# taichi-dev/taichi-nerfs

Measured on AMD Instinct MI355X. Metric: training rays/sec, higher is better.
Workload: dtype f32-table+f16-mlp

## Files before the change

include/ngp_hip.h:

```cpp
#ifndef NGP_HIP_H
#define NGP_HIP_H

#include <stdint.h>

#ifdef __cplusplus
extern "C" {
#endif

#define NGP_MAX_LEVELS 16
#define NGP_ABI_VERSION 3

typedef struct ngp_hash_levels {
    int32_t  n_levels;
    int32_t  n_features;
    int32_t  begin_fast_hash_level;
    int32_t  total_entries;
    float    scale[NGP_MAX_LEVELS];
    uint32_t resolution[NGP_MAX_LEVELS];
    uint32_t map_size[NGP_MAX_LEVELS];
    uint32_t offset[NGP_MAX_LEVELS];
    uint32_t bwd_plan;
} ngp_hash_levels;

#define NGP_BWD_PLAN_DETERMINISTIC 1u
#define NGP_BWD_PLAN_CONCENTRATED  2u

int ngp_abi_version(void);


int ngp_hash_levels_init(ngp_hash_levels* lv, double max_params, int levels, double base_res,
                         double max_res, int features);

int ngp_ray_aabb(const float* rays_o, const float* rays_d, float scale, int n_rays,
                 float* hits_t , void* stream);

int ngp_bitfield_coarsen(const uint8_t* density_bitfield, int cascades, int grid_size, uint32_t* coarse,
                         void* stream);
int ngp_march_train_count_ex(const float* rays_o, const float* rays_d, const float* hits_t,
                             const uint8_t* density_bitfield, const uint32_t* coarse, const float* noise,
                             int cascades, int grid_size, float scale, float exp_step_factor, int max_samples,
                             int n_rays, float* stage, int32_t* counts, void* stream);
int ngp_march_train_fused(const float* rays_o, const float* rays_d, const float* hits_t,
                          const uint8_t* density_bitfield, const uint32_t* coarse, const float* noise, int cascades,
                          int grid_size, float scale, float exp_step_factor, int max_samples, int n_rays,
                          float* stage, int32_t* ctr, int32_t* rays_a, int32_t* total, float* xyzs, float* dirs,
                          float* deltas, float* ts, void* stream);
int ngp_march_train_fused_cap(const float* rays_o, const float* rays_d, const float* hits_t, const uint8_t* density_bitfield,
                              const uint32_t* coarse, const float* noise, int cascades, int grid_size, float scale,
                              float exp_step_factor, int max_samples, int n_rays, long long capacity, float* stage, int32_t* ctr,
                              int32_t* rays_a, int32_t* total, float* xyzs, float* dirs, float* deltas, float* ts, void* stream);
int ngp_march_train_fused_rng(const float* rays_o, const float* rays_d, const float* hits_t, const uint8_t* density_bitfield,
                              const uint32_t* coarse, unsigned long long seed, int cascades, int grid_size, float scale,
                              float exp_step_factor, int max_samples, int n_rays, float* stage, int32_t* ctr, int32_t* rays_a,
                              int32_t* total, float* xyzs, float* dirs, float* deltas, float* ts, void* stream);
int ngp_march_train_fused_shaped(const float* rays_o, const float* rays_d, const float* hits_t, const uint8_t* density_bitfield,
                                 const uint32_t* coarse, const float* noise, unsigned long long seed, int cascades, int grid_size,
                                 float scale, float exp_step_factor, int max_samples, int n_rays, int block_waves, int lds_pad_bytes,
                                 float* stage, int32_t* ctr, int32_t* rays_a, int32_t* total, float* xyzs, float* dirs, float* deltas,
                                 float* ts, void* stream);
int ngp_rng_uniform(unsigned long long seed, int n, float* out, void* stream);
int ngp_march_train_scan(const int32_t* counts, int n_rays, int32_t* rays_a ,
                         int32_t* total , void* stream);
int ngp_march_train_write(const float* rays_o, const float* rays_d, const int32_t* rays_a,
                          const float* stage, int max_samples, int n_rays,
                          float* xyzs, float* dirs, float* deltas, float* ts, void* stream);

int ngp_march_test(const float* rays_o, const float* rays_d, float* hits_t ,
                   const int64_t* alive_indices, const uint8_t* density_bitfield,
                   int cascades, int grid_size, float scale, float exp_step_factor,
                   int max_samples, int n_alive,
                   int64_t* ray_indices, uint8_t* valid_mask, float* deltas, float* ts,
                   int32_t* samples_counter, void* stream);

int ngp_hash_fwd_f32(const float* xyzs , const float* table,
                     const ngp_hash_levels* lv, int n, float* out , void* stream);
int ngp_hash_bwd_f32(const float* xyzs, const float* dout ,
                     const ngp_hash_levels* lv, int n, float* dtable, void* stream);

int ngp_hash_bwd_input_f32 (const float* xyzs, const float* table, const float* denc , const ngp_hash_levels* lv, int n,
                            float* dxyzs , void* stream);
int ngp_hash_bwd_input_bf16(const float* xyzs, const uint16_t* table, const float* denc , const ngp_hash_levels* lv, int n,
                            float* dxyzs , void* stream);
int ngp_hash_bwd_input_f16 (const float* xyzs, const uint16_t* table, const uint16_t* denc , const ngp_hash_levels* lv,
                            int n, float* dxyzs , void* stream);

int ngp_hash_bwd2_gather_f32 (const float* xyzs, const float* table, const float* denc , const float* ddx ,
                              const ngp_hash_levels* lv, int n, float* d_denc , float* d_xyzs ,
                              void* stream);
int ngp_hash_bwd2_gather_bf16(const float* xyzs, const uint16_t* table, const float* denc , const float* ddx ,
                              const ngp_hash_levels* lv, int n, float* d_denc , float* d_xyzs ,
                              void* stream);
int ngp_hash_bwd2_table_f32  (const float* xyzs, const float* denc , const float* ddx , const ngp_hash_levels* lv,
                              int n, float* dtable , void* stream);

int ngp_hash_fwd_f32_ex(const float* xyzs, const float* table, const ngp_hash_levels* lv, int n_max,
                        const int32_t* n_dev, int normalize, float lo, float hi, int enc_pairs, float* out,
                        void* stream);
int ngp_hash_fwd_bf16_ex(const float* xyzs, const uint16_t* table, const ngp_hash_levels* lv, int n_max,
                         const int32_t* n_dev, int normalize, float lo, float hi, int enc_pairs, float* out,
                         void* stream);
int ngp_hash_fwd_list(const float* xyzs, const void* table, int table_kind, const ngp_hash_levels* lv, int n_max,
                      const int32_t* n_list, const int32_t* list, int normalize, float lo, float hi, int enc_pairs, float* out,
                      void* stream);

typedef struct ngp_triplane_levels {
    int32_t  n_levels;
    int32_t  n_features;
    int32_t  max_res;
    int32_t  reserved;
    float    scale[NGP_MAX_LEVELS];
    uint32_t resolution[NGP_MAX_LEVELS];
} ngp_triplane_levels;

int ngp_triplane_levels_init(ngp_triplane_levels* lv, double base_res, double max_res, int levels, int features);
int ngp_triplane_fwd_f32(const float* xyzs , const float* table, const ngp_triplane_levels* lv, int n, int normalize,
                         float lo, float hi, float* out , void* stream);
int ngp_triplane_bwd_f32(const float* xyzs, const float* dout , const float* table, const ngp_triplane_levels* lv,
                         int n, int normalize, float lo, float hi, float* dtable, void* stream);

int ngp_voxel_fwd(const float* xyzs , const float* dirs , const float* sh, const float* density, int n,
                  int grid_size, int sh_degree, float grid_min, float grid_radius, float* sigmas , float* rgbs ,
                  void* stream);
int ngp_voxel_density(const float* xyzs, const float* density, int n, int grid_size, float grid_min, float grid_radius,
                      float* sigmas, void* stream);
int ngp_voxel_bwd(const float* xyzs, const float* dirs, const float* sigmas, const float* rgbs, const float* dsigmas ,
                  const float* drgbs , int n, int grid_size, int sh_degree, float grid_min, float grid_radius, float* dsh,
                  float* ddensity, void* stream);
int ngp_voxel_trilinear_fwd(const float* xyzs , const float* dirs , const float* sh, const float* density,
                            int n, int grid_size, int sh_degree, float grid_min, float grid_radius, float* sigmas ,
                            float* rgbs , void* stream);
int ngp_voxel_trilinear_density(const float* xyzs, const float* density, int n, int grid_size, float grid_min, float grid_radius,
                                float* sigmas, void* stream);
int ngp_voxel_trilinear_bwd(const float* xyzs, const float* dirs, const float* sigmas, const float* rgbs, const float* dsigmas ,
                            const float* drgbs , int n, int grid_size, int sh_degree, float grid_min, float grid_radius,
                            float* dsh, float* ddensity, void* stream);
int ngp_voxel_occ_scratch_doubles(void);
int ngp_voxel_occ_pack(const float* density_grid, long long n_bytes, double density_threshold, double* scratch, uint8_t* bitfield,
                       void* stream);

int ngp_hash_fwd_f16(const float* xyzs, const uint16_t* table, const ngp_hash_levels* lv, int n,
                     uint16_t* out , void* stream);
int ngp_hash_bwd_f16(const float* xyzs, const uint16_t* dout, const ngp_hash_levels* lv, int n,
                     uint16_t* dtable , void* stream);

int ngp_hash_fwd_f16_ex(const float* xyzs, const uint16_t* table, const ngp_hash_levels* lv, int n_max,
                        const int32_t* n_dev, int normalize, float lo, float hi, int enc_pairs, float* out,
                        void* stream);
int ngp_check_finite_f16(const uint16_t* g, long long n, int32_t* found_inf, void* stream);

int ngp_sh16_fwd(const float* dirs , int n, float* out , void* stream);
int ngp_sh16_bwd(const float* dirs, const float* dout , int n, float* ddirs ,
                 void* stream);

int ngp_composite_train_fwd(const float* sigmas, const void* rgbs, int rgbs_is_half,
                            const float* deltas, const float* ts, const int32_t* rays_a,
                            float T_threshold, int n_rays,
                            int32_t* total_samples , float* opacity, float* depth,
                            float* rgb , float* ws , void* stream);
int ngp_composite_train_bwd(const float* dL_dopacity, const float* dL_ddepth, const float* dL_drgb,
                            const float* dL_dws, const float* sigmas, const void* rgbs,
                            int rgbs_is_half, const float* deltas, const float* ts,
                            const int32_t* rays_a, const float* opacity, const float* depth,
                            const float* rgb, const float* ws, float T_threshold, int n_rays,
                            float* dL_dsigmas, void* dL_drgbs, void* stream);
int ngp_composite_train_fwd_bg(const float* sigmas, const void* rgbs, int rgbs_is_half, const float* deltas, const float* ts,
                               const int32_t* rays_a, float T_threshold, int n_rays, int32_t* total_samples, float* opacity,
                               float* depth, float* rgb, float* ws, float* rgb_out, float bg, void* stream);
int ngp_composite_train_bwd_bg(const float* dL_dopacity, const float* dL_ddepth, const float* dL_drgb, const float* dL_dws,
                               const float* sigmas, const void* rgbs, int rgbs_is_half, const float* deltas, const float* ts,
                               const int32_t* rays_a, const float* opacity, const float* depth, const float* rgb, const float* ws,
                               float T_threshold, int n_rays, float* dL_dsigmas, void* dL_drgbs, float bg, void* stream);

int ngp_chunk_schedule(const int32_t* rays_a, const float* sigmas, const float* deltas, int n_rays, int begin, int len,
                       int prev_begin, float thr_stop, float* T_state, int32_t* list, int32_t* count, int32_t* count_zero,
                       void* stream);
int ngp_live_list(const int32_t* rays_a, const int32_t* vr_per_ray , int n_rays, int32_t* live_idx,
                  int32_t* live_total, int32_t* live_zero, void* stream);
int ngp_composite_train_fused_live(const float* sigmas, const void* rgbs, int rgbs_is_half, const float* deltas,
                                   const float* ts, const int32_t* rays_a, const float* target, float bg,
                                   const float* loss_scale, float T_threshold, int n_rays, int32_t* vr_per_ray,
                                   float* opacity, float* depth, float* rgb, float* ws, float* d_sigmas, void* d_rgbs,
                                   float* sq_err, int32_t* live_idx, int32_t* live_total, int32_t* live_zero,
                                   void* stream);

int ngp_live_compact(const int32_t* rays_a, const int32_t* vr_per_ray , int n_rays, int32_t* live_off,
                     int32_t* live_idx, int32_t* live_total, void* stream);
int ngp_mlp_bwd_live(const float* enc, const float* dirs, const uint16_t* wpack, const float* dsigmas, const uint16_t* drgbs,
                     int n_max, const int32_t* n_dev, const int32_t* live_idx, int enc_pairs, float* d_enc, float* dW,
                     int32_t* found_inf, void* stream);
int ngp_mlp_dw_parts_max(void);
int ngp_mlp_bwd_live_parts(const float* enc, const float* dirs, const uint16_t* wpack, const float* dsigmas,
                           const uint16_t* drgbs, int n_max, const int32_t* n_dev, const int32_t* live_idx, int enc_pairs,
                           float* d_enc, float* dW_parts, int32_t* found_inf, void* stream);
int ngp_mlp_dw_reduce(const float* dW_parts, int n_parts, float* dW, void* stream);
int ngp_hash_bwd_f32_live(const float* xyzs, const float* dout, const ngp_hash_levels* lv, int n_max, const int32_t* n_dev,
                          const int32_t* live_idx, int normalize, float lo, float hi, int enc_pairs, float* dtable,
                          int32_t* found_inf, void* stream);
int ngp_hash_bwd_f16_live(const float* xyzs, const float* dout, const ngp_hash_levels* lv, int n_max, const int32_t* n_dev,
                          const int32_t* live_idx, int normalize, float lo, float hi, int enc_pairs, uint16_t* dtable,
                          int32_t* found_inf, void* stream);
long long ngp_hash_bwd_sliced_workspace(const ngp_hash_levels* lv, int n_max);
int ngp_hash_bwd_sliced_prep(const float* xyzs, const ngp_hash_levels* lv, int n_max, const int32_t* n_dev,
                             const int32_t* live_idx, int normalize, float lo, float hi, void* workspace,
                             long long workspace_bytes, void* stream);
int ngp_hash_bwd_sliced_main(const float* dout, const ngp_hash_levels* lv, int n_max, const int32_t* n_dev, int enc_pairs,
                             float* dtable, int32_t* found_inf, const void* workspace, long long workspace_bytes,
                             void* stream);
int ngp_hash_bwd_sliced_main_slabs(const float* dout, const ngp_hash_levels* lv, int n_max, const int32_t* n_dev, int enc_pairs,
                                   void* dtable, int table_is_f16, int32_t* found_inf, const void* workspace,
                                   long long workspace_bytes, const float* mlp_dw_parts, int n_parts, float* mlp_dw, void* stream);
long long ngp_hash_bwd_sliced_adam_prefix(const ngp_hash_levels* lv);
int ngp_hash_bwd_sliced_main_adam_step(const float* dout, const ngp_hash_levels* lv, int n_max, const int32_t* n_dev, int enc_pairs,
                                       float* dtable, const void* workspace, long long workspace_bytes, const float* mlp_dw_parts,
                                       int n_parts, float* mlp_dw, float* table, float* table_m, float* table_v, uint16_t* table_bf16,
                                       float* state_f, int32_t* state_i, float lr0, float eta_min, int t_max, float beta1, float beta2,
                                       float eps, float growth, float backoff, int growth_interval, void* stream);
int ngp_hash_bwd_sliced_main_f16(const float* dout, const ngp_hash_levels* lv, int n_max, const int32_t* n_dev, int enc_pairs,
                                 uint16_t* dtable_f16, int32_t* found_inf, const void* workspace, long long workspace_bytes,
                                 void* stream);
int ngp_hash_bwd_f32_sliced(const float* xyzs, const float* dout, const ngp_hash_levels* lv, int n_max, const int32_t* n_dev,
                            const int32_t* live_idx, int normalize, float lo, float hi, int enc_pairs, float* dtable,
                            int32_t* found_inf, void* workspace, long long workspace_bytes, void* stream);

int ngp_composite_test(const float* sigmas, const void* rgbs, int rgbs_is_half, const float* deltas,
                       const float* ts, const int64_t* pack_info ,
                       int64_t* alive_indices , float T_threshold, int n_alive,
                       float* opacity, float* depth, float* rgb, void* stream);

int ngp_mlp_wpack_halfs(void);
int ngp_mlp_pack(const float* W1, const float* W2, const float* W3, const float* W4, const float* W5,
                 int enc_pairs, uint16_t* wpack, void* stream);
int ngp_mlp_fwd(const float* enc, const float* dirs, const uint16_t* wpack, int n, float* sigmas,
                uint16_t* rgbs, void* stream);
int ngp_mlp_bwd(const float* enc, const float* dirs, const uint16_t* wpack, const float* dsigmas,
                const uint16_t* drgbs, int n, float* d_enc, float* dW, void* stream);

int ngp_mlp_fwd_ex(const float* enc, const float* dirs, const uint16_t* wpack, int n_max, const int32_t* n_dev,
                   int enc_pairs, float* sigmas, uint16_t* rgbs, void* stream);
int ngp_mlp_fwd_list(const float* enc, const float* dirs, const uint16_t* wpack, int n_max, const int32_t* n_list,
                     const int32_t* list, int enc_pairs, float* sigmas, uint16_t* rgbs, void* stream);

int ngp_event_create(void** event);
int ngp_event_record(void* event, void* stream);
int ngp_stream_wait_event(void* stream, void* event);
int ngp_event_destroy(void* event);
int ngp_event_synchronize(void* event);
int ngp_stream_create_low_priority(void** stream, int* least, int* greatest);
int ngp_stream_destroy(void* stream);
int ngp_host_alloc(void** host, long long bytes);
int ngp_host_free(void* host);
int ngp_copy_to_host_async(void* host, const void* dev, long long bytes, void* stream);

typedef struct ngp_render_args {
    const float* rays_o; const float* rays_d; const float* hits_t ; const float* noise ;
    int32_t n_rays, max_samples;
    const uint8_t* bitfield; uint32_t* coarse; int32_t rebuild_coarse, cascades, grid_size;
    float scale, exp_step_factor, T_threshold;
    const void* table; int32_t table_kind , enc_pairs;
    const ngp_hash_levels* levels; float lo, hi;
    const float* w[5]; uint16_t* wpack;
    long long cap;
    float* stage; int32_t* march_ctr; float* xyzs; float* dirs; float* deltas; float* ts; float* enc; float* sigmas; uint16_t* rgbs; float* ws;
    int32_t* rays_a; int32_t* total; int32_t* vr_per_ray; float* opacity; float* depth; float* rgb;
    const float* g_opacity; const float* g_depth; const float* g_rgb; const float* g_ws;
    float* d_sigmas; uint16_t* d_rgbs; float* d_enc; int32_t* live_off; int32_t* live_idx; int32_t* live_total;
    void* workspace; long long workspace_bytes;
    int32_t force_atomic, reserved;
    float* dW_parts; int32_t* live_zero;
    float* dW ; void* dtable ; long long dtable_bytes;
    float bg; int32_t clear_grads; float* rgb_out;
} ngp_render_args;
int ngp_render_train_fwd(const ngp_render_args* args, void* stream);
int ngp_render_train_bwd(const ngp_render_args* args, void* stream);

int ngp_mse_loss_grad(const float* rgb, const float* opacity, const float* target, float bg, int n_rays,
                      float* state_f, float* g_rgb, float* g_opacity, void* stream);
int ngp_mse_loss_grad_rays(const float* rgb, const float* opacity, const float* target, float bg, int n_rays,
                           const float* state_f, float* g_rgb, float* g_opacity, float* sq_err, void* stream);
int ngp_train_prologue(float* state_f, int32_t* state_i, float lr0, float eta_min, int t_max, float beta1,
                       float beta2, float growth, float backoff, int growth_interval, void* stream);
int ngp_train_prologue_reduce(float* state_f, int32_t* state_i, float lr0, float eta_min, int t_max, float beta1,
                              float beta2, float growth, float backoff, int growth_interval, const float* dW_parts,
                              int n_parts, float* dW, void* stream);
int ngp_adam_amp_prologue(float* state_f, int32_t* state_i, const float* grad_scale, const float* found_inf, float lr,
                          float beta1, float beta2, void* stream);
#define NGP_ADAM_MULTI_MAX 16
int ngp_adam_multi(int n_tensors, float* const* p, float* const* g, float* const* m, float* const* v, const long long* n,
                   const float* state_f, const int32_t* state_i, float beta1, float beta2, float eps, void* stream);
int ngp_check_finite_multi(int n_tensors, const float* const* g, const long long* n, float* found_inf, void* stream);
int ngp_adam_amp_check_prologue(int n_tensors, const float* const* g, const long long* n, float* found_inf, float* clear_next,
                                uint32_t* done, float* state_f, int32_t* state_i, const float* grad_scale, float lr, float beta1,
                                float beta2, void* stream);
int ngp_cast_f32_bf16(const float* src, uint16_t* dst, long long n, void* stream);
int ngp_adam_all_ex(float* table, void* table_g, int grad_is_f16, float* table_m, float* table_v, long long n,
                    uint16_t* table_16, int copy_kind, float* mlp, float* mlp_g, float* mlp_m, float* mlp_v,
                    const float* state_f, const int32_t* state_i, float beta1, float beta2, float eps, int enc_pairs,
                    uint16_t* wpack, void* stream);
int ngp_adam_mlp_pack(float* p, float* g, float* m, float* v, const float* state_f, const int32_t* state_i,
                      float beta1, float beta2, float eps, int enc_pairs, uint16_t* wpack, void* stream);

int ngp_morton3d(const int32_t* coords , int m, int32_t* indices, void* stream);
int ngp_morton3d_invert(const int32_t* indices, int m, int32_t* coords , void* stream);
int ngp_packbits(const float* density_grid , float threshold, int n_bytes,
                 uint8_t* bitfield, void* stream);

int ngp_distortion_fwd(const float* ws, const float* deltas, const float* ts, const int32_t* rays_a, int n_rays,
                       float* loss, float* ws_inc, float* wts_inc, void* stream);
int ngp_distortion_bwd(const float* dL_dloss, const float* ws, const float* deltas, const float* ts,
                       const float* ws_inc, const float* wts_inc, const int32_t* rays_a, int n_rays,
                       float* dL_dws, void* stream);

int ngp_get_rays(const float* directions , const float* poses, int per_ray_pose, int n, float* rays_o,
                 float* rays_d, void* stream);
int ngp_stage_batch(const float* a, float* da, const float* b, float* db, const float* c, float* dc, int n, void* stream);
int ngp_sample_rays(const float* poses , const float* directions , const float* rays, int ray_c,
                    long long hw, const int64_t* img_idx, long long img0, const int64_t* pix_idx, int n, float* rays_o,
                    float* rays_d, float* rgb, void* stream);

int ngp_march_train_bwd(const float* d_xyzs , const float* d_dirs , const float* ts ,
                        const int32_t* rays_a , int n_rays, float* d_rays_o , float* d_rays_d , void* stream);
int ngp_sample_rays_bwd(const float* directions , const int64_t* img_idx , long long img0,
                        const int64_t* pix_idx , const float* d_rays_o , const float* d_rays_d ,
                        int n, int n_img, float* d_poses , void* stream);
int ngp_get_rays_bwd(const float* directions , const float* d_rays_o, const float* d_rays_d, int n, float* d_poses , void* stream);

int ngp_occ_compact(const float* density_grid, float threshold, int n_cells, int32_t* list, int32_t* count,
                    int32_t* scratch , void* stream);
int ngp_sorted_uniforms(const float* u, int m, int sets, float* work, float* out, void* stream);
int ngp_occ_sample(const float* u_cell, const float* u_pick, const float* u_jit, const int32_t* list, const int32_t* count,
                   int m, int grid_size, float s, float half_grid, int32_t* indices, float* xyzs, void* stream);
int ngp_occ_all_cells(const float* u_jit, int n_cells, int grid_size, float s, float half_grid, float* xyzs, void* stream);
int ngp_occ_scatter(const int32_t* indices, const float* sigmas, int n, float* tmp, void* stream);
int ngp_occ_scatter_max(const int32_t* indices, const float* sigmas, int n, float* tmp, void* stream);
int ngp_occ_stats_floats(void);
int ngp_occ_merge(float* density_grid, const float* tmp, float decay, int n, float* stats, void* stream);
int ngp_occ_pack(const float* density_grid, float* stats, float density_threshold, int n_bytes, uint8_t* bitfield,
                 void* stream);

int ngp_deploy_shade(const float* xyzs, const float* dirs, const float* table, const ngp_hash_levels* lv, const float* sigma_w,
                     const float* rgb_w, int n, float* sigmas , float* rgbs , float* enc_out, void* stream);

int ngp_deploy_render(const float* rays_o, const float* rays_d, const uint8_t* density_bitfield, const uint32_t* coarse ,
                      const float* table, const ngp_hash_levels* lv, const float* sigma_w, const float* rgb_w, int n_rays,
                      int max_samples, float T_threshold, float* rgb, float* opacity, float* depth, int32_t* n_samples, float* t_last,
                      void* stream);

long long ngp_mesh_workspace_bytes(int nx, int ny, int nz);
int ngp_mesh_count(const float* values, int nx, int ny, int nz, float iso, int sign, void* workspace, int32_t* counts ,
                   void* stream);
int ngp_mesh_emit(const float* values, int nx, int ny, int nz, float iso, int sign, const float* lo ,
                  const float* h , const void* workspace, float* vertices, float* normals , int32_t* faces,
                  void* stream);

#define NGP_MESH_SDF_MAX_LEAF 8
long long ngp_mesh_bvh_bytes(long long n_faces, int leaf_size);
int ngp_mesh_bvh_build(const float* vertices, const int32_t* faces, const int32_t* order, int n_faces, int leaf_size, float* boxes,
                       void* stream);
int ngp_mesh_sdf_query(const float* points, int n, const float* vertices, const int32_t* faces, const int32_t* order, const float* boxes,
                       int n_faces, int leaf_size, const float* edge_normals , const float* vertex_normals ,
                       float* sdf, float* closest , int32_t* face , int32_t* feature ,
                       void* stream);

#define NGP_RAYCAST_ANY_HIT 1
#define NGP_RAYCAST_CULL_BACK 2
#define NGP_RAYCAST_CULL_FRONT 4
int ngp_mesh_raycast(const float* rays_o, const float* rays_d, int n,
                     const float* vertices, const int32_t* faces, const int32_t* order, const float* boxes,
                     int n_faces, int leaf_size, float t_min, float t_max, int flags,
                     float* t , int32_t* face , float* bary ,
                     int32_t* side , void* stream);

long long ngp_mesh_winding_bytes(long long n_faces, int leaf_size);
int ngp_mesh_winding_build(const float* vertices, const int32_t* faces, const int32_t* order, const float* boxes, int n_faces,
                           int leaf_size, float* moments, void* stream);
int ngp_mesh_winding_query(const float* points, int n, const float* vertices, const int32_t* faces, const int32_t* order,
                           const float* moments, int n_faces, int leaf_size, float beta, int order_terms ,
                           float* winding , void* stream);

long long ngp_mesh_components_bytes(int n_faces, int n_vertices);
int ngp_mesh_components_rounds(const int32_t* faces, int n_faces, int n_vertices, int32_t* parent, int32_t* changed, int n_rounds,
                               void* stream);
int ngp_mesh_components_label(const int32_t* faces, int n_faces, int n_vertices, const int32_t* parent, void* workspace,
                              int32_t* vertex_component, int32_t* face_component, int32_t* counts , void* stream);
int ngp_mesh_components_edge_keys(const int32_t* faces, int n_faces, int n_vertices, int64_t* keys , void* stream);
int ngp_mesh_components_table(int n_faces, int n_vertices, const int32_t* vertex_component, const int32_t* face_component,
                              const int64_t* sorted_keys, int n_components, int32_t* table , void* stream);
long long ngp_mesh_components_partial_bytes(int n_faces, int n_components);
int ngp_mesh_components_measure(const float* vertices, const int32_t* faces, const int64_t* order, int n_faces, int n_vertices,
                                const int32_t* face_start, const int32_t* block_start, int n_components, void* partials, double* area,
                                double* volume, float* lo, float* hi, void* stream);
int ngp_mesh_select_count(int n_faces, int n_vertices, const int32_t* vertex_component, const int32_t* face_component,
                          const uint8_t* keep, int n_components, void* workspace, int32_t* vertex_map, int32_t* face_map,
                          int32_t* counts , void* stream);
int ngp_mesh_select_emit(const float* vertices, const float* normals , const int32_t* faces, int n_faces, int n_vertices,
                         const int32_t* vertex_map, const int32_t* face_map, int n_out_vertices, int n_out_faces, float* out_vertices,
                         float* out_normals , int32_t* out_faces, void* stream);

int ngp_surface_composite_fwd(const float* sdf, const float* cosv, const float* rgbs, const float* aux ,
                              const float* deltas, const float* ts, const int32_t* rays_a, const float* inv_s ,
                              float cos_anneal, float T_threshold, int n_rays, float bg, int32_t* total_samples, float* opacity,
                              float* depth, float* rgb, float* rgb_out , float* aux_out , float* ws,
                              float* alphas, void* stream);
int ngp_surface_composite_bwd(const float* dL_dopacity, const float* dL_ddepth, const float* dL_drgb, const float* dL_daux,
                              const float* dL_dws, const float* sdf, const float* cosv, const float* rgbs, const float* aux,
                              const float* deltas, const float* ts, const int32_t* rays_a, const float* inv_s, float cos_anneal, int n_rays,
                              float bg, const int32_t* total_samples, const float* alphas, float* d_sdf, float* d_cos, float* d_rgbs,
                              float* d_aux , float* d_inv_s , float* workspace , void* stream);

int ngp_resample_count(const float* ws, const float* deltas, const float* ts, const int32_t* rays_a, const float* noise, int n_rays,
                       int n_orig, long long n_samples, int K, float floor_w, float* cdf, float* stage_t, int32_t* stage_j,
                       int32_t* counts, int32_t* total , void* stream);
int ngp_resample_scan(const int32_t* counts, const int32_t* rays_a, int n_rays, int32_t* rays_a_out, int32_t* total, void* stream);
int ngp_resample_write(const float* rays_o, const float* rays_d, const float* deltas, const float* ts, const int32_t* rays_a,
                       const int32_t* rays_a_out, const float* stage_t, const int32_t* stage_j, int n_rays, int n_orig,
                       long long n_samples, int K, float* xyzs, float* dirs, float* deltas_out, float* ts_out, int32_t* parent,
                       void* stream);

int ngp_sdf_eval(const float* xyzs, const float* table, const ngp_hash_levels* lv, const float* wpack, int width, int depth, float scale,
                 int n, float* f, float* enc_out , void* stream);
int ngp_sdf_trace(const float* rays_o, const float* rays_d, const uint8_t* density_bitfield, const uint32_t* coarse ,
                  const float* table, const ngp_hash_levels* lv, const float* wpack, int width, int depth, int cascades, float scale,
                  int grid_size, int n_rays, float eps, float step_scale, float min_step, int n_refine, int max_evals, int32_t* status,
                  float* t, float* xyz, int32_t* n_eval, float* f_last, unsigned long long* stats , void* stream);

#ifdef __cplusplus
}
#endif
#endif
```

include/ngp_hip_experimental.h:

```cpp
#ifndef NGP_HIP_EXPERIMENTAL_H
#define NGP_HIP_EXPERIMENTAL_H
#include "ngp_hip.h"

#ifdef __cplusplus
extern "C" {
#endif

int ngp_adam_all(float* table, float* table_g, float* table_m, float* table_v, long long n, uint16_t* table_bf16,
                 float* mlp, float* mlp_g, float* mlp_m, float* mlp_v, const float* state_f, const int32_t* state_i,
                 float beta1, float beta2, float eps, int enc_pairs, uint16_t* wpack, void* stream);

int ngp_adam_step(float* p, float* g, float* m, float* v, long long n, const float* state_f,
                  const int32_t* state_i, float beta1, float beta2, float eps, void* stream);

int ngp_adam_step_bf16(float* p, float* g, float* m, float* v, long long n, const float* state_f,
                       const int32_t* state_i, float beta1, float beta2, float eps, uint16_t* p_bf16, void* stream);

int ngp_composite_train_fused(const float* sigmas, const void* rgbs, int rgbs_is_half, const float* deltas,
                              const float* ts, const int32_t* rays_a, const float* target, float bg,
                              const float* loss_scale, float T_threshold, int n_rays, int32_t* vr_per_ray,
                              float* opacity, float* depth, float* rgb, float* ws, float* d_sigmas, void* d_rgbs,
                              float* sq_err, void* stream);

int ngp_hash_bwd_f16_ex(const float* xyzs, const float* dout, const ngp_hash_levels* lv, int n_max,
                        const int32_t* n_dev, int normalize, float lo, float hi, int enc_pairs, uint16_t* dtable,
                        int32_t* found_inf, void* stream);

int ngp_hash_bwd_f32_ex(const float* xyzs, const float* dout, const ngp_hash_levels* lv, int n_max,
                        const int32_t* n_dev, int normalize, float lo, float hi, int enc_pairs, float* dtable,
                        int32_t* found_inf, void* stream);

int ngp_hash_bwd_sliced_debug(void* device_buffer);

int ngp_hash_bwd_sliced_plan(const ngp_hash_levels* lv, uint16_t* tasks, int max_tasks, uint16_t* xoff , uint16_t* xlen ,
                             uint8_t* nrep , uint32_t* merge_mask, uint32_t* single_mask);

int ngp_march_train_count(const float* rays_o, const float* rays_d, const float* hits_t,
                          const uint8_t* density_bitfield, const float* noise,
                          int cascades, int grid_size, float scale, float exp_step_factor,
                          int max_samples, int n_rays,
                          float* stage , int32_t* counts ,
                          void* stream);

int ngp_mlp_bwd_ex(const float* enc, const float* dirs, const uint16_t* wpack, const float* dsigmas,
                   const uint16_t* drgbs, int n_max, const int32_t* n_dev, int enc_pairs, float* d_enc, float* dW,
                   int32_t* found_inf, void* stream);

int ngp_hash_bwd_sliced_main_adam(const float* dout, const ngp_hash_levels* lv, int n_max, const int32_t* n_dev, int enc_pairs,
                                  float* dtable, const void* workspace, long long workspace_bytes, const float* mlp_dw_parts,
                                  int n_parts, float* mlp_dw, float* table, float* table_m, float* table_v, uint16_t* table_bf16,
                                  const float* state_f, const int32_t* state_i, float beta1, float beta2, float eps,
                                  void* stream);

int ngp_hash_bwd_sliced_main_levels(const float* dout, const ngp_hash_levels* lv, int n_max, const int32_t* n_dev, int enc_pairs,
                                    float* dtable, int32_t* found_inf, const void* workspace, long long workspace_bytes,
                                    unsigned int level_mask, int max_blocks, void* stream);

int ngp_p2p_max_peers(void);
int ngp_p2p_push(const void* src, long long n_per_peer, int elem_bytes, int world, void* const* peer_dst, int32_t* const* peer_flags,
                 long long dst_offset, int broadcast, int rank, int step, uint32_t* done, void* stream);
int ngp_p2p_wait(const int32_t* flags, int world, int step, long long max_spins, const float* inbox, long long n, float scale, int reduce,
                 float* out, int32_t* err, void* stream);

#ifdef __cplusplus
}
#endif
#endif
```

taichi-nerfs_amd/csrc/hash_bwd_lds.hip:

```cpp
#include "ngp_device.h"
#include "hash_common.h"

namespace ngp {

constexpr int BW_SLICE_LOG2 = 13;
constexpr int BW_SLICE_ENTRIES = 1 << BW_SLICE_LOG2;
constexpr int BW_MAX_SLICES = 64;
constexpr int BW_THREADS = 1024;
constexpr int BW_WAVES = BW_THREADS / 64;
constexpr int BW_Q = 256;
constexpr int BW_MAX_TASKS = 1536;
constexpr int BW_PREP_BLOCKS = 2048;
constexpr size_t BW_CTR_BYTES = 64;
constexpr int BW_PERSISTENT_BLOCKS = 256;

struct BwdPlan {
    int32_t n_blocks;
    uint32_t merge_mask;
    uint32_t diag;
    uint32_t det;
    int32_t merge_chunks;
    uint8_t nrep[NGP_MAX_LEVELS];
    uint16_t task[BW_MAX_TASKS];
    uint16_t xoff[8], xlen[8];
// ... 352 lines not shown
            const int i0 = w0 * 64 + lane, i1 = i0 + 64;
            const Batch nxt = load_batch(level, i0, i0 < n, i1, (w0 + 1 < hi_w) && i1 < n, xyzc, dout, plane, enc_pairs, nl, P.diag, HALF);
            accumulate_batch<KIND>(P, sl, pend, slice, found_inf);
            pend = nxt;
        }
        accumulate_batch<KIND>(P, sl, pend, slice, found_inf);
        return;
    }
    int qhead = 0, qlen = 0;
    int SCW = 64;
    if (K == KIND_MERGE || K == KIND_MERGE0) {
        SCW = 4; while (SCW < 64 && SCW < 2 * (int)P.map.ns) SCW <<= 1;
        if (P.merge_chunks > 0) while (SCW > 4 && (hi_w - lo_w) < P.merge_chunks * SCW) SCW >>= 1;
    }
    const int n_sc = (hi_w - lo_w + SCW - 1) / SCW;
    auto load_words = [&](int c) -> unsigned long long {
        const int w = lo_w + c * SCW + lane;
        return (c < n_sc && lane < SCW && w < hi_w) ? brow[w] : 0ull;
    };
    auto grab = [&]() -> int {
        int c = 0;
        if (lane == 0) c = (int)atomicAdd(next_sc, 1u);
        return __builtin_amdgcn_readfirstlane(c);
    };
    auto drain = [&]() {
        __builtin_amdgcn_fence(__ATOMIC_ACQ_REL, "wavefront");
        __builtin_amdgcn_wave_barrier();
        const int i0 = (int)q[(qhead + lane) & (BW_Q - 1)], i1 = (int)q[(qhead + 64 + lane) & (BW_Q - 1)];
        const Batch nxt = load_batch(level, i0, true, i1, true, xyzc, dout, plane, enc_pairs, nl, P.diag, HALF);
        accumulate_batch<KIND>(P, sl, pend, slice, found_inf);
        pend = nxt;
        __builtin_amdgcn_wave_barrier();
        qhead = (qhead + 128) & (BW_Q - 1); qlen -= 128;
    };
    int sc = grab();
    unsigned long long cur = load_words(sc);
    while (sc < n_sc) {
        const int sc_next = grab();
        const unsigned long long nxtw = load_words(sc_next);
        const int wbase = lo_w + sc * SCW;
        if (K == KIND_MERGE || K == KIND_MERGE0) {
            unsigned long long nonzero = __ballot(cur != 0ull);
            while (nonzero) {
                const int k = __builtin_ctzll(nonzero);
                nonzero &= nonzero - 1;
                const unsigned long long b = ((unsigned long long)(uint32_t)__builtin_amdgcn_readlane((int)(cur >> 32), k) << 32) |
                                             (uint32_t)__builtin_amdgcn_readlane((int)cur, k);
                const bool hit = (b >> lane) & 1ull;
                const int pos = qlen + __builtin_amdgcn_mbcnt_hi((uint32_t)(b >> 32), __builtin_amdgcn_mbcnt_lo((uint32_t)b, 0));
                if (hit) q[(qhead + pos) & (BW_Q - 1)] = (uint32_t)((wbase + k) * 64 + lane);
                qlen += __popcll(b);
                if (qlen >= 128) drain();
            }
        } else {
            const unsigned long long w = cur;
            if (__ballot(w != 0ull) != 0ull) {
                int total = 0, pass = 0;
                do {
                    const int sbase = qhead + 128;
                    int off = 0;
#pragma unroll
                    for (int pc = 0; pc < 8; ++pc) {
                        const uint32_t b8 = (uint32_t)(w >> (8 * pc)) & 0xffu;
                        const unsigned long long nz = __ballot(b8 != 0u);
                        const int dst = off - 64 * pass + __builtin_amdgcn_mbcnt_hi((uint32_t)(nz >> 32), __builtin_amdgcn_mbcnt_lo((uint32_t)nz, 0));
                        if (b8 != 0u && (uint32_t)dst < 64u) q[(sbase + dst) & (BW_Q - 1)] = b8 | ((uint32_t)lane << 8) | ((uint32_t)pc << 14);
                        off += __popcll(nz);
                    }
                    total = off;
                    __builtin_amdgcn_fence(__ATOMIC_ACQ_REL, "wavefront");
                    __builtin_amdgcn_wave_barrier();
                    const uint32_t d = (lane < total - 64 * pass) ? q[(sbase + lane) & (BW_Q - 1)] : 0u;
                    __builtin_amdgcn_fence(__ATOMIC_ACQ_REL, "wavefront");
                    __builtin_amdgcn_wave_barrier();
                    uint32_t bits = d & 0xffu;
                    const uint32_t s0 = (uint32_t)(wbase + (int)((d >> 8) & 63u)) * 64u + 8u * (d >> 14);
                    unsigned long long live = __ballot(bits != 0u);
                    while (live) {
                        const int pos = qlen + __builtin_amdgcn_mbcnt_hi((uint32_t)(live >> 32), __builtin_amdgcn_mbcnt_lo((uint32_t)live, 0));
                        if (bits != 0u) {
                            q[(qhead + pos) & (BW_Q - 1)] = s0 + (uint32_t)__builtin_ctz(bits);
                            bits &= bits - 1u;
                        }
                        qlen += __popcll(live);
                        if (qlen >= 128) drain();
                        live = __ballot(bits != 0u);
                    }
                    ++pass;
                } while (64 * pass < total);
            }
        }
        if ((K == KIND_MERGE || K == KIND_MERGE0) && P.det && qlen > 0) {
            __builtin_amdgcn_fence(__ATOMIC_ACQ_REL, "wavefront");
            __builtin_amdgcn_wave_barrier();
            const bool v0 = lane < qlen, v1 = lane + 64 < qlen;
            const int i0 = v0 ? (int)q[(qhead + lane) & (BW_Q - 1)] : 0, i1 = v1 ? (int)q[(qhead + 64 + lane) & (BW_Q - 1)] : 0;
            const Batch nxt = load_batch(level, i0, v0, i1, v1, xyzc, dout, plane, enc_pairs, nl, P.diag, HALF);
            accumulate_batch<KIND>(P, sl, pend, slice, found_inf);
            pend = nxt;
            __builtin_amdgcn_wave_barrier();
            qhead = (qhead + 128) & (BW_Q - 1); qlen = 0;
        }
        cur = nxtw; sc = sc_next;
    }
    if (qlen > 0) {
        __builtin_amdgcn_fence(__ATOMIC_ACQ_REL, "wavefront");
        __builtin_amdgcn_wave_barrier();
        const bool v0 = lane < qlen, v1 = lane + 64 < qlen;
        const int i0 = v0 ? (int)q[(qhead + lane) & (BW_Q - 1)] : 0, i1 = v1 ? (int)q[(qhead + 64 + lane) & (BW_Q - 1)] : 0;
        const Batch nxt = load_batch(level, i0, v0, i1, v1, xyzc, dout, plane, enc_pairs, nl, P.diag, HALF);
        accumulate_batch<KIND>(P, sl, pend, slice, found_inf);
        pend = nxt;
    }
    accumulate_batch<KIND>(P, sl, pend, slice, found_inf);
}

__device__ __forceinline__ uint32_t claim_task(const BwdPlan& plan, uint32_t* __restrict__ ctr, uint32_t xcc, bool& own_empty) {
    const int lane = threadIdx.x & 63;
    if (!own_empty) {
        uint32_t old = 0u;
        if (lane == 0) old = atomicAdd(&ctr[xcc], 1u);
        old = (uint32_t)__builtin_amdgcn_readfirstlane((int)old);
        const uint32_t f = old & 0xffffu, b = old >> 16;
        if (f + b < plan.xlen[xcc]) return plan.xoff[xcc] + f;
        own_empty = true;
    }
    uint32_t dead = 1u << xcc;
    for (int tries = 0; tries < 7; ++tries) {
        int left = 0;
        if (lane < 8 && !((dead >> lane) & 1u)) {
            const uint32_t c = __atomic_load_n(&ctr[lane], __ATOMIC_RELAXED);
            left = (int)plan.xlen[lane] - (int)((c & 0xffffu) + (c >> 16));
        }
        int key = left > 0 ? (left << 3) | (7 - lane) : 0;
#pragma unroll
        for (int d = 1; d < 8; d <<= 1) key = max(key, __shfl_xor(key, d, NGP_WAVE));
        key = __builtin_amdgcn_readfirstlane(key);
        if (key <= 0) break;
        const int best = 7 - (key & 7);
        uint32_t old = 0u;
        if (lane == 0) old = atomicAdd(&ctr[best], 0x10000u);
        old = (uint32_t)__builtin_amdgcn_readfirstlane((int)old);
        const uint32_t f = old & 0xffffu, b = old >> 16;
        if (f + b < plan.xlen[best]) return plan.xoff[best] + plan.xlen[best] - 1u - b;
        dead |= 1u << best;
    }
    return 0xffffffffu;
}

struct MlpSlabs {
    const float* parts;
    int n_parts;
    float* dW;
};

struct FlushAdam {
    float* p;
    float* m;
    float* v;
    uint16_t* shadow;
    const float* sf;
    const int32_t* si;
    float beta1, beta2, eps;
};

struct StepSchedule {
    float* sf;
    int32_t* si;
    float lr0, eta_min;
    int t_max;
    float growth, backoff;
    int growth_interval;
};

template <bool HALF, int ADAM>
__global__ void __launch_bounds__(BW_THREADS) hash_bwd_lds_kernel(const float* __restrict__ xyzc,
                                                                  const unsigned long long* __restrict__ bitmap, size_t wstride,
                                                                  const float* __restrict__ dout, ngp_hash_levels lv, int n,
                                                                  const int32_t* __restrict__ n_dev, int enc_pairs, BwdPlan plan,
                                                                  void* __restrict__ dtable ,
                                                                  int32_t* __restrict__ found_inf, uint32_t* __restrict__ ctr,
                                                                  unsigned long long* __restrict__ dbg, MlpSlabs mlp, FlushAdam ad_in,
                                                                  StepSchedule sch) {
    __shared__ double slice[2 * BW_SLICE_ENTRIES];
    __shared__ float s_sf[8];
    __shared__ int32_t s_si[8];
    FlushAdam ad = ad_in;
    const bool own_schedule = ADAM != 0 && sch.sf != nullptr;
    if (own_schedule) {
        if (threadIdx.x == 0) {
#pragma unroll
            for (int k = 0; k < 8; ++k) { s_sf[k] = sch.sf[k]; s_si[k] = sch.si[k]; }
            train_prologue_thread(s_sf, s_si, sch.lr0, sch.eta_min, sch.t_max, ad.beta1, ad.beta2, sch.growth, sch.backoff,
                                  sch.growth_interval);
        }
        ad.sf = s_sf; ad.si = s_si;
    }
    __shared__ uint32_t queues[BW_WAVES * BW_Q];
    __shared__ uint32_t next_sc;
    __shared__ uint32_t s_claim;
    if (mlp.parts) {
        for (int b = blockIdx.x; b < NGP_MLP_REDUCE_BLOCKS; b += gridDim.x) {
            mlp_dw_reduce_block(mlp.parts, mlp.n_parts, mlp.dW, b);
            __syncthreads();
        }
    }
    const size_t plane = (size_t)n;
    if (n_dev) n = min(n, *n_dev);
    if (n <= 0 && !ADAM) return;
    if (n < 0) n = 0;
    const int tid = threadIdx.x;
    uint32_t xcc;
    asm volatile("s_getreg_b32 %0, hwreg(HW_REG_XCC_ID)" : "=s"(xcc));
    xcc &= 7u;
    double2* s2 = reinterpret_cast<double2*>(slice);
    for (int j = tid; j < BW_SLICE_ENTRIES; j += BW_THREADS) s2[j] = make_double2(0.0, 0.0);
    bool own_empty = false;
    if (tid < 64) {
        const uint32_t c0 = claim_task(plan, ctr, xcc, own_empty);
        if (tid == 0) { s_claim = c0; next_sc = 0u; }
    }
    __syncthreads();
    uint32_t claim = s_claim;
  while (claim != 0xffffffffu) {
    const uint32_t task = plan.task[claim];
    unsigned long long t_begin = 0;
    if (dbg) t_begin = wall_clock64();
    const int level = task & 0xf, rep = (task >> 10) & 0x3f, nrep = plan.nrep[level];
    const uint32_t sl = (task >> 4) & 0x3f;
    LevelParams P;
    P.scale = lv.scale[level]; P.res = lv.resolution[level]; P.size = lv.map_size[level]; P.offset = lv.offset[level];
    P.dense = level < lv.begin_fast_hash_level;
    P.mode = level_mode(lv, level);
    P.map = slice_map(P.size, P.res, P.dense);
    P.diag = plan.diag;
    P.det = plan.det;
    P.merge_chunks = plan.merge_chunks;
    const bool single = P.size <= (uint32_t)BW_SLICE_ENTRIES;
    const bool merge = (plan.merge_mask >> level) & 1u;
    const bool hashed = !P.dense && P.mode == 1u && P.res < (1u << BW_SLICE_LOG2) && !single;

    unsigned long long t_init = 0;
    if (dbg) t_init = wall_clock64();
    uint32_t* q = queues + (tid >> 6) * BW_Q;
    const unsigned long long* brow = bitmap + ((size_t)level * BW_MAX_SLICES + sl) * wstride;
    if (merge && P.dense && P.mode == 0u) bwd_task<KIND_MERGE0 | (HALF ? KIND_HALF : 0)>(P, level, sl, single, n, rep, nrep, xyzc, brow, dout, plane, enc_pairs, lv.n_levels, slice, q, &next_sc, found_inf);
    else if (merge) bwd_task<KIND_MERGE | (HALF ? KIND_HALF : 0)>(P, level, sl, single, n, rep, nrep, xyzc, brow, dout, plane, enc_pairs, lv.n_levels, slice, q, &next_sc, found_inf);
    else if (hashed) bwd_task<KIND_HASHED | (HALF ? KIND_HALF : 0)>(P, level, sl, single, n, rep, nrep, xyzc, brow, dout, plane, enc_pairs, lv.n_levels, slice, q, &next_sc, found_inf);
    else bwd_task<KIND_GENERIC | (HALF ? KIND_HALF : 0)>(P, level, sl, single, n, rep, nrep, xyzc, brow, dout, plane, enc_pairs, lv.n_levels, slice, q, &next_sc, found_inf);
    unsigned long long t_wave = 0;
    if (dbg) t_wave = wall_clock64();
    __syncthreads();
    unsigned long long t_acc = 0;
    if (dbg) t_acc = wall_clock64();
    if (tid < 64) {
        const uint32_t c1 = claim_task(plan, ctr, xcc, own_empty);
        if (tid == 0) { s_claim = c1; next_sc = 0u; }
    }
    if (HALF) {
        typedef _Float16 half2v __attribute__((ext_vector_type(2)));
        half2v* dh = reinterpret_cast<half2v*>(dtable) + P.offset;
        for (int j = tid; j < BW_SLICE_ENTRIES; j += BW_THREADS) {
            const double2 a = s2[j];
            if (a.x == 0.0 && a.y == 0.0) continue;
            s2[j] = make_double2(0.0, 0.0);
            const uint32_t h = entry_of(P.map, sl, (uint32_t)j);
            half2v val;
            val.x = (_Float16)(float)a.x; val.y = (_Float16)(float)a.y;
            if (nrep == 1) dh[h] = dh[h] + val;
            else if (!(val.x == (_Float16)0 && val.y == (_Float16)0))
                __builtin_amdgcn_global_atomic_fadd_v2f16((__attribute__((address_space(1))) half2v*)(dh + h), val);
        }
    } else if (ADAM && nrep == 1) {
        const bool skip = ad.si[SI_SKIP] != 0;
        const AdamConsts ac = adam_consts(ad.sf, ad.beta1, ad.beta2, ad.eps);
        float2* p2 = reinterpret_cast<float2*>(ad.p) + P.offset;
        float2* m2 = reinterpret_cast<float2*>(ad.m) + P.offset;
        float2* v2 = reinterpret_cast<float2*>(ad.v) + P.offset;
        uint32_t* sh = reinterpret_cast<uint32_t*>(ad.shadow) + P.offset;
        constexpr int UNR = BW_SLICE_ENTRIES / BW_THREADS;
        static_assert(UNR * BW_THREADS == BW_SLICE_ENTRIES, "one trip covers the slice");
        {
            float2 pi[UNR], mi[UNR], vi[UNR];
            uint32_t h[UNR];
#pragma unroll
            for (int k = 0; k < UNR; ++k) {
                const int j = tid + k * BW_THREADS;
                h[k] = entry_of(P.map, sl, (uint32_t)j);
                const uint32_t hc = (!skip && h[k] < P.size) ? h[k] : 0u;
                mi[k] = m2[hc]; vi[k] = v2[hc]; pi[k] = p2[hc];
            }
#pragma unroll
            for (int k = 0; k < UNR; ++k) {
                const int j = tid + k * BW_THREADS;
                const double2 a = s2[j];
                if (a.x != 0.0 || a.y != 0.0) s2[j] = make_double2(0.0, 0.0);
                const float gx = 0.0f + (float)a.x, gy = 0.0f + (float)a.y;
                float2 mk = mi[k], vk = vi[k], pk = pi[k];
                const bool in = !skip && h[k] < P.size;
                if (!in || (gx == 0.f && gy == 0.f && mk.x == 0.f && mk.y == 0.f && vk.x == 0.f && vk.y == 0.f)) continue;
                if (!(isfinite(gx) && isfinite(gy))) { atomicOr(&ctr[9], 1u); continue; }
                adam_update(pk.x, mk.x, vk.x, gx, ac);
                adam_update(pk.y, mk.y, vk.y, gy, ac);
                p2[h[k]] = pk; m2[h[k]] = mk; v2[h[k]] = vk;
                if (ADAM == 2) sh[h[k]] = f32_to_bf16_bits(pk.x) | (f32_to_bf16_bits(pk.y) << 16);
            }
        }
    } else {
    float2* dl = reinterpret_cast<float2*>(reinterpret_cast<float*>(dtable) + 2 * (size_t)P.offset);
    for (int j = tid; j < BW_SLICE_ENTRIES; j += BW_THREADS) {
        const double2 a = s2[j];
        if (a.x == 0.0 && a.y == 0.0) continue;
        s2[j] = make_double2(0.0, 0.0);
        const uint32_t h = entry_of(P.map, sl, (uint32_t)j);
        const float vx = (float)a.x, vy = (float)a.y;
        if (nrep == 1) {
            float2 d = dl[h];
            d.x += vx; d.y += vy;
            dl[h] = d;
        } else {
            float* dp = reinterpret_cast<float*>(dl + h);
            if (vx != 0.0f) unsafeAtomicAdd(dp, vx);
            if (vy != 0.0f) unsafeAtomicAdd(dp + 1, vy);
        }
    }
    }
    if (dbg) {
        if (tid == 0 && claim < (uint32_t)BW_MAX_TASKS) {
            unsigned long long* o = dbg + 8 * (size_t)claim;
            o[0] = task; o[1] = t_begin; o[2] = t_init; o[3] = t_wave; o[4] = t_acc; o[5] = wall_clock64(); o[6] = xcc & 0xf; o[7] = (unsigned long long)n;
        }
    }
    __syncthreads();
    claim = s_claim;
  }
    if (tid == 0) {
        if (atomicAdd(&ctr[8], 1u) == gridDim.x - 1u) {
            for (int x = 0; x < 8; ++x) ctr[x] = 0u;
            ctr[8] = 0u;
            const uint32_t overflow = ADAM ? __atomic_load_n(&ctr[9], __ATOMIC_RELAXED) : 0u;
            if (ADAM) ctr[9] = 0u;
            if (own_schedule) {
#pragma unroll
                for (int k = 0; k < 8; ++k) { sch.sf[k] = s_sf[k]; sch.si[k] = s_si[k]; }
                if (overflow) sch.si[SI_FOUND_INF] = 1;
            }
        }
    }
}

struct Knobs {
    int rep_target = 48, merge_res = 128, dense_min_rep = 8;
    uint32_t level_mask = 0xffffffffu, diag = 0u;
    int blocks = 0;
    bool deterministic = false;
    int hashed_rep_res = 0, hashed_rep = 1;
    bool merge_hashed = false;
    int merge_chunks = 32;
    bool operator==(const Knobs& o) const {
        return merge_chunks == o.merge_chunks && rep_target == o.rep_target && merge_res == o.merge_res && dense_min_rep == o.dense_min_rep && level_mask == o.level_mask &&
               diag == o.diag && blocks == o.blocks && deterministic == o.deterministic && hashed_rep_res == o.hashed_rep_res &&
               hashed_rep == o.hashed_rep && merge_hashed == o.merge_hashed;
    }
};
static Knobs read_knobs() {
    Knobs k;
    if (const char* e = ngp_experiment("bwd_rep_target")) k.rep_target = atoi(e) > 0 ? atoi(e) : k.rep_target;
    if (const char* e = ngp_experiment("bwd_merge_res")) k.merge_res = atoi(e);
    if (const char* e = ngp_experiment("bwd_dense_min_rep")) k.dense_min_rep = atoi(e) > 0 ? atoi(e) : k.dense_min_rep;
    if (const char* e = ngp_experiment("bwd_merge_chunks")) k.merge_chunks = atoi(e) >= 0 ? atoi(e) : k.merge_chunks;
#ifdef NGP_BWD_DIAG
    if (const char* e = ngp_experiment("bwd_levels")) k.level_mask = (uint32_t)strtoul(e, nullptr, 0);
    if (const char* e = ngp_experiment("bwd_diag")) k.diag = (uint32_t)atoi(e);
    if (const char* e = ngp_experiment("bwd_blocks")) k.blocks = atoi(e);
#endif
    return k;
}
static void apply_modes(Knobs& k, uint32_t plan_bits) {
    k.deterministic = (plan_bits & NGP_BWD_PLAN_DETERMINISTIC) != 0u;
    if (plan_bits & NGP_BWD_PLAN_CONCENTRATED) {
        static const int res = [] { const char* e = ngp_experiment("bwd_hashed_rep_res"); return e ? atoi(e) : 256; }();
        static const int rep = [] { const char* e = ngp_experiment("bwd_hashed_rep"); return e && atoi(e) > 0 ? atoi(e) : 3; }();
        static const bool mh = [] { const char* e = ngp_experiment("bwd_merge_hashed"); return e ? atoi(e) != 0 : false; }();
        k.hashed_rep_res = res; k.hashed_rep = rep; k.merge_hashed = mh;
    } else { k.hashed_rep_res = 0; k.hashed_rep = 1; k.merge_hashed = false; }
}
static Knobs knobs(uint32_t plan_bits) {
    static const bool dynamic = ngp_experiment("bwd_knobs_dynamic") != nullptr;
    static const Knobs fixed = read_knobs();
    Knobs k;
#ifndef NGP_BWD_DIAG
    if (!dynamic) { k = fixed; apply_modes(k, plan_bits); return k; }
#endif
    k = read_knobs();
    apply_modes(k, plan_bits);
    return k;
}

static bool build_plan_with(const ngp_hash_levels& lv, BwdPlan& plan, uint32_t& single_mask, int dense_min_rep, const Knobs& K) {
    if (lv.n_features != 2 || lv.n_levels < 1 || lv.n_levels > NGP_MAX_LEVELS) return false;
    struct Lvl { int level, n_slices, nrep, tasks; };
    Lvl lvls[NGP_MAX_LEVELS];
    single_mask = 0u;
    plan.merge_mask = 0u;
    const int rep_target = K.rep_target;
    const int merge_res = K.merge_res;
    const uint32_t level_mask = K.level_mask;
    for (int l = 0; l < lv.n_levels; ++l) {
        const uint32_t size = lv.map_size[l];
        const int ns = (int)((size + BW_SLICE_ENTRIES - 1) / BW_SLICE_ENTRIES);
        if (ns < 1 || ns > BW_MAX_SLICES || size % 2 != 0) return false;
        int nrep = ns >= BW_MAX_SLICES ? 1 : (rep_target + ns / 2) / ns;
        if (l < lv.begin_fast_hash_level && ns > 1 && nrep < dense_min_rep) nrep = dense_min_rep;
        if (l >= lv.begin_fast_hash_level && (int)lv.resolution[l] <= K.hashed_rep_res && nrep < K.hashed_rep) nrep = K.hashed_rep;
        if (nrep < 1) nrep = 1;
        if (nrep > 63) nrep = 63;
        if (K.deterministic) nrep = 1;
        lvls[l] = {l, ns, nrep, ((level_mask >> l) & 1u) ? ns * nrep : 0};
        plan.nrep[l] = (uint8_t)nrep;
        if (ns == 1) single_mask |= 1u << l;
        if ((int)lv.resolution[l] <= merge_res && (l < lv.begin_fast_hash_level || K.merge_hashed)) plan.merge_mask |= 1u << l;
    }
    for (int l = lv.n_levels; l < NGP_MAX_LEVELS; ++l) plan.nrep[l] = 1;
    plan.diag = K.diag;
    plan.det = K.deterministic ? 1u : 0u;
    plan.merge_chunks = K.merge_chunks;
    static thread_local uint16_t lists[8][BW_MAX_TASKS];
    int len[8] = {0, 0, 0, 0, 0, 0, 0, 0};
    float load[8] = {0.f, 0.f, 0.f, 0.f, 0.f, 0.f, 0.f, 0.f};
    auto encode = [](int level, int slice, int rep) { return (uint16_t)(level | (slice << 4) | (rep << 10)); };
    auto least = [&]() { int b = 0; for (int x = 1; x < 8; ++x) if (load[x] < load[b]) b = x; return b; };
    auto cost = [&](const Lvl& L) {
        const float S = 400.0f;
        if (L.level >= lv.begin_fast_hash_level) return 3.0f + 1.9f * S * 4.0f / (float)L.n_slices / (float)L.nrep;
        const float frac = L.n_slices == 1 ? 1.0f : (L.n_slices < 8 ? 1.5f : 2.7f) / (float)L.n_slices;
        return 3.0f + 2.7f * S * frac / (float)L.nrep;
    };
    int order[NGP_MAX_LEVELS];
    for (int l = 0; l < lv.n_levels; ++l) order[l] = l;
    for (int a = 0; a < lv.n_levels; ++a)
        for (int b = a + 1; b < lv.n_levels; ++b) {
            const float cb = lvls[order[b]].tasks * cost(lvls[order[b]]), ca = lvls[order[a]].tasks * cost(lvls[order[a]]);
            if (cb > ca || (cb == ca && order[b] > order[a])) { const int t = order[a]; order[a] = order[b]; order[b] = t; }
        }
    int total = 0;
    for (int a = 0; a < lv.n_levels; ++a) total += lvls[order[a]].tasks;
    if (total > BW_MAX_TASKS - 64) return false;
    for (int pass = 0; pass < 2; ++pass)
        for (int a = 0; a < lv.n_levels; ++a) {
            const Lvl& L = lvls[order[a]];
            if (L.tasks == 0) continue;
            const int chunk = L.level < lv.begin_fast_hash_level ? 16 : 32;
            const int full = (L.tasks / chunk) * chunk;
            int t = 0, x = 0;
            for (int s = 0; s < L.n_slices; ++s)
                for (int r = 0; r < L.nrep; ++r, ++t) {
                    const bool in_full = t < full;
                    if ((pass == 0) != in_full) continue;
                    if (pass == 0 ? (t % chunk == 0) : (t == full)) x = least();
                    lists[x][len[x]++] = encode(L.level, s, r);
                    load[x] += cost(L);
                }
        }
    float lcost[NGP_MAX_LEVELS];
    for (int l = 0; l < lv.n_levels; ++l) lcost[l] = cost(lvls[l]);
    int nb = 0;
    for (int x = 0; x < 8; ++x) {
        for (int a = 1; a < len[x]; ++a) {
            const uint16_t t = lists[x][a];
            int b = a - 1;
            while (b >= 0 && lcost[lists[x][b] & 0xf] < lcost[t & 0xf]) { lists[x][b + 1] = lists[x][b]; --b; }
            lists[x][b + 1] = t;
        }
        plan.xoff[x] = (uint16_t)nb; plan.xlen[x] = (uint16_t)len[x];
        for (int p = 0; p < len[x]; ++p) plan.task[nb++] = lists[x][p];
    }
    plan.n_blocks = nb < BW_PERSISTENT_BLOCKS ? nb : BW_PERSISTENT_BLOCKS;
    if (K.blocks > 0 && K.blocks < plan.n_blocks) plan.n_blocks = K.blocks;
    return true;
}

static bool build_plan_uncached(const ngp_hash_levels& lv, BwdPlan& plan, uint32_t& single_mask, const Knobs& K) {
    for (int dense_min_rep = K.dense_min_rep; dense_min_rep >= 1; dense_min_rep >>= 1)
        if (build_plan_with(lv, plan, single_mask, dense_min_rep, K)) return true;
    return false;
}

struct PlanCache {
    bool valid = false, ok = false;
    ngp_hash_levels key;
    Knobs knobs;
    BwdPlan plan;
    uint32_t single_mask = 0u;
};
static const BwdPlan* get_plan(const ngp_hash_levels& lv, uint32_t& single_mask, uint32_t level_mask = 0xffffffffu, int max_blocks = 0) {
    static thread_local PlanCache cache[8];
    static thread_local int victim = 0;
    Knobs K = knobs(lv.bwd_plan);
    K.level_mask &= level_mask;
    if (max_blocks > 0 && (K.blocks <= 0 || max_blocks < K.blocks)) K.blocks = max_blocks;
    for (PlanCache& c : cache)
        if (c.valid && memcmp(&c.key, &lv, sizeof(lv)) == 0 && c.knobs == K) { single_mask = c.single_mask; return c.ok ? &c.plan : nullptr; }
    PlanCache& c = cache[victim];
    victim = (victim + 1) % 8;
    c.valid = true; c.key = lv; c.knobs = K;
    c.ok = build_plan_uncached(lv, c.plan, c.single_mask, K);
    single_mask = c.single_mask;
    return c.ok ? &c.plan : nullptr;
}

struct WsLayout {
    size_t ms, words;
    size_t off_bitmap, off_ctr, total;
};
static WsLayout ws_layout(const ngp_hash_levels& lv, int n_max) {
    WsLayout w;
    w.ms = ((size_t)n_max + 511) & ~(size_t)511;
    w.words = w.ms / 64;
    w.off_bitmap = w.ms * 3 * sizeof(float);
    w.off_ctr = w.off_bitmap + (size_t)lv.n_levels * BW_MAX_SLICES * w.words * sizeof(unsigned long long);
    w.total = w.off_ctr + BW_CTR_BYTES;
    return w;
}

}

using namespace ngp;

static unsigned long long* g_bwd_debug = nullptr;

extern "C" {

int ngp_hash_bwd_sliced_debug(void* device_buffer) { g_bwd_debug = (unsigned long long*)device_buffer; return 0; }

int ngp_hash_bwd_sliced_plan(const ngp_hash_levels* lv, uint16_t* tasks, int max_tasks, uint16_t* xoff, uint16_t* xlen, uint8_t* nrep,
                             uint32_t* merge_mask, uint32_t* single_mask) {
    if (!lv) return -1;
    uint32_t sm = 0;
    const BwdPlan* plan = get_plan(*lv, sm);
    if (!plan) return -2;
    int total = 0;
    for (int x = 0; x < 8; ++x) { total += plan->xlen[x]; if (xoff) xoff[x] = plan->xoff[x]; if (xlen) xlen[x] = plan->xlen[x]; }
    if (tasks) for (int k = 0; k < total && k < max_tasks; ++k) tasks[k] = plan->task[k];
    if (nrep) for (int l = 0; l < NGP_MAX_LEVELS; ++l) nrep[l] = plan->nrep[l];
    if (merge_mask) *merge_mask = plan->merge_mask;
    if (single_mask) *single_mask = sm;
    return total;
}

long long ngp_hash_bwd_sliced_workspace(const ngp_hash_levels* lv, int n_max) {
    if (!lv || n_max <= 0) return 0;
    return (long long)ws_layout(*lv, n_max).total;
}

int ngp_hash_bwd_sliced_prep(const float* xyzs, const ngp_hash_levels* lv, int n_max, const int32_t* n_dev, const int32_t* live_idx,
                             int normalize, float lo, float hi, void* workspace, long long workspace_bytes, void* stream) {
    if (n_max <= 0) return 0;
    if (!workspace || workspace_bytes < ngp_hash_bwd_sliced_workspace(lv, n_max)) return -1;
    uint32_t single_mask;
    const BwdPlan* plan = get_plan(*lv, single_mask);
    if (!plan) return -2;
    const WsLayout W = ws_layout(*lv, n_max);
    char* base = reinterpret_cast<char*>(workspace);
    float* xyzc = reinterpret_cast<float*>(base);
    unsigned long long* bitmap = reinterpret_cast<unsigned long long*>(base + W.off_bitmap);
    uint32_t* ctr = reinterpret_cast<uint32_t*>(base + W.off_ctr);
    const XyzNorm nm = {normalize, lo, hi};
    const PrepLevels pl = make_prep_levels(*lv);
    int lds_begin = 0;
    while (lds_begin < lv->n_levels && pl.l[lds_begin].map.ns <= 8u) ++lds_begin;
    for (int l = lds_begin; l < lv->n_levels; ++l)
        if (pl.l[l].map.ns <= 8u) return -2;
    static const int batch = [] { const char* e = ngp_experiment("prep_batch"); return e ? atoi(e) : 1; }();
#define NGP_PREP(B) hipLaunchKernelGGL(hash_bwd_prep_kernel<B>, dim3(BW_PREP_BLOCKS), dim3(256), 0, (hipStream_t)stream, xyzs, live_idx, pl, \
                                       lv->n_levels, lv->begin_fast_hash_level, lds_begin, n_max, n_dev, nm, W.words, single_mask, xyzc, bitmap, ctr)
    if (batch == 3) NGP_PREP(3); else if (batch == 6) NGP_PREP(6); else if (batch == 12) NGP_PREP(12); else NGP_PREP(1);
#undef NGP_PREP
    NGP_LAUNCH_CHECK();
    return 0;
}

static int adam_first_level(const ngp_hash_levels& lv, const BwdPlan& plan) {
    int first = lv.n_levels;
    while (first > 0 && plan.nrep[first - 1] == 1) --first;
    for (int l = 0; l < first; ++l)
        if (plan.nrep[l] == 1) return -1;
    return first < lv.n_levels ? first : -1;
}

static int sliced_main(bool half, const float* dout, const ngp_hash_levels* lv, int n_max, const int32_t* n_dev, int enc_pairs,
                       void* dtable, int32_t* found_inf, const void* workspace, long long workspace_bytes, void* stream,
                       uint32_t level_mask = 0xffffffffu, int max_blocks = 0, MlpSlabs mlp = MlpSlabs{nullptr, 0, nullptr},
                       FlushAdam ad = FlushAdam{nullptr, nullptr, nullptr, nullptr, nullptr, nullptr, 0.f, 0.f, 0.f},
                       StepSchedule sch = StepSchedule{nullptr, nullptr, 0.f, 0.f, 0, 0.f, 0.f, 0}) {
    if (n_max <= 0) return 0;
    if (enc_pairs && !(lv->n_features == 2 && lv->n_levels == 16)) return -1;
    if (!workspace || workspace_bytes < ngp_hash_bwd_sliced_workspace(lv, n_max)) return -1;
    uint32_t single_mask;
    const BwdPlan* plan = get_plan(*lv, single_mask, level_mask, max_blocks);
    if (!plan) return -2;
    if (ad.p && (half || adam_first_level(*lv, *plan) < 0)) return -2;
    const WsLayout W = ws_layout(*lv, n_max);
    const char* base = reinterpret_cast<const char*>(workspace);
    const float* xyzc = reinterpret_cast<const float*>(base);
    const unsigned long long* bitmap = reinterpret_cast<const unsigned long long*>(base + W.off_bitmap);
    uint32_t* ctr = reinterpret_cast<uint32_t*>(const_cast<char*>(base) + W.off_ctr);
    if (plan->n_blocks <= 0) {
        return mlp.parts ? ngp_mlp_dw_reduce(mlp.parts, mlp.n_parts, mlp.dW, stream) : 0;
    }
#define NGP_BWD_LAUNCH(H, A)                                                                                                        \
    hipLaunchKernelGGL((hash_bwd_lds_kernel<H, A>), dim3(plan->n_blocks), dim3(BW_THREADS), 0, (hipStream_t)stream, xyzc, bitmap,    \
                       W.words, dout, *lv, n_max, n_dev, enc_pairs, *plan, dtable, found_inf, ctr, g_bwd_debug, mlp, ad, sch)
    if (half) NGP_BWD_LAUNCH(true, 0);
    else if (ad.p && ad.shadow) NGP_BWD_LAUNCH(false, 2);
    else if (ad.p) NGP_BWD_LAUNCH(false, 1);
    else NGP_BWD_LAUNCH(false, 0);
#undef NGP_BWD_LAUNCH
    NGP_LAUNCH_CHECK();
    return 0;
}

int ngp_hash_bwd_sliced_main(const float* dout, const ngp_hash_levels* lv, int n_max, const int32_t* n_dev, int enc_pairs, float* dtable,
                             int32_t* found_inf, const void* workspace, long long workspace_bytes, void* stream) {
    return sliced_main(false, dout, lv, n_max, n_dev, enc_pairs, dtable, found_inf, workspace, workspace_bytes, stream);
}

int ngp_hash_bwd_sliced_main_slabs(const float* dout, const ngp_hash_levels* lv, int n_max, const int32_t* n_dev, int enc_pairs,
                                   void* dtable, int table_is_f16, int32_t* found_inf, const void* workspace, long long workspace_bytes,
                                   const float* mlp_dw_parts, int n_parts, float* mlp_dw, void* stream) {
    if (!mlp_dw_parts || !mlp_dw || n_parts <= 0) return -1;
    return sliced_main(table_is_f16 != 0, dout, lv, n_max, n_dev, enc_pairs, dtable, found_inf, workspace, workspace_bytes, stream,
                       0xffffffffu, 0, MlpSlabs{mlp_dw_parts, n_parts, mlp_dw});
}

int ngp_hash_bwd_sliced_main_levels(const float* dout, const ngp_hash_levels* lv, int n_max, const int32_t* n_dev, int enc_pairs,
                                    float* dtable, int32_t* found_inf, const void* workspace, long long workspace_bytes,
                                    unsigned int level_mask, int max_blocks, void* stream) {
    return sliced_main(false, dout, lv, n_max, n_dev, enc_pairs, dtable, found_inf, workspace, workspace_bytes, stream, level_mask,
                       max_blocks);
}

int ngp_hash_bwd_sliced_main_f16(const float* dout, const ngp_hash_levels* lv, int n_max, const int32_t* n_dev, int enc_pairs,
                                 uint16_t* dtable_f16, int32_t* found_inf, const void* workspace, long long workspace_bytes,
                                 void* stream) {
    return sliced_main(true, dout, lv, n_max, n_dev, enc_pairs, dtable_f16, found_inf, workspace, workspace_bytes, stream);
}

long long ngp_hash_bwd_sliced_adam_prefix(const ngp_hash_levels* lv) {
    if (!lv) return -1;
    uint32_t sm;
    const BwdPlan* plan = get_plan(*lv, sm);
    if (!plan) return -2;
    const int first = adam_first_level(*lv, *plan);
    if (first < 0) return -2;
    return (long long)lv->offset[first] * lv->n_features;
}

int ngp_hash_bwd_sliced_main_adam(const float* dout, const ngp_hash_levels* lv, int n_max, const int32_t* n_dev, int enc_pairs,
                                  float* dtable, const void* workspace, long long workspace_bytes, const float* mlp_dw_parts,
                                  int n_parts, float* mlp_dw, float* table, float* table_m, float* table_v, uint16_t* table_bf16,
                                  const float* state_f, const int32_t* state_i, float beta1, float beta2, float eps, void* stream) {
    if (!table || !table_m || !table_v || !state_f || !state_i) return -1;
    const MlpSlabs mlp = (mlp_dw_parts && mlp_dw && n_parts > 0) ? MlpSlabs{mlp_dw_parts, n_parts, mlp_dw} : MlpSlabs{nullptr, 0, nullptr};
    return sliced_main(false, dout, lv, n_max, n_dev, enc_pairs, dtable, nullptr, workspace, workspace_bytes, stream, 0xffffffffu, 0, mlp,
                       FlushAdam{table, table_m, table_v, table_bf16, state_f, state_i, beta1, beta2, eps});
}

int ngp_hash_bwd_sliced_main_adam_step(const float* dout, const ngp_hash_levels* lv, int n_max, const int32_t* n_dev, int enc_pairs,
                                       float* dtable, const void* workspace, long long workspace_bytes, const float* mlp_dw_parts,
                                       int n_parts, float* mlp_dw, float* table, float* table_m, float* table_v, uint16_t* table_bf16,
                                       float* state_f, int32_t* state_i, float lr0, float eta_min, int t_max, float beta1, float beta2,
                                       float eps, float growth, float backoff, int growth_interval, void* stream) {
    if (!table || !table_m || !table_v || !state_f || !state_i || t_max <= 0 || n_max <= 0) return -1;
    const MlpSlabs mlp = (mlp_dw_parts && mlp_dw && n_parts > 0) ? MlpSlabs{mlp_dw_parts, n_parts, mlp_dw} : MlpSlabs{nullptr, 0, nullptr};
    return sliced_main(false, dout, lv, n_max, n_dev, enc_pairs, dtable, nullptr, workspace, workspace_bytes, stream, 0xffffffffu, 0, mlp,
                       FlushAdam{table, table_m, table_v, table_bf16, state_f, state_i, beta1, beta2, eps},
                       StepSchedule{state_f, state_i, lr0, eta_min, t_max, growth, backoff, growth_interval});
}

int ngp_hash_bwd_f32_sliced(const float* xyzs, const float* dout, const ngp_hash_levels* lv, int n_max, const int32_t* n_dev,
                            const int32_t* live_idx, int normalize, float lo, float hi, int enc_pairs, float* dtable,
                            int32_t* found_inf, void* workspace, long long workspace_bytes, void* stream) {
    if (n_max <= 0) return 0;
    if (enc_pairs && !(lv->n_features == 2 && lv->n_levels == 16)) return -1;
    const int rc = ngp_hash_bwd_sliced_prep(xyzs, lv, n_max, n_dev, live_idx, normalize, lo, hi, workspace, workspace_bytes, stream);
    if (rc != 0) return rc;
    return ngp_hash_bwd_sliced_main(dout, lv, n_max, n_dev, enc_pairs, dtable, found_inf, workspace, workspace_bytes, stream);
}

}
```

taichi-nerfs_amd/csrc/mlp.hip:

```cpp
#include "ngp_device.h"
#include <stdlib.h>

namespace ngp {

typedef _Float16 half_t;
typedef half_t half8 __attribute__((ext_vector_type(8)));
typedef half_t half4 __attribute__((ext_vector_type(4)));
typedef float floatx4 __attribute__((ext_vector_type(4)));

#define NGP_MFMA(a, b, c) __builtin_amdgcn_mfma_f32_16x16x32_f16((a), (b), (c), 0, 0, 0)

constexpr int N_FWD_FRAGS = 20;
constexpr int N_ALL_FRAGS = 42;
constexpr int F_W1 = 0;
constexpr int F_W2 = 4;
constexpr int F_W3 = 6;
constexpr int F_W4 = 10;
constexpr int F_W5 = 18;
constexpr int B_W5T = 20;
constexpr int B_W4T = 24;
constexpr int B_W3T = 32;
constexpr int B_W2T = 34;
constexpr int B_W1T = 38;

__device__ __forceinline__ int chain_k(int s, int g, int j) { return 32 * s + 16 * (j >> 2) + 4 * g + (j & 3); }

__device__ __forceinline__ int pair_nat(int p, int slot) { return slot < 2 ? 2 * p + slot : 2 * (15 - p) + (slot - 2); }
__device__ __forceinline__ int enc_feat(int pairs, int g, int j) { return pairs ? pair_nat(2 * g + (j >> 2), j & 3) : 8 * g + j; }
__device__ __forceinline__ int enc_row(int pairs, int mt, int i) { return pairs ? pair_nat(4 * mt + (i >> 2), i & 3) : 16 * mt + i; }

__device__ __forceinline__ void pack_one(int tid, const float* W1, const float* W2, const float* W3, const float* W4,
                                         const float* W5, int pairs, half_t* wpack) {
    const int j = tid & 7, lane = (tid >> 3) & 63, frag = tid >> 9;
    const int i = lane & 15, g = lane >> 4;
    float v = 0.0f;
    if (frag < F_W2) {
        const int mt = frag - F_W1;
        v = W1[(16 * mt + i) * 32 + enc_feat(pairs, g, j)];
    } else if (frag < F_W3) {
        const int s = frag - F_W2;
        v = W2[i * 64 + chain_k(s, g, j)];
    } else if (frag < F_W4) {
        const int mt = frag - F_W3;
        const int k = (j < 4) ? (4 * g + j) : (16 + 4 * g + (j - 4));
        v = W3[(16 * mt + i) * 32 + k];
    } else if (frag < F_W5) {
        const int mt = (frag - F_W4) >> 1, s = (frag - F_W4) & 1;
        v = W4[(16 * mt + i) * 64 + chain_k(s, g, j)];
    } else if (frag < B_W5T) {
        const int s = frag - F_W5;
        v = (i < 3) ? W5[i * 64 + chain_k(s, g, j)] : 0.0f;
    } else if (frag < B_W4T) {
        const int mt = frag - B_W5T;
        const int k = 4 * g + j;
        v = (j < 4 && k < 3) ? W5[k * 64 + 16 * mt + i] : 0.0f;
    } else if (frag < B_W3T) {
        const int mt = (frag - B_W4T) >> 1, s = (frag - B_W4T) & 1;
        v = W4[chain_k(s, g, j) * 64 + 16 * mt + i];
    } else if (frag < B_W2T) {
        const int s = frag - B_W3T;
        v = W3[chain_k(s, g, j) * 32 + 16 + i];
    } else if (frag < B_W1T) {
        const int mt = frag - B_W2T;
        v = (j < 4) ? W2[(4 * g + j) * 64 + 16 * mt + i] : 0.0f;
    } else {
        const int mt = (frag - B_W1T) >> 1, s = (frag - B_W1T) & 1;
        v = W1[chain_k(s, g, j) * 32 + enc_row(pairs, mt, i)];
    }
    wpack[tid] = (half_t)v;
}

__global__ void __launch_bounds__(256) mlp_pack_kernel(const float* __restrict__ W1, const float* __restrict__ W2,
                                                       const float* __restrict__ W3, const float* __restrict__ W4,
                                                       const float* __restrict__ W5, int pairs, half_t* __restrict__ wpack) {
    const int tid = blockIdx.x * blockDim.x + threadIdx.x;
    if (tid < N_ALL_FRAGS * 64 * 8) pack_one(tid, W1, W2, W3, W4, W5, pairs, wpack);
}

__device__ __forceinline__ void adam_mlp_pack_block(float* __restrict__ p, float* __restrict__ g, float* __restrict__ m,
                                                    float* __restrict__ v, const float* __restrict__ sf,
                                                    const int32_t* __restrict__ si, float beta1, float beta2, float eps,
                                                    int pairs, half_t* __restrict__ wpack) {
    __shared__ float wl[9408];
    const bool skip = si[SI_SKIP] != 0;
    const AdamConsts ac = adam_consts(sf, beta1, beta2, eps);
    constexpr int PER = (9408 + 1023) / 1024;
    float pi[PER], gi[PER], mi[PER], vi[PER];
#pragma unroll
    for (int k = 0; k < PER; ++k) {
        const int i = (int)threadIdx.x + 1024 * k, ic = i < 9408 ? i : 0;
        pi[k] = p[ic]; gi[k] = g[ic]; mi[k] = m[ic]; vi[k] = v[ic];
    }
#pragma unroll
    for (int k = 0; k < PER; ++k) {
        const int i = (int)threadIdx.x + 1024 * k;
        if (i >= 9408) continue;
        if (!skip) {
            float mk = mi[k], vk = vi[k];
            adam_update(pi[k], mk, vk, gi[k], ac);
            p[i] = pi[k]; m[i] = mk; v[i] = vk;
        }
        g[i] = 0.0f;
        wl[i] = pi[k];
    }
    __syncthreads();
    for (int item = threadIdx.x; item < N_ALL_FRAGS * 64; item += blockDim.x) {
#pragma unroll
        for (int j = 0; j < 8; ++j) pack_one(8 * item + j, wl, wl + 2048, wl + 3072, wl + 5120, wl + 9216, pairs, wpack);
    }
}

__global__ void __launch_bounds__(1024) adam_mlp_pack_kernel(float* __restrict__ p, float* __restrict__ g, float* __restrict__ m,
                                                             float* __restrict__ v, const float* __restrict__ sf,
                                                             const int32_t* __restrict__ si, float beta1, float beta2, float eps,
                                                             int pairs, half_t* __restrict__ wpack) {
    adam_mlp_pack_block(p, g, m, v, sf, si, beta1, beta2, eps, pairs, wpack);
}

template <int SHADOW, bool GRAD16>
__global__ void __launch_bounds__(1024) adam_all_kernel(float4* __restrict__ tp, void* __restrict__ tg, float4* __restrict__ tm,
                                                        float4* __restrict__ tv, long n4, uint2* __restrict__ shadow,
                                                        float* __restrict__ p, float* __restrict__ g, float* __restrict__ m,
                                                        float* __restrict__ v, const float* __restrict__ sf,
                                                        const int32_t* __restrict__ si, float beta1, float beta2, float eps,
                                                        int pairs, half_t* __restrict__ wpack) {
    if (blockIdx.x == 0) { if (p) adam_mlp_pack_block(p, g, m, v, sf, si, beta1, beta2, eps, pairs, wpack); }
    else adam_table_pass<SHADOW, GRAD16>(tp, tg, tm, tv, n4, sf, si, beta1, beta2, eps, shadow, (long)blockIdx.x - 1, (long)gridDim.x - 1);
}

typedef unsigned short ushort4v __attribute__((ext_vector_type(4)));
__device__ __forceinline__ half4 to_h4(const floatx4& d) { return __builtin_convertvector(d, half4); }
__device__ __forceinline__ half4 relu_h4(const floatx4& d) {
    const half4 z = {(half_t)0, (half_t)0, (half_t)0, (half_t)0};
    return __builtin_elementwise_max(to_h4(d), z);
}
__device__ __forceinline__ half8 cat_h4(const half4& a, const half4& b) {
    return __builtin_shufflevector(a, b, 0, 1, 2, 3, 4, 5, 6, 7);
}
__device__ __forceinline__ half4 mask_h4(const floatx4& d, const half4& act) {
    typedef unsigned int uint2v __attribute__((ext_vector_type(2)));
    const uint2v a = __builtin_bit_cast(uint2v, act), h = __builtin_bit_cast(uint2v, to_h4(d));
    uint2v r;
    asm("v_pk_sub_i16 %0, 0, %2\n\t"
        "v_pk_sub_i16 %1, 0, %3\n\t"
        "v_pk_ashrrev_i16 %0, 15, %0 op_sel_hi:[0,1]\n\t"
        "v_pk_ashrrev_i16 %1, 15, %1 op_sel_hi:[0,1]\n\t"
        "v_and_b32 %0, %0, %4\n\t"
        "v_and_b32 %1, %1, %5"
        : "=&v"(r.x), "=&v"(r.y) : "v"(a.x), "v"(a.y), "v"(h.x), "v"(h.y));
    return __builtin_bit_cast(half4, r);
}

__device__ __forceinline__ float fast_exp(float x) { return __expf(x); }
__device__ __forceinline__ float fast_rcp(float x) { return __builtin_amdgcn_rcpf(x); }
__device__ __forceinline__ float fast_rsq(float x) { return __builtin_amdgcn_rsqf(x); }

__device__ __forceinline__ half4 sh_quad(int g, float x, float y, float z) {
    const float xy = x * y, xz = x * z, yz = y * z, x2 = x * x, y2 = y * y, z2 = z * z;
    float a, b, c, d;
    if (g == 0) {
        a = 0.28209479177387814f; b = -0.48860251190291987f * y; c = 0.48860251190291987f * z; d = -0.48860251190291987f * x;
    } else if (g == 1) {
        a = 1.0925484305920792f * xy; b = -1.0925484305920792f * yz; c = 0.94617469575755997f * z2 - 0.31539156525251999f;
        d = -1.0925484305920792f * xz;
    } else if (g == 2) {
        a = 0.54627421529603959f * x2 - 0.54627421529603959f * y2; b = 0.59004358992664352f * y * (-3.0f * x2 + y2);
        c = 2.8906114426405538f * xy * z; d = 0.45704579946446572f * y * (1.0f - 5.0f * z2);
    } else {
        a = 0.3731763325901154f * z * (5.0f * z2 - 3.0f); b = 0.45704579946446572f * x * (1.0f - 5.0f * z2);
        c = 1.4453057213202769f * z * (x2 - y2); d = 0.59004358992664352f * x * (-x2 + 3.0f * y2);
    }
    half4 r;
    r[0] = (half_t)a; r[1] = (half_t)b; r[2] = (half_t)c; r[3] = (half_t)d;
    return r;
}

__device__ __forceinline__ half4 sh_quad_flat(int g, float x, float y, float z) {
    const float xy = x * y, xz = x * z, yz = y * z, x2 = x * x, y2 = y * y, z2 = z * z;
    const float a0 = 0.28209479177387814f, b0 = -0.48860251190291987f * y, c0 = 0.48860251190291987f * z, d0 = -0.48860251190291987f * x;
    const float a1 = 1.0925484305920792f * xy, b1 = -1.0925484305920792f * yz, c1 = 0.94617469575755997f * z2 - 0.31539156525251999f,
                d1 = -1.0925484305920792f * xz;
    const float a2 = 0.54627421529603959f * x2 - 0.54627421529603959f * y2, b2 = 0.59004358992664352f * y * (-3.0f * x2 + y2),
                c2 = 2.8906114426405538f * xy * z, d2 = 0.45704579946446572f * y * (1.0f - 5.0f * z2);
    const float a3 = 0.3731763325901154f * z * (5.0f * z2 - 3.0f), b3 = 0.45704579946446572f * x * (1.0f - 5.0f * z2),
                c3 = 1.4453057213202769f * z * (x2 - y2), d3 = 0.59004358992664352f * x * (-x2 + 3.0f * y2);
    const bool g0 = g == 0, g1 = g == 1, g2 = g == 2;
    half4 r;
    r[0] = (half_t)(g0 ? a0 : (g1 ? a1 : (g2 ? a2 : a3)));
    r[1] = (half_t)(g0 ? b0 : (g1 ? b1 : (g2 ? b2 : b3)));
    r[2] = (half_t)(g0 ? c0 : (g1 ? c1 : (g2 ? c2 : c3)));
    r[3] = (half_t)(g0 ? d0 : (g1 ? d1 : (g2 ? d2 : d3)));
    return r;
}

__device__ __forceinline__ void enc_ptrs(const float* __restrict__ enc, int pairs, size_t plane, int smp, int g, const float*& p0,
                                         const float*& p1) {
    if (pairs) { p0 = enc + ((size_t)(2 * g) * plane + smp) * 4; p1 = enc + ((size_t)(2 * g + 1) * plane + smp) * 4; }
    else { p0 = enc + (size_t)smp * 32 + 8 * g; p1 = p0 + 4; }
}

struct TileFwd {
    half8 b_enc;
    half4 a1[4];
    half4 h;
    half8 b_in3;
    half4 a3[4], a4[4];
    half4 rgb;
    float sigma;
};

__device__ __forceinline__ const half8& wfrag(const half8* __restrict__ wl, int id, int lane) { return wl[id * 64 + lane]; }

template <bool COLOR, bool FLAT_SH = false, class WF>
__device__ __forceinline__ void tile_forward_frags(const WF& W, int g, const float4& e0, const float4& e1,
                                                   float dx, float dy, float dz, TileFwd& t) {
    const floatx4 zero = {0.f, 0.f, 0.f, 0.f};
    t.b_enc[0] = (half_t)e0.x; t.b_enc[1] = (half_t)e0.y; t.b_enc[2] = (half_t)e0.z; t.b_enc[3] = (half_t)e0.w;
    t.b_enc[4] = (half_t)e1.x; t.b_enc[5] = (half_t)e1.y; t.b_enc[6] = (half_t)e1.z; t.b_enc[7] = (half_t)e1.w;
#pragma unroll
    for (int mt = 0; mt < 4; ++mt) t.a1[mt] = relu_h4(NGP_MFMA(W(F_W1 + mt), t.b_enc, zero));
    floatx4 d2 = NGP_MFMA(W(F_W2 + 0), cat_h4(t.a1[0], t.a1[1]), zero);
    d2 = NGP_MFMA(W(F_W2 + 1), cat_h4(t.a1[2], t.a1[3]), d2);
    t.h = to_h4(d2);
    t.sigma = expf((float)t.h[0]);
    if (!COLOR) return;
    const float inv = fast_rsq(dx * dx + dy * dy + dz * dz);
    const float x = (dx * inv + 1.0f) / 2.0f, y = (dy * inv + 1.0f) / 2.0f, z = (dz * inv + 1.0f) / 2.0f;
    t.b_in3 = cat_h4(FLAT_SH ? sh_quad_flat(g, x, y, z) : sh_quad(g, x, y, z), t.h);
    const float nan_dir = 0.0f * (x + y + z);
#pragma unroll
    for (int mt = 0; mt < 4; ++mt) t.a3[mt] = relu_h4(NGP_MFMA(W(F_W3 + mt), t.b_in3, zero));
    const half8 b30 = cat_h4(t.a3[0], t.a3[1]), b31 = cat_h4(t.a3[2], t.a3[3]);
#pragma unroll
    for (int mt = 0; mt < 4; ++mt) {
        floatx4 d4 = NGP_MFMA(W(F_W4 + 2 * mt), b30, zero);
        d4 = NGP_MFMA(W(F_W4 + 2 * mt + 1), b31, d4);
        t.a4[mt] = relu_h4(d4);
    }
    floatx4 d5 = NGP_MFMA(W(F_W5 + 0), cat_h4(t.a4[0], t.a4[1]), zero);
    d5 = NGP_MFMA(W(F_W5 + 1), cat_h4(t.a4[2], t.a4[3]), d5);
#pragma unroll
    for (int r = 0; r < 4; ++r) {
        const float c = (float)(half_t)d5[r] + nan_dir;
        t.rgb[r] = (half_t)fast_rcp(1.0f + fast_exp(-c));
    }
}

template <bool COLOR>
__device__ __forceinline__ void tile_forward_regs(const half8* __restrict__ wl, int lane, int g, const float4& e0, const float4& e1,
                                                  float dx, float dy, float dz, TileFwd& t) {
    tile_forward_frags<COLOR>([&](int id) -> const half8& { return wl[id * 64 + lane]; }, g, e0, e1, dx, dy, dz, t);
}

template <int THREADS, int N_FRAGS>
__device__ __forceinline__ void load_wpack(const half_t* __restrict__ wpack, half8* __restrict__ wl) {
    const uint4* src = reinterpret_cast<const uint4*>(wpack);
    uint4* dst = reinterpret_cast<uint4*>(wl);
    constexpr int PER = (N_FRAGS * 64 + THREADS - 1) / THREADS;
    uint4 v[PER];
#pragma unroll
    for (int i = 0; i < PER; ++i) {
// ... 205 lines not shown
#ifdef NGP_MLP_DIAG
        unsigned long long t_prev = __builtin_readcyclecounter();
        __builtin_amdgcn_s_waitcnt(0);
        MLP_T(0);
#endif
        tile_forward_regs<true>(wl, lane, g, in.e0, in.e1, in.dx, in.dy, in.dz, t);
        MLP_T(1);
        if (g == 0) {
#pragma unroll
            for (int r = 0; r < 3; ++r) {
                const float y = (float)t.rgb[r];
                dz5[r] = (half_t)(in.drgb(r) * ((1.0f - y) * y));
            }
        }
        {
            const half8 b_dz5 = cat_h4(dz5, hzero);
#pragma unroll
            for (int mt = 0; mt < 4; ++mt) dz4[mt] = mask_h4(NGP_MFMA(wfrag(wl, B_W5T + mt, lane), b_dz5, zero), t.a4[mt]);
            __builtin_amdgcn_sched_barrier(0);
            const half8 b40 = cat_h4(dz4[0], dz4[1]), b41 = cat_h4(dz4[2], dz4[3]);
#pragma unroll
            for (int mt = 0; mt < 4; ++mt) {
                floatx4 d = NGP_MFMA(wfrag(wl, B_W4T + 2 * mt, lane), b40, zero);
                d = NGP_MFMA(wfrag(wl, B_W4T + 2 * mt + 1, lane), b41, d);
                dz3[mt] = mask_h4(d, t.a3[mt]);
                __builtin_amdgcn_sched_barrier(0);
            }
            floatx4 dh = NGP_MFMA(wfrag(wl, B_W3T + 0, lane), cat_h4(dz3[0], dz3[1]), zero);
            dh = NGP_MFMA(wfrag(wl, B_W3T + 1, lane), cat_h4(dz3[2], dz3[3]), dh);
            dz2 = to_h4(dh);
            if (g == 0) {
                const float h0 = (float)t.h[0];
                const half_t gs = (half_t)(in.dsig * fast_exp(fminf(fmaxf(h0, -15.0f), 15.0f)));
                dz2[0] = (half_t)((float)dz2[0] + (float)gs);
            }
            __builtin_amdgcn_sched_barrier(0);
            const half8 b_dz2 = cat_h4(dz2, hzero);
#pragma unroll
            for (int mt = 0; mt < 4; ++mt) dz1[mt] = mask_h4(NGP_MFMA(wfrag(wl, B_W2T + mt, lane), b_dz2, zero), t.a1[mt]);
            __builtin_amdgcn_sched_barrier(0);
            const half8 b10 = cat_h4(dz1[0], dz1[1]), b11 = cat_h4(dz1[2], dz1[3]);
#pragma unroll
            for (int mt = 0; mt < 2; ++mt) {
                floatx4 d = NGP_MFMA(wfrag(wl, B_W1T + 2 * mt, lane), b10, zero);
                d = NGP_MFMA(wfrag(wl, B_W1T + 2 * mt + 1, lane), b11, d);
                bad_denc |= !(isfinite(d[0]) && isfinite(d[1]) && isfinite(d[2]) && isfinite(d[3]));
                if (smp < S) {
                    float* dp = pairs ? d_enc + ((size_t)(4 * mt + g) * plane + smp) * 4 : d_enc + (size_t)smp * 32 + 16 * mt + 4 * g;
                    *reinterpret_cast<float4*>(dp) = make_float4(d[0], d[1], d[2], d[3]);
                }
                __builtin_amdgcn_sched_barrier(0);
            }
        }

        MLP_T(2);
        bwd_request(raw, enc, dirs, dsigmas, drgbs, src_next, g, pairs, plane);
        img_store(img, A_DZ5, lofs, dz5);
#pragma unroll
        for (int mt = 0; mt < 4; ++mt) {
            img_store(img, A_DZ4 + mt, lofs, dz4[mt]);
            img_store(img, A_A4 + mt, lofs, t.a4[mt]);
            img_store(img, A_A3 + mt, lofs, t.a3[mt]);
        }
        __syncthreads();
        if (lo8) {
#pragma unroll 3
            for (int k = 0; k < BG; ++k) {
                const half_t* Ik = Iall + k * IMG_HALFS;
                const half8 a = img_load_tr(Ik, A_DZ4 + mtL, g, n);
                accA0 = NGP_MFMA(a, img_load_tr(Ik, A_A3 + 2 * ntL, g, n), accA0);
                accA1 = NGP_MFMA(a, img_load_tr(Ik, A_A3 + 2 * ntL + 1, g, n), accA1);
            }
        } else {
#pragma unroll 3
            for (int k = 0; k < BG; ++k) {
                const half_t* Ik = Iall + k * IMG_HALFS;
                accC = NGP_MFMA(img_load_tr(Ik, A_DZ5, g, n), img_load_tr(Ik, A_A4 + v4, g, n), accC);
            }
        }
        __syncthreads();
        MLP_T(3);
        img_store(img, B_DZ2, lofs, dz2);
        img_store(img, B_IN3, lofs, __builtin_shufflevector(t.b_in3, t.b_in3, 0, 1, 2, 3));
        img_store(img, B_IN3 + 1, lofs, __builtin_shufflevector(t.b_in3, t.b_in3, 4, 5, 6, 7));
#pragma unroll
        for (int mt = 0; mt < 4; ++mt) {
            img_store(img, B_DZ3 + mt, lofs, dz3[mt]);
            img_store(img, B_A1 + mt, lofs, t.a1[mt]);
        }
        __syncthreads();
        if (lo8) {
#pragma unroll 3
            for (int k = 0; k < BG; ++k) {
                const half_t* Ik = Iall + k * IMG_HALFS;
                accB = NGP_MFMA(img_load_tr(Ik, B_DZ3 + mtL, g, n), img_load_tr(Ik, B_IN3 + ntL, g, n), accB);
            }
        } else {
#pragma unroll 3
            for (int k = 0; k < BG; ++k) {
                const half_t* Ik = Iall + k * IMG_HALFS;
                accB = NGP_MFMA(img_load_tr(Ik, B_DZ2, g, n), img_load_tr(Ik, B_A1 + v4, g, n), accB);
            }
        }
        __syncthreads();
        MLP_T(4);
#pragma unroll
        for (int mt = 0; mt < 4; ++mt) img_store(img, C_DZ1 + mt, lofs, dz1[mt]);
        {
            const int te = C_ENC + (g >> 1), sw = n >> 2, gi = 2 * (g & 1);
            img_store(img, te, lrow + 4 * (gi ^ sw), __builtin_shufflevector(t.b_enc, t.b_enc, 0, 1, 2, 3));
            img_store(img, te, lrow + 4 * ((gi + 1) ^ sw), __builtin_shufflevector(t.b_enc, t.b_enc, 4, 5, 6, 7));
        }
        __syncthreads();
        if (lo8) {
#pragma unroll 3
            for (int k = 0; k < BG; ++k) {
                const half_t* Ik = Iall + k * IMG_HALFS;
                accC = NGP_MFMA(img_load_tr(Ik, C_DZ1 + mtL, g, n), img_load_tr(Ik, C_ENC + ntL, g, n), accC);
            }
        }
        __syncthreads();
        MLP_T(5);
    }

    if (!dW && !parts) { if (found_inf && bad_denc) *found_inf = 1; return; }
    bool bad = false;
    float* slab = parts ? parts + (size_t)blockIdx.x * N_W : nullptr;
    auto leave = [&](int w, float v) {
        if (slab) slab[w] = v;
        else if (v != 0.0f) unsafeAtomicAdd(dW + w, v);
    };
#pragma unroll
    for (int r = 0; r < 4; ++r) {
        const int o = 16 * mtL + 4 * g + r, o2 = 4 * g + r;
        const float a0 = accA0[r], a1 = accA1[r], b = accB[r], c = accC[r];
        if (lo8) {
            leave(OFF_W4 + o * 64 + 32 * ntL + n, a0);
            leave(OFF_W4 + o * 64 + 32 * ntL + 16 + n, a1);
            leave(OFF_W3 + o * 32 + 16 * ntL + n, b);
            leave(OFF_W1 + o * 32 + enc_feat(pairs, (16 * ntL + n) >> 3, n & 7), c);
        } else {
            leave(OFF_W2 + o2 * 64 + 16 * v4 + n, b);
            if (o2 < 3) leave(OFF_W5 + o2 * 64 + 16 * v4 + n, c);
        }
        bad |= !isfinite(a0) || !isfinite(a1) || !isfinite(b) || !isfinite(c);
    }
    if (found_inf && (bad || bad_denc)) *found_inf = 1;
}

#ifdef NGP_MLP_BWD_REG
#include "../../profiles/microbench/mlp_bwd_reg_kernel.inc"
#endif

}

using namespace ngp;

extern "C" {

#ifdef NGP_MLP_DIAG
int ngp_mlp_debug_read(unsigned long long* host128, int reset) {
    if (hipMemcpyFromSymbol(host128, HIP_SYMBOL(ngp_mlp_dbg), sizeof(ngp_mlp_dbg)) != hipSuccess) return -1;
    if (reset) { unsigned long long z[16 * 8] = {}; if (hipMemcpyToSymbol(HIP_SYMBOL(ngp_mlp_dbg), z, sizeof(z)) != hipSuccess) return -1; }
    return 0;
}
#endif

int ngp_mlp_wpack_halfs(void) { return N_ALL_FRAGS * 64 * 8; }

int ngp_mlp_pack(const float* W1, const float* W2, const float* W3, const float* W4, const float* W5, int enc_pairs, uint16_t* wpack,
                 void* stream) {
    const int total = N_ALL_FRAGS * 64 * 8;
    hipLaunchKernelGGL(mlp_pack_kernel, dim3((total + 255) / 256), dim3(256), 0, (hipStream_t)stream, W1, W2, W3, W4, W5, enc_pairs,
                       (half_t*)wpack);
    NGP_LAUNCH_CHECK();
    return 0;
}

int ngp_adam_mlp_pack(float* p, float* g, float* m, float* v, const float* state_f, const int32_t* state_i, float beta1, float beta2,
                      float eps, int enc_pairs, uint16_t* wpack, void* stream) {
    hipLaunchKernelGGL(adam_mlp_pack_kernel, dim3(1), dim3(1024), 0, (hipStream_t)stream, p, g, m, v, state_f, state_i, beta1, beta2,
                       eps, enc_pairs, (half_t*)wpack);
    NGP_LAUNCH_CHECK();
    return 0;
}

#define NGP_ADAM_ALL(SH, G16)                                                                                                     \
    hipLaunchKernelGGL((adam_all_kernel<SH, G16>), grid, block, 0, (hipStream_t)stream, (float4*)table, table_g, (float4*)table_m,    \
                       (float4*)table_v, n4, (uint2*)table_16, mlp, mlp_g, mlp_m, mlp_v, state_f, state_i, beta1, beta2, eps,         \
                       enc_pairs, (half_t*)wpack)

int ngp_adam_all_ex(float* table, void* table_g, int grad_is_f16, float* table_m, float* table_v, long long n, uint16_t* table_16,
                    int copy_kind, float* mlp, float* mlp_g, float* mlp_m, float* mlp_v, const float* state_f, const int32_t* state_i,
                    float beta1, float beta2, float eps, int enc_pairs, uint16_t* wpack, void* stream) {
    if (n <= 0 || n % 4 != 0) return -1;
    if ((copy_kind != 0) != (table_16 != nullptr) || copy_kind < 0 || copy_kind > 2) return -1;
    const long n4 = (long)(n / 4);
    long blocks = (n4 + 1023) / 1024;
    if (blocks > 256L * 4) blocks = 256L * 4;
    const dim3 grid((unsigned)blocks + 1), block(1024);
    if (grad_is_f16) {
        if (copy_kind == 2) NGP_ADAM_ALL(2, true); else if (copy_kind == 1) NGP_ADAM_ALL(1, true); else NGP_ADAM_ALL(0, true);
    } else {
        if (copy_kind == 2) NGP_ADAM_ALL(2, false); else if (copy_kind == 1) NGP_ADAM_ALL(1, false); else NGP_ADAM_ALL(0, false);
    }
    NGP_LAUNCH_CHECK();
    return 0;
}
#undef NGP_ADAM_ALL

int ngp_adam_all(float* table, float* table_g, float* table_m, float* table_v, long long n, uint16_t* table_bf16, float* mlp,
                 float* mlp_g, float* mlp_m, float* mlp_v, const float* state_f, const int32_t* state_i, float beta1, float beta2,
                 float eps, int enc_pairs, uint16_t* wpack, void* stream) {
    return ngp_adam_all_ex(table, table_g, 0, table_m, table_v, n, table_bf16, table_bf16 ? 1 : 0, mlp, mlp_g, mlp_m, mlp_v, state_f,
                           state_i, beta1, beta2, eps, enc_pairs, wpack, stream);
}

static inline int mlp_grid(int S) {
    static const int cap = [] { const char* e = ngp_experiment("mlp_fwd_blocks"); const int v = e ? atoi(e) : 0; return v > 0 ? v : 768; }();
    const int iters = (S + 31) / 32;
    int blocks = (iters + 3) / 4;
    if (blocks > cap) blocks = cap;
    return blocks < 1 ? 1 : blocks;
}

int ngp_mlp_fwd_ex(const float* enc, const float* dirs, const uint16_t* wpack, int n_max, const int32_t* n_dev, int enc_pairs,
                   float* sigmas, uint16_t* rgbs, void* stream) {
    if (n_max <= 0) return 0;
#define NGP_FWD(C, P, D, R)                                                                                          \
    hipLaunchKernelGGL((mlp_fwd_kernel<C, P>), dim3(mlp_grid(n_max)), dim3(256), 0, (hipStream_t)stream, enc, (const float*)(D), \
                       (const half_t*)wpack, n_max, n_dev, sigmas, (half_t*)(R))
    if (dirs && rgbs) { if (enc_pairs) NGP_FWD(true, true, dirs, rgbs); else NGP_FWD(true, false, dirs, rgbs); }
    else { if (enc_pairs) NGP_FWD(false, true, nullptr, nullptr); else NGP_FWD(false, false, nullptr, nullptr); }
#undef NGP_FWD
    NGP_LAUNCH_CHECK();
    return 0;
}

int ngp_mlp_fwd_list(const float* enc, const float* dirs, const uint16_t* wpack, int n_max, const int32_t* n_list, const int32_t* list,
                     int enc_pairs, float* sigmas, uint16_t* rgbs, void* stream) {
    if (n_max <= 0) return 0;
    if (!n_list || !list || !dirs || !rgbs) return -1;
    if (enc_pairs) hipLaunchKernelGGL((mlp_fwd_kernel<true, true, true>), dim3(mlp_grid(n_max)), dim3(256), 0, (hipStream_t)stream, enc, dirs,
                                      (const half_t*)wpack, n_max, n_list, sigmas, (half_t*)rgbs, list);
    else hipLaunchKernelGGL((mlp_fwd_kernel<true, false, true>), dim3(mlp_grid(n_max)), dim3(256), 0, (hipStream_t)stream, enc, dirs,
                            (const half_t*)wpack, n_max, n_list, sigmas, (half_t*)rgbs, list);
    NGP_LAUNCH_CHECK();
    return 0;
}

int ngp_mlp_fwd(const float* enc, const float* dirs, const uint16_t* wpack, int n, float* sigmas, uint16_t* rgbs, void* stream) {
    return ngp_mlp_fwd_ex(enc, dirs, wpack, n, nullptr, 0, sigmas, rgbs, stream);
}

static int mlp_bwd_launch(const float* enc, const float* dirs, const uint16_t* wpack, const float* dsigmas, const uint16_t* drgbs,
                          int n_max, const int32_t* n_dev, const int32_t* live_idx, int enc_pairs, float* d_enc, float* dW,
                          float* parts, int32_t* found_inf, void* stream) {
    int blocks;
#ifdef NGP_MLP_BWD_REG
    const char* form = ngp_experiment("mlp_bwd");
    if (form && form[0] == 'r') {
        if ((long long)n_max * 128 > 0xffffffffLL) return -1;
        blocks = ((n_max + 31) / 32 + RW - 1) / RW;
        if (blocks > 256) blocks = 256;
        if (blocks < 1) blocks = 1;
#define NGP_BWD_REG(P, L)                                                                                                        \
    hipLaunchKernelGGL((mlp_bwd_reg_kernel<P, L>), dim3(blocks), dim3(64 * RW), 0, (hipStream_t)stream, enc, dirs, (const half_t*)wpack, \
                       dsigmas, (const half_t*)drgbs, n_max, n_dev, live_idx, d_enc, dW, parts, found_inf)
        if (enc_pairs) { if (live_idx) NGP_BWD_REG(true, true); else NGP_BWD_REG(true, false); }
        else { if (live_idx) NGP_BWD_REG(false, true); else NGP_BWD_REG(false, false); }
#undef NGP_BWD_REG
        NGP_LAUNCH_CHECK();
        return blocks;
    }
#endif
    blocks = ((n_max + 31) / 32 + BG - 1) / BG;
    if (blocks > 256) blocks = 256;
    if (blocks < 1) blocks = 1;
    hipLaunchKernelGGL(mlp_bwd_kernel, dim3(blocks), dim3(64 * BW), 0, (hipStream_t)stream, enc, dirs, (const half_t*)wpack, dsigmas,
                       (const half_t*)drgbs, n_max, n_dev, live_idx, enc_pairs, d_enc, dW, parts, found_inf);
    NGP_LAUNCH_CHECK();
    return blocks;
}

int ngp_mlp_bwd_live(const float* enc, const float* dirs, const uint16_t* wpack, const float* dsigmas, const uint16_t* drgbs,
                     int n_max, const int32_t* n_dev, const int32_t* live_idx, int enc_pairs, float* d_enc, float* dW,
                     int32_t* found_inf, void* stream) {
    if (n_max <= 0) return 0;
    const int rc = mlp_bwd_launch(enc, dirs, wpack, dsigmas, drgbs, n_max, n_dev, live_idx, enc_pairs, d_enc, dW, nullptr, found_inf,
                                  stream);
    return rc < 0 ? rc : 0;
}

int ngp_mlp_dw_parts_max(void) { return 256; }

int ngp_mlp_bwd_live_parts(const float* enc, const float* dirs, const uint16_t* wpack, const float* dsigmas, const uint16_t* drgbs,
                           int n_max, const int32_t* n_dev, const int32_t* live_idx, int enc_pairs, float* d_enc, float* dW_parts,
                           int32_t* found_inf, void* stream) {
    if (n_max <= 0) return 0;
    if (!dW_parts) return -1;
    return mlp_bwd_launch(enc, dirs, wpack, dsigmas, drgbs, n_max, n_dev, live_idx, enc_pairs, d_enc, nullptr, dW_parts, found_inf,
                          stream);
}

__global__ void __launch_bounds__(NGP_MLP_REDUCE_THREADS) mlp_dw_reduce_kernel(const float* __restrict__ parts, int n_parts, float* __restrict__ dW) {
    mlp_dw_reduce_block(parts, n_parts, dW, blockIdx.x);
}

int ngp_mlp_dw_reduce(const float* dW_parts, int n_parts, float* dW, void* stream) {
    if (n_parts <= 0) return 0;
    hipLaunchKernelGGL(mlp_dw_reduce_kernel, dim3(NGP_MLP_REDUCE_BLOCKS), dim3(NGP_MLP_REDUCE_THREADS), 0, (hipStream_t)stream, dW_parts, n_parts, dW);
    NGP_LAUNCH_CHECK();
    return 0;
}

int ngp_mlp_bwd_ex(const float* enc, const float* dirs, const uint16_t* wpack, const float* dsigmas, const uint16_t* drgbs,
                   int n_max, const int32_t* n_dev, int enc_pairs, float* d_enc, float* dW, int32_t* found_inf, void* stream) {
    return ngp_mlp_bwd_live(enc, dirs, wpack, dsigmas, drgbs, n_max, n_dev, nullptr, enc_pairs, d_enc, dW, found_inf, stream);
}

int ngp_mlp_bwd(const float* enc, const float* dirs, const uint16_t* wpack, const float* dsigmas, const uint16_t* drgbs, int n,
                float* d_enc, float* dW, void* stream) {
    return ngp_mlp_bwd_ex(enc, dirs, wpack, dsigmas, drgbs, n, nullptr, 0, d_enc, dW, nullptr, stream);
}

}
```

taichi-nerfs_amd/csrc/ngp_device.h:

```cpp
#pragma once
#include <hip/hip_runtime.h>
#include <hip/hip_fp16.h>
#include <stdint.h>
#include "../../include/ngp_hip.h"
#include "../../include/ngp_hip_experimental.h"
#include <stdlib.h>
#include <string.h>

static inline const char* ngp_experiment(const char* key) {
    const char* e = getenv("NGP_EXPERIMENT");
    if (!e || !key) return nullptr;
    static thread_local char buf[64];
    const size_t kl = strlen(key);
    while (*e) {
        while (*e == ';' || *e == ' ') ++e;
        const char* end = strchr(e, ';');
        const size_t len = end ? (size_t)(end - e) : strlen(e);
        if (len > kl && strncmp(e, key, kl) == 0 && e[kl] == '=') {
            size_t vl = len - kl - 1;
            if (vl >= sizeof(buf)) vl = sizeof(buf) - 1;
            memcpy(buf, e + kl + 1, vl);
            buf[vl] = 0;
            return buf;
        }
        e += len;
    }
    return nullptr;
}


#define NGP_WAVE 64

#if defined(__HIP_DEVICE_COMPILE__) && !defined(__gfx950__)
#error "libngp_hip is written for gfx950 (MI355X / CDNA4): build with --offload-arch=gfx950"
#endif

#define NGP_LAUNCH_CHECK()                                   \
    do {                                                     \
        hipError_t e__ = hipGetLastError();                  \
        if (e__ != hipSuccess) return -(int)e__;             \
    } while (0)

namespace ngp {

__device__ __forceinline__ uint32_t f2u_bits(float x) { return __float_as_uint(x); }
__device__ __forceinline__ float u2f_bits(uint32_t u) { return __uint_as_float(u); }

__device__ __forceinline__ uint32_t f2u_sat(float v) {
    uint32_t r;
    asm("v_cvt_u32_f32 %0, %1" : "=v"(r) : "v"(v));
    return r;
}

__device__ __forceinline__ uint32_t f16_bits_rn(float v) {
    uint32_t r;
    asm("v_cvt_f16_f32 %0, %1" : "=v"(r) : "v"(v));
    return r & 0xffffu;
}
__device__ __forceinline__ float f16_round(float v) {
    float r;
    asm("v_cvt_f16_f32 %0, %1\n\tv_cvt_f32_f16 %0, %0" : "=v"(r) : "v"(v));
    return r;
}

template <int G>
__device__ __forceinline__ float4 sh16_quad(float x, float y, float z) {
    static_assert(G >= 0 && G < 4, "SH16 has four quads");
    const float xy = x * y, xz = x * z, yz = y * z, x2 = x * x, y2 = y * y, z2 = z * z;
    if constexpr (G == 0)
        return make_float4(0.28209479177387814f, -0.48860251190291987f * y, 0.48860251190291987f * z, -0.48860251190291987f * x);
    else if constexpr (G == 1)
        return make_float4(1.0925484305920792f * xy, -1.0925484305920792f * yz, 0.94617469575755997f * z2 - 0.31539156525251999f,
                           -1.0925484305920792f * xz);
    else if constexpr (G == 2)
        return make_float4(0.54627421529603959f * x2 - 0.54627421529603959f * y2, 0.59004358992664352f * y * (-3.0f * x2 + y2),
                           2.8906114426405538f * xy * z, 0.45704579946446572f * y * (1.0f - 5.0f * z2));
    else
        return make_float4(0.3731763325901154f * z * (5.0f * z2 - 3.0f), 0.45704579946446572f * x * (1.0f - 5.0f * z2),
                           1.4453057213202769f * z * (x2 - y2), 0.59004358992664352f * x * (-x2 + 3.0f * y2));
}

__device__ __forceinline__ float calc_dt(float t, float esf, float dt_min, float dt_max) {
    return fminf(dt_max, fmaxf(dt_min, t * esf));
}

__device__ __forceinline__ int frexp_bit(float x) {
    int exponent = 0;
    if (x != 0.0f) {
        uint32_t bits = f2u_bits(x);
        exponent = (int)((bits & 0x7f800000u) >> 23) - 127;
        float frac = u2f_bits((bits & 0x7fffffu) | 0x3f800000u);
        if (frac > 1.0f) exponent += 1;
    }
    return exponent;
}

__device__ __forceinline__ uint32_t expand_bits(uint32_t v) {
    v = (v * 0x00010001u) & 0xFF0000FFu;
    v = (v * 0x00000101u) & 0x0F00F00Fu;
    v = (v * 0x00000011u) & 0xC30C30C3u;
    v = (v * 0x00000005u) & 0x49249249u;
    return v;
}
__device__ __forceinline__ uint32_t morton3d(uint32_t x, uint32_t y, uint32_t z) {
    return expand_bits(x) | (expand_bits(y) << 1) | (expand_bits(z) << 2);
}
__device__ __forceinline__ int32_t morton3d_invert1(uint32_t x) {
    x = x & 0x49249249u;
    x = (x | (x >> 2)) & 0xc30c30c3u;
    x = (x | (x >> 4)) & 0x0f00f00fu;
    x = (x | (x >> 8)) & 0xff0000ffu;
    x = (x | (x >> 16)) & 0x0000ffffu;
    return (int32_t)x;
}

__device__ __forceinline__ float fsign(float x) { return (float)((x > 0.0f) - (x < 0.0f)); }

__device__ __forceinline__ int lane_id() { return (int)(threadIdx.x & (NGP_WAVE - 1)); }

__device__ __forceinline__ float wave_sum(float v) {
#pragma unroll
    for (int d = 32; d >= 1; d >>= 1) v += __shfl_xor(v, d, NGP_WAVE);
    return v;
}
__device__ __forceinline__ int wave_sum_i(int v) {
#pragma unroll
    for (int d = 32; d >= 1; d >>= 1) v += __shfl_xor(v, d, NGP_WAVE);
    return v;
}
__device__ __forceinline__ float wave_scan_mul(float v, int lane) {
#pragma unroll
    for (int d = 1; d < NGP_WAVE; d <<= 1) {
        float o = __shfl_up(v, d, NGP_WAVE);
        if (lane >= d) v *= o;
    }
    return v;
}
__device__ __forceinline__ float wave_scan_add(float v, int lane) {
#pragma unroll
    for (int d = 1; d < NGP_WAVE; d <<= 1) {
        float o = __shfl_up(v, d, NGP_WAVE);
        if (lane >= d) v += o;
    }
    return v;
}
__device__ __forceinline__ int wave_scan_add_i(int v, int lane) {
#pragma unroll
    for (int d = 1; d < NGP_WAVE; d <<= 1) {
        int o = __shfl_up(v, d, NGP_WAVE);
        if (lane >= d) v += o;
    }
    return v;
}

enum { SF_LOSS_SCALE = 0, SF_INV_SCALE = 1, SF_LR = 2, SF_BC1 = 3, SF_BC2_SQRT = 4, SF_LOSS = 5, SF_LOSS_ACC = 6 };
__host__ __device__ __forceinline__ float rng_uniform(unsigned long long seed, unsigned int index) {
    unsigned long long z = seed + ((unsigned long long)index + 1ull) * 0x9E3779B97F4A7C15ull;
    z = (z ^ (z >> 30)) * 0xBF58476D1CE4E5B9ull;
    z = (z ^ (z >> 27)) * 0x94D049BB133111EBull;
    z ^= z >> 31;
    return (float)(unsigned int)(z >> 40) * (1.0f / 16777216.0f);
}

constexpr int NGP_MLP_NW = 9408;
constexpr int NGP_MLP_REDUCE_BLOCKS = (NGP_MLP_NW + 63) / 64;
constexpr int NGP_MLP_REDUCE_THREADS = 1024;
__device__ __forceinline__ void mlp_dw_reduce_block(const float* __restrict__ parts, int n_parts, float* __restrict__ dW, int block) {
    __shared__ float partial[15][64];
    const int lane = threadIdx.x & 63, w = block * 64 + lane, q = threadIdx.x >> 6;
    float v[16];
#pragma unroll
    for (int k = 0; k < 16; ++k) {
        const int p = q + 16 * k;
        v[k] = (w < NGP_MLP_NW && p < n_parts) ? parts[(size_t)p * NGP_MLP_NW + w] : 0.0f;
    }
    float s = 0.0f;
    for (int p = q + 256; p < n_parts; p += 16) s += (w < NGP_MLP_NW) ? parts[(size_t)p * NGP_MLP_NW + w] : 0.0f;
#pragma unroll
    for (int k = 0; k < 16; k += 4) s += (v[k] + v[k + 1]) + (v[k + 2] + v[k + 3]);
    if (q) partial[q - 1][lane] = s;
    __syncthreads();
    if (q == 0 && w < NGP_MLP_NW) {
#pragma unroll
        for (int k = 0; k < 15; ++k) s += partial[k][lane];
        dW[w] += s;
    }
}

enum { SI_ITER = 0, SI_OPT_STEP = 1, SI_GROWTH = 2, SI_FOUND_INF = 3, SI_SKIP = 4, SI_SKIPPED_TOTAL = 5 };

__device__ __forceinline__ void train_prologue_thread(float* __restrict__ sf, int32_t* __restrict__ si, float lr0, float eta_min, int t_max,
                                                      float beta1, float beta2, float growth, float backoff, int growth_interval) {
    const int iter = si[SI_ITER];
    const int found = si[SI_FOUND_INF];
    const float scale = sf[SF_LOSS_SCALE];
    sf[SF_INV_SCALE] = 1.0f / scale;
    si[SI_SKIP] = found ? 1 : 0;
    const float c = cosf(3.14159265358979323846f * (float)(iter < t_max ? iter : t_max) / (float)t_max);
    sf[SF_LR] = eta_min + (lr0 - eta_min) * 0.5f * (1.0f + c);
    if (!found) {
        const int step = si[SI_OPT_STEP] + 1;
        si[SI_OPT_STEP] = step;
        sf[SF_BC1] = 1.0f - powf(beta1, (float)step);
        sf[SF_BC2_SQRT] = sqrtf(1.0f - powf(beta2, (float)step));
        int g = si[SI_GROWTH] + 1;
        if (g >= growth_interval) { sf[SF_LOSS_SCALE] = scale * growth; g = 0; }
        si[SI_GROWTH] = g;
    } else {
        sf[SF_LOSS_SCALE] = scale * backoff;
        si[SI_GROWTH] = 0;
        si[SI_SKIPPED_TOTAL] += 1;
    }
    si[SI_FOUND_INF] = 0;
    si[SI_ITER] = iter + 1;
}

__device__ __forceinline__ uint32_t f32_to_bf16_bits(float f) {
    uint32_t u = __float_as_uint(f);
    if ((u & 0x7fffffffu) > 0x7f800000u) return (u >> 16) | 0x40u;
    return (u + 0x7fffu + ((u >> 16) & 1u)) >> 16;
}

__device__ __forceinline__ uint32_t f32_to_f16_bits(float f) { return (uint32_t)__half_as_ushort(__float2half_rn(f)); }

struct AdamConsts {
    float inv_scale, step_size , bc2_sqrt, beta1, beta2, eps;
};
__device__ __forceinline__ AdamConsts adam_consts(const float* __restrict__ sf, float beta1, float beta2, float eps) {
    return {sf[SF_INV_SCALE], sf[SF_LR] / sf[SF_BC1], sf[SF_BC2_SQRT], beta1, beta2, eps};
}
__device__ __forceinline__ void adam_update(float& p, float& m, float& v, float g, const AdamConsts& c) {
    const float gr = g * c.inv_scale;
    m = m + (gr - m) * (1.0f - c.beta1);
    v = v * c.beta2 + gr * gr * (1.0f - c.beta2);
    const float denom = sqrtf(v) / c.bc2_sqrt + c.eps;
    p = p - c.step_size * (m / denom);
}

template <int SHADOW, bool GRAD16 = false>
__device__ __forceinline__ void adam_table_pass(float4* __restrict__ p, void* __restrict__ gv, float4* __restrict__ m,
                                                float4* __restrict__ v, long n4, const float* __restrict__ sf,
                                                const int32_t* __restrict__ si, float beta1, float beta2, float eps,
                                                uint2* __restrict__ shadow, long block, long n_blocks) {
    const bool skip = si[SI_SKIP] != 0;
    const AdamConsts ac = adam_consts(sf, beta1, beta2, eps);
    const float4 zero = make_float4(0.f, 0.f, 0.f, 0.f);
    float4* g32 = reinterpret_cast<float4*>(gv);
    uint2* g16 = reinterpret_cast<uint2*>(gv);
    for (long i = block * blockDim.x + threadIdx.x; i < n4; i += n_blocks * blockDim.x) {
        float4 gi;
        if constexpr (GRAD16) {
            const uint2 r = g16[i];
            const float2 a = __half22float2(*reinterpret_cast<const __half2*>(&r.x)), b = __half22float2(*reinterpret_cast<const __half2*>(&r.y));
            gi = make_float4(a.x, a.y, b.x, b.y);
        } else {
            gi = g32[i];
        }
        const bool g_any = !(gi.x == 0.f && gi.y == 0.f && gi.z == 0.f && gi.w == 0.f);
        if (skip) {
            if (g_any) { if constexpr (GRAD16) g16[i] = make_uint2(0u, 0u); else g32[i] = zero; }
            continue;
        }
        float4 mi = m[i], vi = v[i];
        if (!g_any && mi.x == 0.f && mi.y == 0.f && mi.z == 0.f && mi.w == 0.f && vi.x == 0.f && vi.y == 0.f && vi.z == 0.f && vi.w == 0.f)
            continue;
        float4 pi = p[i];
        adam_update(pi.x, mi.x, vi.x, gi.x, ac); adam_update(pi.y, mi.y, vi.y, gi.y, ac);
        adam_update(pi.z, mi.z, vi.z, gi.z, ac); adam_update(pi.w, mi.w, vi.w, gi.w, ac);
        p[i] = pi; m[i] = mi; v[i] = vi;
        if (g_any) { if constexpr (GRAD16) g16[i] = make_uint2(0u, 0u); else g32[i] = zero; }
        if constexpr (SHADOW == 1)
            shadow[i] = make_uint2(f32_to_bf16_bits(pi.x) | (f32_to_bf16_bits(pi.y) << 16),
                                   f32_to_bf16_bits(pi.z) | (f32_to_bf16_bits(pi.w) << 16));
        if constexpr (SHADOW == 2)
            shadow[i] = make_uint2(f32_to_f16_bits(pi.x) | (f32_to_f16_bits(pi.y) << 16),
                                   f32_to_f16_bits(pi.z) | (f32_to_f16_bits(pi.w) << 16));
    }
}

}
```

taichi-nerfs_amd/ngp_hip/experiment.py:

```python
import os

KEYS = {
    "flush_adam": "0: the table's optimizer as its own launch (rounds 1-4) instead of inside the scatter-add's flush",
    "live_backward": "0: backward over every marched sample instead of the live ones",
    "march_fused": "0: the count / scan / write chain instead of the one-launch march",
    "march_rng": "torch: jitter from torch.rand instead of the march kernel's counter-based generator",
    "prefetch_host_wait": "1: the HOST waits for the prefetched march where it was issued a step earlier (no cross-queue wait packet on the main stream; default: the stream-side wait)",
    "prefetch_at": "0 / 1 / 2 / 2.5 / 2.75 / 3 / 4: where in the step the next batch's march goes on the side stream (unset: adaptive)",
    "side_priority": "low / default: stream priority of that march (unset: adaptive)",
    "march_shape": "'waves,idle_lds_bytes': launch shape of that march (unset: adaptive)",
    "chunked_fwd": "1 / 0: shade in chunks of 64 / 64 / 128 / ... samples per live ray (unset: on for multi-cascade scenes)",
    "bwd_concentrated": "1 / 0: the scatter-add's concentrated-scene task plan (unset: on for multi-cascade scenes)",
    "mlp_dw": "atomic: round 3's float-atomic weight gradients instead of per-block slabs",
    "mlp_dw_reduce": "prologue: the slab sum in the prologue launch instead of the head of the scatter-add launch",
    "svox_trilinear": "1: VoxelGrid(use_trilinear=None) interpolates the eight surrounding grid points instead of reading the nearest (how the reference's train.py, which has no flag for it, reaches the lookup)",
    "comm_overlap": "1: one scatter-add launch + async reduce-scatter / Adam / all-gather per level group",
    "comm_groups": "first level of each group in launch order (default '8,0')",
    "comm_scatter_blocks": "workgroup cap of the later group launches (default 240)",
    "comm_stub": "1: every collective replaced by its local part (bench.py: what of comm_ms is exposed)",
    "bwd_rep_target": "[C] tasks a replicated level of the scatter-add gets (48)",
    "bwd_merge_res": "[C] run pre-summing on levels up to this resolution (128)",
    "bwd_dense_min_rep": "[C] sample ranges per dense slice, at least (8)",
    "bwd_merge_chunks": "[C] run-pre-summing levels: at least this many super-chunks per task (32; 0: round 5's slice-count rule alone)",
    "bwd_hashed_rep_res": "[C] concentrated plan: hashed levels up to this resolution get replicas (256)",
    "bwd_hashed_rep": "[C] ... this many (3)",
    "bwd_merge_hashed": "[C] concentrated plan: run pre-summing on those levels too (0)",
    "bwd_knobs_dynamic": "[C] re-read the bwd_* knobs on every call (one process A/Bs them on the same inputs)",
    "bwd_levels": "[C] -DNGP_BWD_DIAG builds only: level mask (wrong results by construction)",
    "bwd_diag": "[C] -DNGP_BWD_DIAG builds only: 1 no LDS adds, 2 no gathers, 4 no accumulate, 8 one gather per hit",
    "bwd_blocks": "[C] -DNGP_BWD_DIAG builds only: fewer persistent workgroups",
    "prep_batch": "[C] 3 / 6 / 12: LDS-form levels per fence in the scatter-add's prepass (1)",
    "hash_fwd_v1": "[C] 1: the round-1..3 loop of the forward hash gather",
    "hash_fwd_tiles": "[C] tile cap of the forward hash gather's persistent grid (768)",
    "hash_fwd_free_levels": "[C] -DNGP_HASH_FWD_DIAG builds only: levels whose gathers all read one line",
    "march_group": "[C] 16 / 32 / 64 lanes per ray of the march's count pass (32)",
    "mlp_fwd_blocks": "[C] persistent grid of the MLP forward (768)",
    "mlp_bwd": "[C] reg: round 4's register-resident MLP backward (-DNGP_MLP_BWD_REG builds only)",
}


def parse(text=None):
    text = os.environ.get("NGP_EXPERIMENT", "") if text is None else text
    out = {}
    for item in text.split(";"):
        item = item.strip()
        if not item:
            continue
        key, sep, value = item.partition("=")
        key = key.strip()
        if not sep or key not in KEYS:
            raise ValueError("NGP_EXPERIMENT: %r is not 'key=value' with a key of ngp_hip.experiment.KEYS" % item)
        out[key] = value.strip()
    return out


def get(key, default=None):
    if key not in KEYS:
        raise KeyError(key)
    return parse().get(key, default)


def has(key):
    return get(key) is not None
```

taichi-nerfs_amd/ngp_hip/lib.py:

```python
import ctypes
import glob
import os
import shutil
import subprocess

from . import cabi

_HERE = os.path.dirname(os.path.abspath(__file__))
PKG_ROOT = os.path.dirname(_HERE)
CSRC = os.path.join(PKG_ROOT, "csrc")
INCLUDE = os.path.join(os.path.dirname(PKG_ROOT), "include")
LIB_PATH = os.path.join(CSRC, "libngp_hip.so")
SOURCES = ["march.hip", "hash_grid.hip", "hash_bwd_lds.hip", "composite.hip", "sh_grid.hip", "mlp.hip", "optim.hip", "distortion.hip", "occupancy.hip", "rays.hip",
           "render.hip", "exchange.hip", "triplane.hip", "voxel_grid.hip", "deploy.hip", "hash_grad_input.hip", "hash_grad_input2.hip", "mesh.hip",
           "ray_grad.hip", "surface.hip", "resample.hip", "sdf_trace.hip", "mesh_sdf.hip", "mesh_raycast.hip", "mesh_winding.hip",
           "mesh_components.hip"]
HIPCC_FLAGS = ["--offload-arch=gfx950", "-O3", "-std=c++17", "-ffp-contract=off", "-fPIC", "-shared"]
FLAGS_STAMP = LIB_PATH + ".flags"
ABI_HEADERS = [os.path.join(INCLUDE, "ngp_hip.h"), os.path.join(INCLUDE, "ngp_hip_experimental.h")]


def _read_headers():
    out = []
    for path in ABI_HEADERS:
        if not os.path.exists(path):
            raise RuntimeError("%s is missing: libngp_hip.so cannot be bound without the header that declares it. "
                               "There is no CPU fallback." % path)
        with open(path) as f:
            out.append(cabi.parse(f.read(), out[0].defines if out else None))
    return out


_ABI, _ABI_EXPERIMENTAL = _read_headers()
NGP_MAX_LEVELS = _ABI.defines["NGP_MAX_LEVELS"]
ABI_VERSION = _ABI.defines["NGP_ABI_VERSION"]
BWD_PLAN_DETERMINISTIC, BWD_PLAN_CONCENTRATED = _ABI.defines["NGP_BWD_PLAN_DETERMINISTIC"], _ABI.defines["NGP_BWD_PLAN_CONCENTRATED"]


class HashLevels(ctypes.Structure):
    _fields_ = _ABI.structs["ngp_hash_levels"]

    def with_plan(self, bits):
        bits = int(bits)
        if bits == self.bwd_plan:
            return self
        cache = self.__dict__.setdefault("_plans", {})
        lv = cache.get(bits)
        if lv is None:
            lv = HashLevels()
            ctypes.memmove(ctypes.byref(lv), ctypes.byref(self), ctypes.sizeof(HashLevels))
            lv.bwd_plan = bits
            cache[bits] = lv
        return lv


class TriPlaneLevels(ctypes.Structure):
    _fields_ = _ABI.structs["ngp_triplane_levels"]


class RenderArgs(ctypes.Structure):
    _fields_ = _ABI.structs["ngp_render_args"]


def _sources():
    return [os.path.join(CSRC, s) for s in SOURCES if os.path.exists(os.path.join(CSRC, s))]


def _flags():
    return HIPCC_FLAGS + os.environ.get("NGP_HIPCC_EXTRA", "").split()


def needs_build():
    if not os.path.exists(LIB_PATH):
        return True
    t = os.path.getmtime(LIB_PATH)
    deps = _sources() + glob.glob(os.path.join(CSRC, "*.h")) + ABI_HEADERS
    if any(os.path.getmtime(d) > t for d in deps if os.path.exists(d)):
        return True
    if os.path.exists(FLAGS_STAMP):
        return open(FLAGS_STAMP).read().split() != _flags()
    return bool(os.environ.get("NGP_HIPCC_EXTRA", "").split())


def build(force=False, verbose=False):
    if not force and not needs_build():
        return LIB_PATH
    hipcc = shutil.which("hipcc") or "/opt/rocm/bin/hipcc"
    if not os.path.exists(hipcc):
        raise RuntimeError("hipcc not found: cannot build libngp_hip.so")
    tmp = LIB_PATH + ".tmp.%d" % os.getpid()
    cmd = [hipcc] + _flags() + ["-o", tmp] + _sources()
    if verbose:
        print(" ".join(cmd))
    res = subprocess.run(cmd, capture_output=True, text=True)
    if res.returncode != 0:
        raise RuntimeError("hipcc failed:\n" + res.stdout + res.stderr)
    os.replace(tmp, LIB_PATH)
    with open(FLAGS_STAMP, "w") as f:
        f.write(" ".join(_flags()))
    return LIB_PATH


_BOUND = cabi.bind({**_ABI.functions, **_ABI_EXPERIMENTAL.functions},
                   {"ngp_hash_levels": ctypes.POINTER(HashLevels), "ngp_triplane_levels": ctypes.POINTER(TriPlaneLevels),
                    "ngp_render_args": ctypes.c_void_p})
SIGNATURES = {name: argtypes for name, (_, argtypes) in _BOUND.items()}
RESTYPES = {name: restype for name, (restype, _) in _BOUND.items()}
EXPERIMENTAL = set(_ABI_EXPERIMENTAL.functions)
_lib = None


def load():
    global _lib
    if _lib is not None:
        return _lib
    import torch
    if not os.path.exists(LIB_PATH):
        raise RuntimeError(
            "libngp_hip.so is not built (%s). Run `python __graft_entry__.py` or "
            "`python -c 'import __graft_entry__ as g; g.build()'`. There is no CPU fallback." % LIB_PATH)
    lib = ctypes.CDLL(LIB_PATH, mode=ctypes.RTLD_GLOBAL)
    for name, argtypes in SIGNATURES.items():
        fn = getattr(lib, name)
        fn.argtypes = argtypes
        fn.restype = RESTYPES[name]
    if lib.ngp_abi_version() != ABI_VERSION:
        raise RuntimeError("%s reports ABI version %d, but include/ngp_hip.h declares %d: rebuild the library from this tree "
                           "(`python __graft_entry__.py`). There is no CPU fallback." % (LIB_PATH, lib.ngp_abi_version(), ABI_VERSION))
    _lib = lib
    return lib


def check(rc, what):
    if rc != 0:
        raise RuntimeError("%s failed with code %d (negated hipError_t, or -1 for bad arguments)" % (what, rc))
```

taichi-nerfs_amd/ngp_hip/trainer.py:

```python
import ctypes
import math
import os

import torch
import torch.distributed as dist

from . import experiment as _exp
from . import lib as _lib_mod
from .dist import all_reduce_avg
from .fused import RenderConfig, TrainArena, concentrated_scene
from .lib import check
from .ops import MLP_N_WEIGHTS, _ptr, _stream, launch_march_train, rng_uniform

_SF_LOSS_SCALE, _SF_LOSS = 0, 5
_SI_ITER, _SI_OPT_STEP, _SI_FOUND_INF, _SI_SKIPPED = 0, 1, 3, 5


class _PrefetchPoint:
    __slots__ = ("at", "action")

    def __init__(self):
        self.at, self.action = 0.0, None

    def arm(self, at, action):
        self.at, self.action = min(at, 4), action

    def reach(self, p):
        if self.action is not None and p >= self.at:
            action, self.action = self.action, None
            action()


class _Step:
    __slots__ = ("M", "A", "cfg", "st", "P", "n", "pf", "found", "vr_per_ray", "opacity", "depth", "rgb", "sq_err", "cnt", "live_idx",
                 "lvp", "ws")

    def __init__(self, M, A, cfg, st, P, n, pf, found, dev):
        self.M, self.A, self.cfg, self.st, self.P, self.n, self.pf, self.found = M, A, cfg, st, P, n, pf, found
        f32 = dict(device=dev, dtype=torch.float32)
        self.vr_per_ray = torch.empty(n, device=dev, dtype=torch.int32)
        self.opacity, self.depth, self.rgb = torch.empty(n, **f32), torch.empty(n, **f32), torch.empty(n, 3, **f32)
        self.sq_err = torch.empty(n, **f32)
        self.cnt = self.live_idx = self.lvp = self.ws = None

    def result(self):
        M = self.M
        return {"rm_samples": M.total, "vr_per_ray": self.vr_per_ray, "rgb": self.rgb, "opacity": self.opacity, "depth": self.depth,
                "rays_a": M.rays_a, "deltas": M.deltas, "ts": M.ts, "sq_err": self.sq_err}


class FusedTrainer:
    _MARCH_NARROW_MAX = 1_000_000

    @staticmethod
    def chunk_rounds(max_samples):
        rounds, b, l, pb = [], 0, 64, 0
        while b < max_samples:
            l = min(l, max_samples - b)
            rounds.append((b, l, pb))
            pb, b = b, b + l
            l = b
        return rounds

    def __init__(self, model, lr=1e-2, betas=(0.9, 0.999), eps=1e-15, max_steps=20000, eta_min=None, init_scale=2.0**19,
                 growth_factor=2.0, backoff_factor=0.5, growth_interval=2000, exp_step_factor=0.0, T_threshold=1e-4,
                 max_samples=1024, process_group=None, world_size=None, grad_comm_dtype=None,
                 distortion_loss_w=0.0, shard_optimizer=None, chunked_forward=None, exchange="rccl"):
        if not hasattr(model, "pos_encoder"):
            raise ValueError("FusedTrainer drives NGP's hash-grid encoder only; train a %s through the drop-in path "
                             "(modules.rendering.render + a torch optimizer, as the reference's train.py does)" % type(model).__name__)
        if getattr(model, "pos_encoder_type", "hash") != "hash":
            raise ValueError("FusedTrainer drives the hash-grid encoder only; train a %r model through the drop-in path "
                             "(modules.rendering.render + a torch optimizer, as the reference's train.py does)" % model.pos_encoder_type)
        if not model.use_fused_mlp:
            raise ValueError("FusedTrainer needs the default architecture (L=16, F=2 hash grid, 64-wide MLPs)")
        self.half = bool(model.half_opt)
        self.model = model
        self.L = _lib_mod.load()
        dev = model.pos_encoder.hash_table.device
        if dev.type != "cuda":
            raise RuntimeError("FusedTrainer needs the model on a GPU (libngp_hip has no CPU path)")
        self.dev = dev
        self.lr0, self.eta_min = float(lr), float(lr / 30 if eta_min is None else eta_min)
        self.t_max = int(max_steps)
        self.beta1, self.beta2, self.eps = float(betas[0]), float(betas[1]), float(eps)
        self.growth, self.backoff, self.growth_interval = float(growth_factor), float(backoff_factor), int(growth_interval)
        self.exp_step_factor, self.T_threshold, self.max_samples = float(exp_step_factor), float(T_threshold), int(max_samples)
        self.bg = 1.0 if exp_step_factor == 0 else 0.0
        self.distortion_loss_w = float(distortion_loss_w)
        self._init_options(model, exp_step_factor, max_samples, chunked_forward, process_group, world_size)
        self._init_buffers(model, dev, init_scale, grad_comm_dtype, shard_optimizer, process_group)
        self._init_prefetch(dev)
        self._init_table_copies(model, dev, exp_step_factor)
        self._init_exchange(model, dev, exchange)
        self.repack()

    def _init_options(self, model, exp_step_factor, max_samples, chunked_forward, process_group, world_size):
        ck = _exp.get("chunked_fwd")
        if chunked_forward is None and ck is not None:
            chunked_forward = ck == "1"
        if chunked_forward is None:
            chunked_forward = float(exp_step_factor) > 0 or int(model.cascades) > 1
        self.chunked = bool(chunked_forward) and not self.half and int(max_samples) % 64 == 0 and int(max_samples) >= 128
        self._chunk_rounds = self.chunk_rounds(int(max_samples)) if self.chunked else []
        self._chunk_counts = None
        self._chunk_T = {}
        self.live_backward = _exp.get("live_backward", "1") != "0"
        self.march_fused = _exp.get("march_fused", "1") != "0"
        self._march_rng = _exp.get("march_rng", "kernel") != "torch"
        self.hash_bwd = os.environ.get("NGP_HASH_BWD", "sliced")
        self.group = process_group
        self.world = world_size if world_size is not None else (dist.get_world_size(process_group) if dist.is_initialized() else 1)

    def _init_buffers(self, model, dev, init_scale, grad_comm_dtype, shard_optimizer, process_group):

        ws = list(model._mlp_weights())
        flat = torch.cat([w.detach().reshape(-1) for w in ws]).contiguous()
        assert flat.numel() == MLP_N_WEIGHTS
        off = 0
        for w in ws:
            n = w.numel()
            w.data = flat[off:off + n].view_as(w)
            off += n
        self.mlp_flat = flat
        f32 = dict(device=dev, dtype=torch.float32)
        nt = model.pos_encoder.hash_table.numel()
        assert nt % 8 == 0
        self.shard = bool(self.world > 1 if shard_optimizer is None else shard_optimizer)
        if self.shard and not dist.is_initialized():
            raise RuntimeError("the sharded optimizer needs an initialised torch.distributed process group")
        self.rank = dist.get_rank(process_group) if (self.shard or self.world > 1) and dist.is_initialized() else 0
        unit = 4 * self.world if self.shard else 4
        self.nt, self.nt_pad = nt, (nt + unit - 1) // unit * unit
        self.shard_len = self.nt_pad // self.world if self.shard else self.nt_pad
        hp = model.pos_encoder.hash_table
        store = torch.zeros(self.nt_pad, **f32)
        store[:nt].copy_(hp.detach().reshape(-1))
        hp.data = store[:nt].view_as(hp)
        self.table_store = store
        self.table = store[:nt]
        if self.half:
            self.table_grad_store = torch.zeros(self.nt_pad, device=dev, dtype=torch.float16)
            self.table_grad = self.table_grad_store[:nt]
            self.grad_flat = torch.zeros(MLP_N_WEIGHTS + 4, **f32)
            self.mlp_grad = self.grad_flat[:MLP_N_WEIGHTS]
            self._flag_f = self.grad_flat[MLP_N_WEIGHTS:MLP_N_WEIGHTS + 1]
            self.small_bucket = self.grad_flat
        else:
            self.grad_flat = torch.zeros(self.nt_pad + MLP_N_WEIGHTS + 4, **f32)
            self.table_grad_store = self.grad_flat[:self.nt_pad]
            self.table_grad = self.grad_flat[:nt]
            self.mlp_grad = self.grad_flat[self.nt_pad:self.nt_pad + MLP_N_WEIGHTS]
            self._flag_f = self.grad_flat[self.nt_pad + MLP_N_WEIGHTS:self.nt_pad + MLP_N_WEIGHTS + 1]
            self.small_bucket = self.grad_flat[self.nt_pad:]
        self.shard_grad = (torch.zeros(self.shard_len, device=dev, dtype=self.table_grad_store.dtype) if self.shard else None)
        if grad_comm_dtype is None:
            enc_dt = getattr(model.pos_encoder, "table_dtype", torch.float32)
            grad_comm_dtype = torch.bfloat16 if (enc_dt == torch.bfloat16 and not self.half) else torch.float32
        self.grad_comm_dtype = grad_comm_dtype
        if grad_comm_dtype not in (torch.float32, torch.bfloat16):
            raise ValueError("grad_comm_dtype must be torch.float32 or torch.bfloat16")
        self._comm = self._comm_shard = None
        if grad_comm_dtype != torch.float32 and self.world > 1 and not self.half:
            if self.shard:
                self._comm = torch.empty(self.nt_pad, device=dev, dtype=grad_comm_dtype)
                self._comm_shard = torch.empty(self.shard_len, device=dev, dtype=grad_comm_dtype)
            else:
                self._comm = torch.empty_like(self.grad_flat, dtype=grad_comm_dtype)
        self.mlp_parts = torch.empty(self.L.ngp_mlp_dw_parts_max() * MLP_N_WEIGHTS, **f32)
        self._dw_atomic = _exp.get("mlp_dw", "") == "atomic"
        self.table_m, self.table_v = torch.zeros(self.nt_pad, **f32), torch.zeros(self.nt_pad, **f32)
        self.mlp_m, self.mlp_v = torch.zeros(MLP_N_WEIGHTS, **f32), torch.zeros(MLP_N_WEIGHTS, **f32)
        self.state_f = torch.zeros(8, **f32)
        self.state_i = torch.zeros(8, device=dev, dtype=torch.int32)
        self.state_f[_SF_LOSS_SCALE] = float(init_scale)
        self._live_pair = torch.zeros(2, device=dev, dtype=torch.int32)
        self._graph = None
        self._launch_incomplete = False
        self._grads_only = False
        self.stats = {}
        self._sets = {}
        self._cur = 0

    def _init_prefetch(self, dev):
        self._side = torch.cuda.Stream(device=dev)
        self._one_gpu_flush = (self.world == 1 and not self.half and _exp.get("flush_adam", "1") != "0"
                               and self.hash_bwd == "sliced")
        pinned = any(_exp.has(k) for k in ("prefetch_at", "march_shape", "side_priority"))
        self._adaptive_prefetch = self._one_gpu_flush and not pinned
        self._host_wait_ok = _exp.get("prefetch_host_wait", "0") == "1"
        self._side_prio = None
        self._side_default = self._side
        self._side_low = None
        if self._adaptive_prefetch or _exp.get("side_priority", "low") == "low":
            h, lo, hi = ctypes.c_void_p(), ctypes.c_int(), ctypes.c_int()
            check(self.L.ngp_stream_create_low_priority(ctypes.byref(h), ctypes.byref(lo), ctypes.byref(hi)), "ngp_stream_create_low_priority")
            self._side_low = torch.cuda.ExternalStream(h.value, device=dev)
            self._side_prio = (lo.value, hi.value)
            self._side = self._side_low
        self._hook_at = 3
        self._marched_host = None
        if self._adaptive_prefetch:
            h = ctypes.c_void_p()
            check(self.L.ngp_host_alloc(ctypes.byref(h), 64), "ngp_host_alloc")
            self._marched_host = h
            ctypes.c_int32.from_address(h.value).value = 1 << 30
        self._ev_start = self._DevEvent(self.L)
        self.prefetch_hits = 0
        self._prefetch_at = float(_exp.get("prefetch_at", "3" if self.world == 1 else "4"))
        shape = _exp.get("march_shape", "")
        self._march_shape = tuple(int(x) for x in shape.split(",")) if shape and shape != "16,0" else None
        self.sync_occupancy = True
        self.comm_probe = None

    def _init_table_copies(self, model, dev, exp_step_factor):
        nt = self.nt
        lvs = model.pos_encoder.levels_struct
        self.enc_pairs = 1 if (lvs.n_levels == 16 and lvs.n_features == 2) else 0
        self.wpack = torch.empty(self.L.ngp_mlp_wpack_halfs(), device=dev, dtype=torch.float16)
        enc = model.pos_encoder
        self.table_bf16 = self.table_f16 = self.copy16_store = None
        if getattr(enc, "table_dtype", torch.float32) == torch.bfloat16:
            self.copy16_store = torch.zeros(self.nt_pad, device=dev, dtype=torch.bfloat16)
            enc._bf16, enc._bf16_ver = self.copy16_store[:nt].view(enc.hash_table.shape), None
            self.table_bf16 = enc.table_bf16()
        elif self.half:
            self.copy16_store = torch.zeros(self.nt_pad, device=dev, dtype=torch.float16)
            enc._f16, enc._f16_ver = self.copy16_store[:nt].view(enc.hash_table.shape), None
            self.table_f16 = enc.table_f16().view(-1)
        self._kind16 = 2 if self.half else (1 if self.table_bf16 is not None else 0)
        self._copy16 = self.copy16_store[:nt] if self.copy16_store is not None else None
        self._fwd_table = self.table_f16 if self.half else (self.table_bf16 if self.table_bf16 is not None else self.table)
        self._master_stale = False
        self._flush_adam = _exp.get("flush_adam", "1") != "0"
        self._fold_prologue = True
        self._adam_prefix = {}
        self.deterministic = False
        self._concentrated = concentrated_scene(exp_step_factor, model.cascades)
        self.set_deterministic(os.environ.get("NGP_DETERMINISTIC", "0") == "1")

    def _init_exchange(self, model, dev, exchange):
        lvs = model.pos_encoder.levels_struct
        self._comm_stub = _exp.get("comm_stub", "0") == "1"
        self._p2p = None
        if exchange not in ("rccl", "p2p"):
            raise ValueError("exchange must be 'rccl' or 'p2p'")
        if exchange == "p2p" and self.world > 1:
            if not self.shard or self.half or self._comm is not None:
                raise ValueError("exchange='p2p' needs the sharded optimizer, the fp32 encoder and fp32 gradient transport")
            from .p2p import PeerExchange
            stores = {"table": self.table_store}
            if self.copy16_store is not None:
                stores["copy16"] = self.copy16_store
            self._p2p = PeerExchange(self.rank, self.world, dev, self.shard_len, stores, group=self.group)
        self._pending_comm = []
        self._groups = None
        if (self.shard and _exp.get("comm_overlap", "0") == "1" and not self.half and self.hash_bwd == "sliced"
                and lvs.n_features == 2):
            self._groups = self._make_groups(lvs, _exp.get("comm_groups", "8,0"))

    def set_deterministic(self, on):
        if getattr(self, "_graph", None) is not None and bool(on) != self.deterministic:
            raise RuntimeError("set_deterministic() after capture(): the captured graphs hold the previous mode's launches; "
                               "set the mode before capture()")
        self.deterministic = bool(on)
        self.model._ngp_deterministic = self.deterministic
        return self

    def _scatter_mode(self):
        return ((_lib_mod.BWD_PLAN_DETERMINISTIC if self.deterministic else 0)
                | (_lib_mod.BWD_PLAN_CONCENTRATED if self._concentrated else 0))

    def repack(self):
        ws = self.model._mlp_weights()
        self.sync_master()
        if self.table_bf16 is not None:
            self.model.pos_encoder._bf16_ver = None
            assert self.model.pos_encoder.table_bf16() is self.table_bf16
        if self.half:
            self.model.pos_encoder._f16_ver = None
            assert self.model.pos_encoder.table_f16().data_ptr() == self.table_f16.data_ptr()
        check(self.L.ngp_mlp_pack(*[_ptr(w) for w in ws], self.enc_pairs, _ptr(self.wpack), _stream()), "ngp_mlp_pack")

    class _DevEvent:

        def __init__(self, L):
            self.L = L
            h = ctypes.c_void_p()
            check(L.ngp_event_create(ctypes.byref(h)), "ngp_event_create")
            self.h = h

        def record(self, stream):
            check(self.L.ngp_event_record(self.h, ctypes.c_void_p(stream.cuda_stream)), "ngp_event_record")

        def wait(self, stream):
            check(self.L.ngp_stream_wait_event(ctypes.c_void_p(stream.cuda_stream), self.h), "ngp_stream_wait_event")

        def synchronize(self):
            check(self.L.ngp_event_synchronize(self.h), "ngp_event_synchronize")

        def __del__(self):
            try:
                self.L.ngp_event_destroy(self.h)
            except Exception:
                pass

    class _MarchSet:

        def __init__(self, dev, n, max_samples):
            cap = n * max_samples
            f32 = dict(device=dev, dtype=torch.float32)
            self.n, self.cap = n, cap
            self.stage = torch.empty(cap, 2, **f32)
            self.counts = torch.empty(n, device=dev, dtype=torch.int32)
            self.rays_a = torch.empty(n, 3, device=dev, dtype=torch.int32)
            self.total = torch.zeros(1, device=dev, dtype=torch.int32)
            self.ctr = torch.zeros(2, device=dev, dtype=torch.int32)
            self.hits_t = torch.empty(n, 2, **f32)
            self.xyzs, self.dirs = torch.empty(cap, 3, **f32), torch.empty(cap, 3, **f32)
            self.deltas, self.ts = torch.empty(cap, **f32), torch.empty(cap, **f32)
            self.ready = None
            self.issued_early = False
            self.src = None
            self.held = None

        def marched_for(self, src):
            k = self.src
            return (self.ready is not None and k is not None and src is not None and k[0] is src[0] and k[1] is src[1]
                    and k[2] == src[0]._version and k[3] == src[1]._version)


    @property
    def _live_total(self):
        par = 1 - self._cur
        return self._live_pair[par:par + 1]

    def _march_sets(self, n):
        key = n
        sets = self._sets.get(key)
        if sets is None:
            sets = self._sets[key] = [self._MarchSet(self.dev, n, self.max_samples) for _ in range(2)]
            for m_ in sets:
                m_.ev_ready = self._DevEvent(self.L)
            sets[0].index, sets[1].index = 0, 1
        return sets

    def _coarse_bits(self, cfg, A):
        coarse, stale = A.coarse_state(cfg)
        if stale:
            check(self.L.ngp_bitfield_coarsen(_ptr(cfg.bitfield), cfg.cascades, cfg.grid_size, _ptr(coarse), _stream()),
                  "ngp_bitfield_coarsen")
        return coarse

    def _march(self, M, rays_o, rays_d, cfg, A, coarse=None, noise=None, shape=None):
        n = rays_o.shape[0]
        if coarse is None:
            coarse = self._coarse_bits(cfg, A)
        ray_order = self.deterministic or not self.march_fused
        seed = 0
        if noise is None and (self.deterministic or (self.march_fused and self._march_rng)):
            seed = int(torch.randint(0, 2**62, (), dtype=torch.int64))
            if self.deterministic:
                noise = rng_uniform(seed, n, self.dev)
        elif noise is None:
            noise = torch.rand(n, device=self.dev, dtype=torch.float32)
        launch_march_train(self.L, M, rays_o, rays_d, None, cfg.bitfield, coarse, noise, seed, cfg.cascades, cfg.grid_size, cfg.scale,
                           cfg.exp_step_factor, cfg.max_samples, shape=shape if noise is None else None, ray_order=ray_order)

    def _launch(self, rays_o, rays_d, target, prefetch=None, src=None, src_next=None, noise=None):
        self.finish_comm()
        n = rays_o.shape[0]
        cfg = RenderConfig.cached(self.model, self.exp_step_factor, self.T_threshold, self.max_samples)
        A = TrainArena.get(self.dev, n, self.max_samples)
        sets = self._march_sets(n)
        M = sets[self._cur]
        hit = noise is None and M.marched_for(src)
        self.prefetch_hits += int(hit)
        if M.ready is not None:
            if self._host_wait_ok and M.issued_early and self._graph is None:
                M.ready.synchronize()
            else:
                M.ready.wait(torch.cuda.current_stream())
        if not hit:
            self._march(M, rays_o, rays_d, cfg, A, noise=noise)
        M.ready, M.src, M.held = None, None, None
        pf = _PrefetchPoint()
        if prefetch is not None and (prefetch[0].shape != rays_o.shape or prefetch[1].shape != rays_d.shape):
            raise ValueError("prefetch rays must have the shape of the current batch (the two march buffers are sized per batch size)")
        if prefetch is not None:
            nxt = sets[1 - self._cur]

            at, shape, side = self._prefetch_at, self._march_shape, self._side
            if self._adaptive_prefetch:
                marched = ctypes.c_int32.from_address(self._marched_host.value).value
                if marched <= self._MARCH_NARROW_MAX:
                    at, shape, side = 0, (4, 0), self._side_default
                else:
                    at, shape, side = 3, (4, 0), self._side_low
            self._hook_at = at

            def issue():
                start = self._ev_start
                start.record(torch.cuda.current_stream())
                with torch.cuda.stream(side):
                    start.wait(side)
                    if nxt.ready is not None:
                        nxt.ready.wait(side)
                    self._march(nxt, prefetch[0], prefetch[1], cfg, A, shape=shape)
                    nxt.ready = nxt.ev_ready
                    nxt.ready.record(side)
                    nxt.issued_early = at == 0
                    if self._marched_host is not None:
                        check(self.L.ngp_copy_to_host_async(self._marched_host, _ptr(nxt.total), 4, ctypes.c_void_p(side.cuda_stream)),
                              "ngp_copy_to_host_async")
                nxt.src = None if src_next is None else (src_next[0], src_next[1], src_next[0]._version, src_next[1]._version)
                nxt.held = prefetch
            pf.arm(at if self._graph is None else 0, issue)
            pf.reach(0)
        if self._launch_incomplete:
            self._live_pair.zero_()
            if self._chunk_counts is not None:
                self._chunk_counts.zero_()
        self._launch_incomplete = True
        cur, self._cur = self._cur, 1 - self._cur
# ... 5 lines not shown
            raise ValueError("graph mode was captured for %d rays per step" % self._graph_n)
        check(self.L.ngp_stage_batch(_ptr(target), _ptr(self._static_target), _ptr(None), _ptr(None), _ptr(None), _ptr(None), 3 * n,
                                     _stream()), "ngp_stage_batch")
        if cur not in self._graph:
            g = torch.cuda.CUDAGraph()
            with torch.cuda.graph(g):
                stats = self._shade(M, n, self._static_target, cfg, A, pf)
            self._graph[cur] = (g, stats)
        g, stats = self._graph[cur]
        g.replay()
        self._launch_incomplete = False
        return stats

    def _shade(self, M, n, target, cfg, A, pf):
        L, st = self.L, _stream()
        found = ctypes.c_void_p(self.state_i.data_ptr() + 4 * _SI_FOUND_INF)
        s = _Step(M, A, cfg, st, self.enc_pairs, n, pf, found, self.dev)
        if not (self.chunked and self._forward_chunked(s)):
            self._forward_all(s)
        self._composite_and_loss(s, target)
        det = self._scatter_mode()
        s.lvp = cfg.levels.with_plan(det)
        pf.reach(2.5)
        sliced = self._prepass(s)
        pf.reach(2.75)
        n_parts = self._mlp_backward(s)
        slabs_to = None
        if self.world == 1 and not self._grads_only and n_parts > 0 and self._groups is None:
            in_scatter = sliced and not self.half and _exp.get("mlp_dw_reduce", "scatter") == "scatter"
            slabs_to = "scatter" if in_scatter else "prologue"
        elif n_parts > 0:
            check(L.ngp_mlp_dw_reduce(_ptr(self.mlp_parts), n_parts, _ptr(self.mlp_grad), st), "ngp_mlp_dw_reduce")
        pf.reach(3)
        npre = -1
        if slabs_to == "scatter" and self._flush_adam:
            npre = self._adam_prefix.get(det)
            if npre is None:
                npre = int(L.ngp_hash_bwd_sliced_adam_prefix(ctypes.byref(s.lvp)))
                npre = self._adam_prefix[det] = npre if npre % 4 == 0 else -2
        if npre >= 0:
            self._tail_flush_adam(s, n_parts, npre)
        elif self._groups is not None and sliced and not self._grads_only:
            self._tail_overlapped(s)
        else:
            self._tail_plain(s, sliced, n_parts, slabs_to)
        return s.result()

    def _composite_and_loss(self, s, target):
        L, st, M, A, n = self.L, s.st, s.M, s.A, s.n
        par, distortion = M.index, self.distortion_loss_w > 0
        live_total, live_next = self._live_pair[par:par + 1], self._live_pair[1 - par:2 - par]
        fused_live = self.live_backward and not self.deterministic and not distortion
        if distortion:
            self._composite_with_distortion(s, target)
        else:
            lst = (A.live_idx, live_total, live_next) if fused_live else (None, None, None)
            check(L.ngp_composite_train_fused_live(_ptr(A.sigmas), _ptr(A.rgbs), 1, _ptr(M.deltas), _ptr(M.ts), _ptr(M.rays_a),
                                                   _ptr(target), self.bg, _ptr(self.state_f), s.cfg.T_threshold, n, _ptr(s.vr_per_ray),
                                                   _ptr(s.opacity), _ptr(s.depth), _ptr(s.rgb), _ptr(A.ws), _ptr(A.d_sigmas),
                                                   _ptr(A.d_rgbs), _ptr(s.sq_err), _ptr(lst[0]), _ptr(lst[1]), _ptr(lst[2]), st),
                  "ngp_composite_train_fused_live")
        if fused_live:
            pass
        elif not self.live_backward:
            live_next.zero_()
        elif self.deterministic:
            check(L.ngp_live_compact(_ptr(M.rays_a), _ptr(s.vr_per_ray), n, _ptr(A.live_off(n)), _ptr(A.live_idx), _ptr(live_total), st),
                  "ngp_live_compact")
            live_next.zero_()
        else:
            check(L.ngp_live_list(_ptr(M.rays_a), _ptr(s.vr_per_ray), n, _ptr(A.live_idx), _ptr(live_total), _ptr(live_next), st),
                  "ngp_live_list")
        s.live_idx, s.cnt = (A.live_idx, live_total) if self.live_backward else (None, M.total)

    def _prepass(self, s):
        if self.hash_bwd != "sliced":
            return False
        M, A, cfg = s.M, s.A, s.cfg
        s.ws = A.sliced_ws(cfg.levels)
        rc = self.L.ngp_hash_bwd_sliced_prep(_ptr(M.xyzs), ctypes.byref(s.lvp), A.cap, _ptr(s.cnt), _ptr(s.live_idx), 1, cfg.lo, cfg.hi,
                                             _ptr(s.ws), s.ws.numel(), s.st)
        if rc == -2:
            if self._groups is not None:
                raise RuntimeError("NGP_EXPERIMENT comm_overlap=1 needs the LDS-sliced scatter-add, which this level table does not fit "
                                   "(ngp_hash_bwd_sliced_prep returned -2); unset NGP_EXPERIMENT comm_overlap")
            self.hash_bwd = "atomic"
            return False
        check(rc, "ngp_hash_bwd_sliced_prep")
        return True

    def _mlp_backward(self, s):
        L, M, A = self.L, s.M, s.A
        head = (_ptr(A.enc), _ptr(M.dirs), _ptr(self.wpack), _ptr(A.d_sigmas), _ptr(A.d_rgbs), A.cap, _ptr(s.cnt), _ptr(s.live_idx),
                s.P, _ptr(A.d_enc))
        if self._dw_atomic:
            check(L.ngp_mlp_bwd_live(*head, _ptr(self.mlp_grad), s.found, s.st), "ngp_mlp_bwd_live")
            return 0
        n_parts = L.ngp_mlp_bwd_live_parts(*head, _ptr(self.mlp_parts), s.found, s.st)
        if n_parts <= 0:
            check(n_parts or -1, "ngp_mlp_bwd_live_parts")
        return n_parts

    def _tail_plain(self, s, sliced, n_parts, slabs_to):
        L, st, M, A, cfg, found = self.L, s.st, s.M, s.A, s.cfg, s.found
        if sliced:
            head = (_ptr(A.d_enc), ctypes.byref(s.lvp), A.cap, _ptr(s.cnt), s.P, _ptr(self.table_grad))
            if slabs_to == "scatter":
                check(L.ngp_hash_bwd_sliced_main_slabs(*head, 0, found, _ptr(s.ws), s.ws.numel(), _ptr(self.mlp_parts), n_parts,
                                                       _ptr(self.mlp_grad), st), "ngp_hash_bwd_sliced_main_slabs")
            else:
                name = "ngp_hash_bwd_sliced_main_f16" if self.half else "ngp_hash_bwd_sliced_main"
                check(getattr(L, name)(*head, found, _ptr(s.ws), s.ws.numel(), st), name)
        else:
            name = "ngp_hash_bwd_f16_live" if self.half else "ngp_hash_bwd_f32_live"
            check(getattr(L, name)(_ptr(M.xyzs), _ptr(A.d_enc), ctypes.byref(cfg.levels), A.cap, _ptr(s.cnt), _ptr(s.live_idx), 1,
                                   cfg.lo, cfg.hi, s.P, _ptr(self.table_grad), found, st), name)
        s.pf.reach(4)
        sharded = self.shard and not self._grads_only
        if sharded:
            self._exchange_sharded(found, st)
        else:
            if self.world > 1:
                self._all_reduce()
            if self.half:
                check(L.ngp_check_finite_f16(_ptr(self.table_grad), self.table_grad.numel(), found, st), "ngp_check_finite_f16")
        if self._grads_only:
            return
        self._prologue(st, n_parts if slabs_to == "prologue" else 0)
        if not sharded:
            self._adam(st, 0, self.nt, self.table_grad)
            return
        lo = self.rank * self.shard_len
        self._adam(st, lo, self.shard_len, self.shard_grad)
        if self.copy16_store is not None:
            self._all_gather(self.copy16_store, slice(lo, lo + self.shard_len))
            self._master_stale = True
        else:
            self._all_gather(self.table_store, slice(lo, lo + self.shard_len))

    def _prologue(self, st, n_parts=0):
        L, sf, si = self.L, self.state_f, self.state_i
        hyper = (self.lr0, self.eta_min, self.t_max, self.beta1, self.beta2, self.growth, self.backoff, self.growth_interval)
        if n_parts:
            check(L.ngp_train_prologue_reduce(_ptr(sf), _ptr(si), *hyper, _ptr(self.mlp_parts), n_parts, _ptr(self.mlp_grad), st),
                  "ngp_train_prologue_reduce")
        else:
            check(L.ngp_train_prologue(_ptr(sf), _ptr(si), *hyper, st), "ngp_train_prologue")

    def _adam(self, st, lo, n, grad, mlp=True):
        L = self.L
        quartet = [_ptr(t if mlp else None) for t in (self.mlp_flat, self.mlp_grad, self.mlp_m, self.mlp_v)]
        rest = (_ptr(self.state_f), _ptr(self.state_i), self.beta1, self.beta2, self.eps, self.enc_pairs, _ptr(self.wpack), st)
        if n == 0:
            check(L.ngp_adam_mlp_pack(*quartet, *rest), "ngp_adam_mlp_pack")
            return

        def at(t):
            return ctypes.c_void_p(t.data_ptr() + lo * t.element_size()) if t is not None else ctypes.c_void_p(0)
        check(L.ngp_adam_all_ex(at(self.table_store), _ptr(grad), int(self.half), at(self.table_m), at(self.table_v), n,
                                at(self.copy16_store), self._kind16, *quartet, *rest), "ngp_adam_all_ex")

    _GATHER = ("ngp_hash_fwd_f32_ex", "ngp_hash_fwd_bf16_ex", "ngp_hash_fwd_f16_ex")

    def _forward_all(self, s):
        L, M, A, cfg, st = self.L, s.M, s.A, s.cfg, s.st
        name = self._GATHER[self._kind16]
        check(getattr(L, name)(_ptr(M.xyzs), _ptr(self._fwd_table), ctypes.byref(cfg.levels), A.cap, _ptr(M.total), 1, cfg.lo, cfg.hi,
                               s.P, _ptr(A.enc), st), name)
        s.pf.reach(1)
        check(L.ngp_mlp_fwd_ex(_ptr(A.enc), _ptr(M.dirs), _ptr(self.wpack), A.cap, _ptr(M.total), s.P, _ptr(A.sigmas), _ptr(A.rgbs), st),
              "ngp_mlp_fwd_ex")
        s.pf.reach(2)

    def _forward_chunked(self, s):
        L, M, A, cfg, st, n, P = self.L, s.M, s.A, s.cfg, s.st, s.n, s.P
        R = len(self._chunk_rounds)
        T_state = self._chunk_state(n)
        par = M.index
        c_cur = self._chunk_counts.data_ptr() + 4 * R * par
        c_oth = self._chunk_counts.data_ptr() + 4 * R * (1 - par)
        lst = A.live_idx
        for r, (b, l, pb) in enumerate(self._chunk_rounds):
            cnt = ctypes.c_void_p(c_cur + 4 * r)
            check(L.ngp_chunk_schedule(_ptr(M.rays_a), _ptr(A.sigmas), _ptr(M.deltas), n, b, l, pb, 0.5 * cfg.T_threshold, _ptr(T_state),
                                       _ptr(lst), cnt, ctypes.c_void_p(c_oth + 4 * r), st), "ngp_chunk_schedule")
            rc = L.ngp_hash_fwd_list(_ptr(M.xyzs), _ptr(self._fwd_table), self._kind16, ctypes.byref(cfg.levels), A.cap, cnt, _ptr(lst), 1,
                                     cfg.lo, cfg.hi, P, _ptr(A.enc), st)
            if rc == -2 and r == 0:
                self._chunk_counts.zero_()
                self.chunked = False
                return False
            check(rc, "ngp_hash_fwd_list")
            if r == 0:
                s.pf.reach(1)
            check(L.ngp_mlp_fwd_list(_ptr(A.enc), _ptr(M.dirs), _ptr(self.wpack), A.cap, cnt, _ptr(lst), P, _ptr(A.sigmas),
                                     _ptr(A.rgbs), st), "ngp_mlp_fwd_list")
        s.pf.reach(2)
        return True

    def _chunk_state(self, n):
        if self._chunk_counts is None:
            self._chunk_counts = torch.zeros(2, len(self._chunk_rounds), device=self.dev, dtype=torch.int32)
        T_state = self._chunk_T.get(n)
        if T_state is None:
            T_state = self._chunk_T[n] = torch.empty(n, device=self.dev, dtype=torch.float32)
        return T_state

    def shaded_samples(self):
        if not self.chunked or self._chunk_counts is None:
            return None
        return int(self._chunk_counts[1 - self._cur].sum())

    def _tail_flush_adam(self, s, n_parts, npre):
        L, A, st, sf, si = self.L, s.A, s.st, self.state_f, self.state_i
        args = (_ptr(A.d_enc), ctypes.byref(s.lvp), A.cap, _ptr(s.cnt), s.P, _ptr(self.table_grad), _ptr(s.ws), s.ws.numel(),
                _ptr(self.mlp_parts), n_parts, _ptr(self.mlp_grad), _ptr(self.table), _ptr(self.table_m), _ptr(self.table_v),
                _ptr(self._copy16), _ptr(sf), _ptr(si))
        if self._fold_prologue:
            check(L.ngp_hash_bwd_sliced_main_adam_step(*args, self.lr0, self.eta_min, self.t_max, self.beta1, self.beta2, self.eps,
                                                       self.growth, self.backoff, self.growth_interval, st),
                  "ngp_hash_bwd_sliced_main_adam_step")
        else:
            self._prologue(st)
            check(L.ngp_hash_bwd_sliced_main_adam(*args, self.beta1, self.beta2, self.eps, st), "ngp_hash_bwd_sliced_main_adam")
        s.pf.reach(4)
        self._adam(st, 0, npre, self.table_grad)

    def _composite_with_distortion(self, s, target):
        L, st, sf = self.L, s.st, self.state_f
        A, M, cfg, n, vr_per_ray, opacity, depth, rgb = s.A, s.M, s.cfg, s.n, s.vr_per_ray, s.opacity, s.depth, s.rgb
        f32 = dict(device=self.dev, dtype=torch.float32)
        rays_a = M.rays_a
        check(L.ngp_composite_train_fwd(_ptr(A.sigmas), _ptr(A.rgbs), 1, _ptr(M.deltas), _ptr(M.ts), _ptr(rays_a), cfg.T_threshold,
                                        n, _ptr(vr_per_ray), _ptr(opacity), _ptr(depth), _ptr(rgb), _ptr(A.ws), st),
              "ngp_composite_train_fwd")
        dist_loss = torch.zeros(n, **f32)
        ws_inc, wts_inc, g_ws = A.scratch("ws_inc"), A.scratch("wts_inc"), A.scratch("g_ws")
        check(L.ngp_distortion_fwd(_ptr(A.ws), _ptr(M.deltas), _ptr(M.ts), _ptr(rays_a), n, _ptr(dist_loss), _ptr(ws_inc),
                                   _ptr(wts_inc), st), "ngp_distortion_fwd")
        g_dist = (sf[_SF_LOSS_SCALE] * (self.distortion_loss_w / n)).expand(n).contiguous()
        check(L.ngp_distortion_bwd(_ptr(g_dist), _ptr(A.ws), _ptr(M.deltas), _ptr(M.ts), _ptr(ws_inc), _ptr(wts_inc), _ptr(rays_a), n,
                                   _ptr(g_ws), st), "ngp_distortion_bwd")
        g_rgb, g_op, sq_err = torch.empty(n, 3, **f32), torch.empty(n, **f32), torch.empty(n, **f32)
        check(L.ngp_mse_loss_grad_rays(_ptr(rgb), _ptr(opacity), _ptr(target), self.bg, n, _ptr(sf), _ptr(g_rgb), _ptr(g_op), _ptr(sq_err), st),
              "ngp_mse_loss_grad_rays")
        check(L.ngp_composite_train_bwd(_ptr(g_op), _ptr(None), _ptr(g_rgb), _ptr(g_ws), _ptr(A.sigmas), _ptr(A.rgbs), 1, _ptr(M.deltas),
                                        _ptr(M.ts), _ptr(rays_a), _ptr(opacity), _ptr(depth), _ptr(rgb), _ptr(A.ws), cfg.T_threshold, n,
                                        _ptr(A.d_sigmas), _ptr(A.d_rgbs), st), "ngp_composite_train_bwd")
        self._dist_loss = dist_loss
        s.sq_err = sq_err

    def _make_groups(self, lvs, spec):
        from .dist import GroupedExchange, make_level_groups
        groups = make_level_groups([int(lvs.offset[l]) for l in range(int(lvs.n_levels))], int(lvs.n_features), self.nt_pad,
                                   self.world, self.rank, spec)
        if groups[0].hi <= groups[0].lo:
            raise ValueError("the first level group leaves rank %d without a chunk" % self.rank)
        self._gx = GroupedExchange(groups, self.rank, self.world, self.dev, group=self.group,
                                   comm_dtype=self._comm.dtype if self._comm is not None else None, timed=self._timed)
        return groups

    def _rs_async(self, g):
        self._gx.stub = self._comm_stub
        return self._gx.rs_async(g, self.table_grad_store)

    def _ag_async(self, g, store):
        self._gx.stub = self._comm_stub
        return self._gx.ag_async(g, store)

    def finish_comm(self):
        pend, self._pending_comm = self._pending_comm, []
        for fin in pend:
            fin()

    def _gather_groups(self, store):
        for g in self._groups:
            self._ag_async(g, store)()

    def _tail_overlapped(self, s):
        L, A, st = self.L, s.A, s.st
        max_blocks = int(_exp.get("comm_scatter_blocks", "240"))
        fins = []
        for k, g in enumerate(self._groups):
            check(L.ngp_hash_bwd_sliced_main_levels(_ptr(A.d_enc), ctypes.byref(s.lvp), A.cap, _ptr(s.cnt), s.P, _ptr(self.table_grad),
                                                    s.found, _ptr(s.ws), s.ws.numel(), g.mask, 0 if k == 0 else max_blocks, st),
                  "ngp_hash_bwd_sliced_main_levels")
            fins.append(self._rs_async(g))
        s.pf.reach(4)

        def small():
            self._timed("wait_all_reduce_mlp_grad_and_flag", self._rank_avg(self.small_bucket, async_op=True))
        self._carry_flag(small)
        self._prologue(st)
        back = self.copy16_store if self.copy16_store is not None else self.table_store
        for k, (g, fin) in enumerate(zip(self._groups, fins)):
            fin()
            if g.hi > g.lo:
                self._adam(st, g.lo, g.hi - g.lo, g.shard, mlp=k == 0)
            self._pending_comm.append(self._ag_async(g, back))
        if self.copy16_store is not None:
            self._master_stale = True

    def _rank_avg(self, t, async_op=False):
        if self._comm_stub:
            return (lambda: None) if async_op else None
        return all_reduce_avg(t, self.world, self.group, async_op)

    def _carry_flag(self, collective):
        flag_i = self.state_i[_SI_FOUND_INF:_SI_FOUND_INF + 1]
        self._flag_f.copy_(flag_i)
        collective()
        flag_i.copy_(self._flag_f != 0)
        self._flag_f.zero_()

    def _exchange_sharded(self, found, st):
        src = self.table_grad_store
        if self._comm is not None:
            self._comm.copy_(src)
            self._reduce_scatter(self._comm_shard, self._comm)
            self.shard_grad.copy_(self._comm_shard)
        else:
            self._reduce_scatter(self.shard_grad, src)
        src.zero_()
        if self.half:
            check(self.L.ngp_check_finite_f16(_ptr(self.shard_grad), self.shard_grad.numel(), found, st), "ngp_check_finite_f16")
        self._carry_flag(lambda: self._timed("all_reduce_mlp_grad_and_flag", lambda: self._rank_avg(self.small_bucket)))

    def _timed(self, name, fn):
        probe = self.comm_probe() if self.comm_probe is not None else None
        if not probe or not probe[0]:
            return fn()
        e0, e1 = torch.cuda.Event(enable_timing=True), torch.cuda.Event(enable_timing=True)
        e0.record()
        out = fn()
        e1.record()
        probe[1].append((name, e0, e1))
        return out

    def comm_bytes_per_step(self):
        if self.world <= 1:
            return {}
        small = self.small_bucket.numel() * self.small_bucket.element_size()
        if self.shard:
            g = self._comm if self._comm is not None else self.table_grad_store
            back = self.copy16_store if self.copy16_store is not None else self.table_store
            return {"reduce_scatter_table_grad": g.numel() * g.element_size(), "all_reduce_mlp_grad_and_flag": small,
                    "all_gather_table": back.numel() * back.element_size()}
        buf = self._comm if self._comm is not None else self.grad_flat
        out = {"all_reduce_flat_bucket": buf.numel() * buf.element_size()}
        if self.half:
            out["all_reduce_f16_table_grad"] = self.table_grad.numel() * 2
        return out

    def _reduce_scatter(self, out, inp):
        from .dist import reduce_scatter_avg
        if self._comm_stub:
            return out.copy_(inp[self.rank * out.numel():(self.rank + 1) * out.numel()])
        if self._p2p is not None and inp.dtype == torch.float32:
            return self._timed("p2p_reduce_scatter_table_grad", lambda: self._p2p.reduce_scatter_avg(out, inp))
        self._timed("reduce_scatter_table_grad", lambda: reduce_scatter_avg(out, inp, self.rank, self.world, self.group))

    def _all_gather(self, store, sl):
        from .dist import all_gather_shards
        if self._comm_stub:
            return store
        if self._p2p is not None:
            name = "table" if store is self.table_store else ("copy16" if store is self.copy16_store else None)
            if name is not None:
                return self._timed("p2p_all_gather_table", lambda: self._p2p.all_gather(name, sl))
        self._timed("all_gather_table", lambda: all_gather_shards(store, self.rank, self.shard_len, self.world, self.group))

    def sync_master(self):
        self.finish_comm()
        if self.shard and self._master_stale:
            if self._groups is not None:
                self._gather_groups(self.table_store)
            else:
                lo = self.rank * self.shard_len
                self._all_gather(self.table_store, slice(lo, lo + self.shard_len))
            self._master_stale = False

    def _all_reduce(self):
        def bucket():
            if self.half:
                all_reduce_avg(self.table_grad, self.world, self.group)
            buf = self.grad_flat
            if self._comm is not None and not self.shard:
                buf = self._comm
                buf.copy_(self.grad_flat)
            self._timed("all_reduce_flat_bucket", lambda: self._rank_avg(buf))
            if buf is not self.grad_flat:
                self.grad_flat.copy_(buf)
        self._carry_flag(bucket)

    def step(self, rays_o, rays_d, target, prefetch=None, noise=None):
        src, src_next = (rays_o, rays_d), None
        if prefetch is not None:
            src_next = (prefetch[0], prefetch[1])
            prefetch = (prefetch[0].contiguous().float(), prefetch[1].contiguous().float())
        self.stats = self._launch(rays_o.contiguous().float(), rays_d.contiguous().float(), target.contiguous().float(), prefetch,
                                  src, src_next, noise)
        if self._pending_comm and prefetch is None:
            self.finish_comm()
        return self.stats

    def compute_gradients(self, rays_o, rays_d, target, noise=None):
        if self._graph is not None:
            raise RuntimeError("not available after capture()")
        self._grads_only = True
        try:
            out = self._launch(rays_o.contiguous().float(), rays_d.contiguous().float(), target.contiguous().float(), noise=noise)
        finally:
            self._grads_only = False
        inv = 1.0 / self.state_f[_SF_LOSS_SCALE]
        out["table_grad"], out["mlp_grad"] = self.table_grad.float() * inv, self.mlp_grad * inv
        out["found_inf"] = self.state_i[_SI_FOUND_INF].clone()
        self.grad_flat.zero_()
        if self.half:
            self.table_grad.zero_()
        self.state_i[_SI_FOUND_INF] = 0
        return out

    def capture(self, n_rays):
        if self.world > 1:
            raise RuntimeError("graph capture is only wired for the single-GPU step")
        TrainArena.get(self.dev, n_rays, self.max_samples)
        self._march_sets(n_rays)
        if self.chunked:
            self._chunk_state(n_rays)
        self._static_target = torch.zeros(n_rays, 3, device=self.dev, dtype=torch.float32)
        self._graph = {}
        self._graph_n = n_rays
        return self._graph

    def update_density_grid(self, density_threshold, warmup=False, **kw):
        self.finish_comm()
        with torch.autocast(device_type="cuda", dtype=torch.float16):
            self.model.update_density_grid(density_threshold, warmup=warmup, **kw)
        if self.world > 1 and self.sync_occupancy:
            from .dist import broadcast_occupancy
            broadcast_occupancy(self.model, src=0, group=self.group)
        TrainArena.invalidate_coarse()
        for sets in self._sets.values():
            for M in sets:
                M.src = None

    def state_dict(self):
        self.sync_master()
        if self.shard and self._groups is not None:
            self._gather_groups(self.table_m)
            self._gather_groups(self.table_v)
        elif self.shard:
            lo = self.rank * self.shard_len
            sl = slice(lo, lo + self.shard_len)
            self._all_gather(self.table_m, sl)
            self._all_gather(self.table_v, sl)
        return {"table_m": self.table_m[:self.nt].clone(), "table_v": self.table_v[:self.nt].clone(), "mlp_m": self.mlp_m.clone(),
                "mlp_v": self.mlp_v.clone(), "state_f": self.state_f.clone(), "state_i": self.state_i.clone()}

    def load_state_dict(self, sd):
        for k in ("table_m", "table_v"):
            src, dst = sd[k], getattr(self, k)
            if src.numel() not in (self.nt, dst.numel()):
                raise ValueError("%s has %d elements; this trainer expects %d (or %d padded)" % (k, src.numel(), self.nt, dst.numel()))
            n = min(src.numel(), self.nt)
            dst[:n].copy_(src[:n])
            dst[self.nt:].zero_()
        for k in ("mlp_m", "mlp_v", "state_f", "state_i"):
            getattr(self, k).copy_(sd[k])
        self.grad_flat.zero_()
        if self.half:
            self.table_grad.zero_()
        if self.shard_grad is not None:
            self.shard_grad.zero_()
        TrainArena.invalidate_coarse()
        self._master_stale = False
        self.repack()

    def close(self):
        side, self._side, self._side_low = getattr(self, "_side_low", None), None, None
        host, self._marched_host = getattr(self, "_marched_host", None), None
        dflt, self._side_default = getattr(self, "_side_default", None), None
        if host is not None:
            try:
                for s_ in (side, dflt):
                    if s_ is not None:
                        s_.synchronize()
                self.L.ngp_host_free(host)
            except Exception:
                pass
        self._adaptive_prefetch = False
        if side is not None and getattr(self, "_side_prio", None) is not None:
            try:
                side.synchronize()
                self.L.ngp_stream_destroy(ctypes.c_void_p(side.cuda_stream))
            except Exception:
                pass
            self._side_prio = None

    def __del__(self):
        try:
            self.close()
        except Exception:
            pass

    def last_loss(self):
        se = self.stats.get("sq_err")
        if se is None and self.distortion_loss_w > 0 and self.stats:
            return float(self.state_f[_SF_LOSS].item())
        return float("nan") if se is None else float(se.sum().item()) / (3.0 * se.numel())

    def loss_scale(self):
        return float(self.state_f[_SF_LOSS_SCALE].item())

    def counters(self):
        s = self.state_i.tolist()
        return {"iter": s[_SI_ITER], "opt_steps": s[_SI_OPT_STEP], "skipped": s[_SI_SKIPPED]}

    def lr_at(self, it):
        return self.eta_min + (self.lr0 - self.eta_min) * 0.5 * (1 + math.cos(math.pi * min(it, self.t_max) / self.t_max))
```

Before: 17.83 million.

## Fuse MLP Adam step and fp16 repack into scatter-add head reduce

```diff
diff --git a/include/ngp_hip.h b/include/ngp_hip.h
--- a/include/ngp_hip.h
+++ b/include/ngp_hip.h
@@ -24,6 +24,7 @@
 
 #define NGP_BWD_PLAN_DETERMINISTIC 1u
 #define NGP_BWD_PLAN_CONCENTRATED  2u
+#define NGP_BWD_PLAN_MLP_STEP      4u
 
 int ngp_abi_version(void);
 
@@ -298,6 +299,8 @@
                     uint16_t* wpack, void* stream);
 int ngp_adam_mlp_pack(float* p, float* g, float* m, float* v, const float* state_f, const int32_t* state_i,
                       float beta1, float beta2, float eps, int enc_pairs, uint16_t* wpack, void* stream);
+int ngp_mlp_step_register(float* dW, float* p, float* m, float* v, uint16_t* wpack, int enc_pairs);
+int ngp_mlp_step_unregister(const float* dW);
 
 int ngp_morton3d(const int32_t* coords , int m, int32_t* indices, void* stream);
 int ngp_morton3d_invert(const int32_t* indices, int m, int32_t* coords , void* stream);
diff --git a/include/ngp_hip_experimental.h b/include/ngp_hip_experimental.h
--- a/include/ngp_hip_experimental.h
+++ b/include/ngp_hip_experimental.h
@@ -35,6 +35,8 @@
 int ngp_hash_bwd_sliced_plan(const ngp_hash_levels* lv, uint16_t* tasks, int max_tasks, uint16_t* xoff , uint16_t* xlen ,
                              uint8_t* nrep , uint32_t* merge_mask, uint32_t* single_mask);
 
+int ngp_mlp_pack_slot_map(int enc_pairs, int32_t* src_of_slot, uint32_t* slots_of_weight );
+
 int ngp_march_train_count(const float* rays_o, const float* rays_d, const float* hits_t,
                           const uint8_t* density_bitfield, const float* noise,
                           int cascades, int grid_size, float scale, float exp_step_factor,
diff --git a/taichi-nerfs_amd/csrc/hash_bwd_lds.hip b/taichi-nerfs_amd/csrc/hash_bwd_lds.hip
--- a/taichi-nerfs_amd/csrc/hash_bwd_lds.hip
+++ b/taichi-nerfs_amd/csrc/hash_bwd_lds.hip
@@ -528,6 +528,7 @@
     const float* parts;
     int n_parts;
     float* dW;
+    const MlpStep* step;
 };
 
 struct FlushAdam {
@@ -577,7 +578,8 @@
     __shared__ uint32_t s_claim;
     if (mlp.parts) {
         for (int b = blockIdx.x; b < NGP_MLP_REDUCE_BLOCKS; b += gridDim.x) {
-            mlp_dw_reduce_block(mlp.parts, mlp.n_parts, mlp.dW, b);
+            if (ADAM != 0 && mlp.step) mlp_dw_reduce_block<true>(mlp.parts, mlp.n_parts, mlp.dW, b, mlp.step, ad.sf, ad.si, ad.beta1, ad.beta2, ad.eps);
+            else mlp_dw_reduce_block(mlp.parts, mlp.n_parts, mlp.dW, b);
             __syncthreads();
         }
     }
@@ -869,9 +871,11 @@
     BwdPlan plan;
     uint32_t single_mask = 0u;
 };
-static const BwdPlan* get_plan(const ngp_hash_levels& lv, uint32_t& single_mask, uint32_t level_mask = 0xffffffffu, int max_blocks = 0) {
+static const BwdPlan* get_plan(const ngp_hash_levels& lv_in, uint32_t& single_mask, uint32_t level_mask = 0xffffffffu, int max_blocks = 0) {
     static thread_local PlanCache cache[8];
     static thread_local int victim = 0;
+    ngp_hash_levels lv = lv_in;
+    lv.bwd_plan &= ~NGP_BWD_PLAN_MLP_STEP;
     Knobs K = knobs(lv.bwd_plan);
     K.level_mask &= level_mask;
     if (max_blocks > 0 && (K.blocks <= 0 || max_blocks < K.blocks)) K.blocks = max_blocks;
@@ -966,7 +970,7 @@
 
 static int sliced_main(bool half, const float* dout, const ngp_hash_levels* lv, int n_max, const int32_t* n_dev, int enc_pairs,
                        void* dtable, int32_t* found_inf, const void* workspace, long long workspace_bytes, void* stream,
-                       uint32_t level_mask = 0xffffffffu, int max_blocks = 0, MlpSlabs mlp = MlpSlabs{nullptr, 0, nullptr},
+                       uint32_t level_mask = 0xffffffffu, int max_blocks = 0, MlpSlabs mlp = MlpSlabs{nullptr, 0, nullptr, nullptr},
                        FlushAdam ad = FlushAdam{nullptr, nullptr, nullptr, nullptr, nullptr, nullptr, 0.f, 0.f, 0.f},
                        StepSchedule sch = StepSchedule{nullptr, nullptr, 0.f, 0.f, 0, 0.f, 0.f, 0}) {
     if (n_max <= 0) return 0;
@@ -976,6 +980,11 @@
     const BwdPlan* plan = get_plan(*lv, single_mask, level_mask, max_blocks);
     if (!plan) return -2;
     if (ad.p && (half || adam_first_level(*lv, *plan) < 0)) return -2;
+    if (lv->bwd_plan & NGP_BWD_PLAN_MLP_STEP) {
+        if (!ad.p || !mlp.parts || plan->n_blocks <= 0) return -1;
+        mlp.step = mlp_step_lookup(mlp.dW);
+        if (!mlp.step) return -3;
+    }
     const WsLayout W = ws_layout(*lv, n_max);
     const char* base = reinterpret_cast<const char*>(workspace);
     const float* xyzc = reinterpret_cast<const float*>(base);
@@ -1006,7 +1015,7 @@
                                    const float* mlp_dw_parts, int n_parts, float* mlp_dw, void* stream) {
     if (!mlp_dw_parts || !mlp_dw || n_parts <= 0) return -1;
     return sliced_main(table_is_f16 != 0, dout, lv, n_max, n_dev, enc_pairs, dtable, found_inf, workspace, workspace_bytes, stream,
-                       0xffffffffu, 0, MlpSlabs{mlp_dw_parts, n_parts, mlp_dw});
+                       0xffffffffu, 0, MlpSlabs{mlp_dw_parts, n_parts, mlp_dw, nullptr});
 }
 
 int ngp_hash_bwd_sliced_main_levels(const float* dout, const ngp_hash_levels* lv, int n_max, const int32_t* n_dev, int enc_pairs,
@@ -1037,7 +1046,7 @@
                                   int n_parts, float* mlp_dw, float* table, float* table_m, float* table_v, uint16_t* table_bf16,
                                   const float* state_f, const int32_t* state_i, float beta1, float beta2, float eps, void* stream) {
     if (!table || !table_m || !table_v || !state_f || !state_i) return -1;
-    const MlpSlabs mlp = (mlp_dw_parts && mlp_dw && n_parts > 0) ? MlpSlabs{mlp_dw_parts, n_parts, mlp_dw} : MlpSlabs{nullptr, 0, nullptr};
+    const MlpSlabs mlp = (mlp_dw_parts && mlp_dw && n_parts > 0) ? MlpSlabs{mlp_dw_parts, n_parts, mlp_dw, nullptr} : MlpSlabs{nullptr, 0, nullptr, nullptr};
     return sliced_main(false, dout, lv, n_max, n_dev, enc_pairs, dtable, nullptr, workspace, workspace_bytes, stream, 0xffffffffu, 0, mlp,
                        FlushAdam{table, table_m, table_v, table_bf16, state_f, state_i, beta1, beta2, eps});
 }
@@ -1048,7 +1057,7 @@
                                        float* state_f, int32_t* state_i, float lr0, float eta_min, int t_max, float beta1, float beta2,
                                        float eps, float growth, float backoff, int growth_interval, void* stream) {
     if (!table || !table_m || !table_v || !state_f || !state_i || t_max <= 0 || n_max <= 0) return -1;
-    const MlpSlabs mlp = (mlp_dw_parts && mlp_dw && n_parts > 0) ? MlpSlabs{mlp_dw_parts, n_parts, mlp_dw} : MlpSlabs{nullptr, 0, nullptr};
+    const MlpSlabs mlp = (mlp_dw_parts && mlp_dw && n_parts > 0) ? MlpSlabs{mlp_dw_parts, n_parts, mlp_dw, nullptr} : MlpSlabs{nullptr, 0, nullptr, nullptr};
     return sliced_main(false, dout, lv, n_max, n_dev, enc_pairs, dtable, nullptr, workspace, workspace_bytes, stream, 0xffffffffu, 0, mlp,
                        FlushAdam{table, table_m, table_v, table_bf16, state_f, state_i, beta1, beta2, eps},
                        StepSchedule{state_f, state_i, lr0, eta_min, t_max, growth, backoff, growth_interval});
diff --git a/taichi-nerfs_amd/csrc/mlp.hip b/taichi-nerfs_amd/csrc/mlp.hip
--- a/taichi-nerfs_amd/csrc/mlp.hip
+++ b/taichi-nerfs_amd/csrc/mlp.hip
@@ -1,5 +1,8 @@
 #include "ngp_device.h"
 #include <stdlib.h>
+#include <string.h>
+#include <mutex>
+#include <vector>
 
 namespace ngp {
 
@@ -23,50 +26,58 @@
 constexpr int B_W2T = 34;
 constexpr int B_W1T = 38;
 
-__device__ __forceinline__ int chain_k(int s, int g, int j) { return 32 * s + 16 * (j >> 2) + 4 * g + (j & 3); }
-
-__device__ __forceinline__ int pair_nat(int p, int slot) { return slot < 2 ? 2 * p + slot : 2 * (15 - p) + (slot - 2); }
-__device__ __forceinline__ int enc_feat(int pairs, int g, int j) { return pairs ? pair_nat(2 * g + (j >> 2), j & 3) : 8 * g + j; }
-__device__ __forceinline__ int enc_row(int pairs, int mt, int i) { return pairs ? pair_nat(4 * mt + (i >> 2), i & 3) : 16 * mt + i; }
-
-__device__ __forceinline__ void pack_one(int tid, const float* W1, const float* W2, const float* W3, const float* W4,
-                                         const float* W5, int pairs, half_t* wpack) {
+__host__ __device__ __forceinline__ int chain_k(int s, int g, int j) { return 32 * s + 16 * (j >> 2) + 4 * g + (j & 3); }
+
+__host__ __device__ __forceinline__ int pair_nat(int p, int slot) { return slot < 2 ? 2 * p + slot : 2 * (15 - p) + (slot - 2); }
+__host__ __device__ __forceinline__ int enc_feat(int pairs, int g, int j) { return pairs ? pair_nat(2 * g + (j >> 2), j & 3) : 8 * g + j; }
+__host__ __device__ __forceinline__ int enc_row(int pairs, int mt, int i) { return pairs ? pair_nat(4 * mt + (i >> 2), i & 3) : 16 * mt + i; }
+
+constexpr int O_W1 = 0, O_W2 = 2048, O_W3 = 3072, O_W4 = 5120, O_W5 = 9216;
+__host__ __device__ __forceinline__ int pack_src(int tid, int pairs) {
     const int j = tid & 7, lane = (tid >> 3) & 63, frag = tid >> 9;
     const int i = lane & 15, g = lane >> 4;
-    float v = 0.0f;
     if (frag < F_W2) {
         const int mt = frag - F_W1;
-        v = W1[(16 * mt + i) * 32 + enc_feat(pairs, g, j)];
+        return O_W1 + (16 * mt + i) * 32 + enc_feat(pairs, g, j);
     } else if (frag < F_W3) {
         const int s = frag - F_W2;
-        v = W2[i * 64 + chain_k(s, g, j)];
+        return O_W2 + i * 64 + chain_k(s, g, j);
     } else if (frag < F_W4) {
         const int mt = frag - F_W3;
         const int k = (j < 4) ? (4 * g + j) : (16 + 4 * g + (j - 4));
-        v = W3[(16 * mt + i) * 32 + k];
+        return O_W3 + (16 * mt + i) * 32 + k;
     } else if (frag < F_W5) {
         const int mt = (frag - F_W4) >> 1, s = (frag - F_W4) & 1;
-        v = W4[(16 * mt + i) * 64 + chain_k(s, g, j)];
+        return O_W4 + (16 * mt + i) * 64 + chain_k(s, g, j);
     } else if (frag < B_W5T) {
         const int s = frag - F_W5;
-        v = (i < 3) ? W5[i * 64 + chain_k(s, g, j)] : 0.0f;
+        return (i < 3) ? O_W5 + i * 64 + chain_k(s, g, j) : -1;
     } else if (frag < B_W4T) {
         const int mt = frag - B_W5T;
         const int k = 4 * g + j;
-        v = (j < 4 && k < 3) ? W5[k * 64 + 16 * mt + i] : 0.0f;
+        return (j < 4 && k < 3) ? O_W5 + k * 64 + 16 * mt + i : -1;
     } else if (frag < B_W3T) {
         const int mt = (frag - B_W4T) >> 1, s = (frag - B_W4T) & 1;
-        v = W4[chain_k(s, g, j) * 64 + 16 * mt + i];
+        return O_W4 + chain_k(s, g, j) * 64 + 16 * mt + i;
     } else if (frag < B_W2T) {
         const int s = frag - B_W3T;
-        v = W3[chain_k(s, g, j) * 32 + 16 + i];
+        return O_W3 + chain_k(s, g, j) * 32 + 16 + i;
     } else if (frag < B_W1T) {
         const int mt = frag - B_W2T;
-        v = (j < 4) ? W2[(4 * g + j) * 64 + 16 * mt + i] : 0.0f;
+        return (j < 4) ? O_W2 + (4 * g + j) * 64 + 16 * mt + i : -1;
     } else {
         const int mt = (frag - B_W1T) >> 1, s = (frag - B_W1T) & 1;
-        v = W1[chain_k(s, g, j) * 32 + enc_row(pairs, mt, i)];
-    }
+        return O_W1 + chain_k(s, g, j) * 32 + enc_row(pairs, mt, i);
+    }
+}
+
+__device__ __forceinline__ void pack_one(int tid, const float* W1, const float* W2, const float* W3, const float* W4,
+                                         const float* W5, int pairs, half_t* wpack) {
+    const int src = pack_src(tid, pairs);
+    float v = 0.0f;
+    if (src >= O_W4) v = src >= O_W5 ? W5[src - O_W5] : W4[src - O_W4];
+    else if (src >= O_W2) v = src >= O_W3 ? W3[src - O_W3] : W2[src - O_W2];
+    else if (src >= 0) v = W1[src];
     wpack[tid] = (half_t)v;
 }
 
@@ -106,7 +117,7 @@
     __syncthreads();
     for (int item = threadIdx.x; item < N_ALL_FRAGS * 64; item += blockDim.x) {
 #pragma unroll
-        for (int j = 0; j < 8; ++j) pack_one(8 * item + j, wl, wl + 2048, wl + 3072, wl + 5120, wl + 9216, pairs, wpack);
+        for (int j = 0; j < 8; ++j) pack_one(8 * item + j, wl + O_W1, wl + O_W2, wl + O_W3, wl + O_W4, wl + O_W5, pairs, wpack);
     }
 }
 
@@ -618,6 +629,46 @@
 #include "../../profiles/microbench/mlp_bwd_reg_kernel.inc"
 #endif
 
+static int build_slot_map(int pairs, uint32_t* slots) {
+    for (int w = 0; w < NGP_MLP_NW; ++w) slots[w] = 0xffffffffu;
+    int n = 0;
+    for (int t = 0; t < N_ALL_FRAGS * 64 * 8; ++t) {
+        const int w = pack_src(t, pairs);
+        if (w < 0) continue;
+        if (w >= NGP_MLP_NW) return -1;
+        if (slots[w] == 0xffffffffu) slots[w] = (NGP_MLP_NO_SLOT << 16) | (uint32_t)t;
+        else if ((slots[w] >> 16) == NGP_MLP_NO_SLOT) slots[w] = (slots[w] & 0xffffu) | ((uint32_t)t << 16);
+        else return -1;
+        ++n;
+    }
+    for (int w = 0; w < NGP_MLP_NW; ++w) if (slots[w] == 0xffffffffu) return -1;
+    return n;
+}
+static_assert(N_ALL_FRAGS * 64 * 8 < (int)NGP_MLP_NO_SLOT, "a slot index fits sixteen bits");
+
+struct StepEntry { const float* dW; MlpStep* dev; int device; };
+static std::mutex g_step_mu;
+static std::vector<StepEntry> g_steps;
+struct SlotMap { int device, pairs; uint32_t* dev; };
+static std::vector<SlotMap> g_slot_maps;
+
+static const uint32_t* device_slot_map(int device, int pairs) {
+    for (const SlotMap& s : g_slot_maps) if (s.device == device && s.pairs == pairs) return s.dev;
+    uint32_t host[NGP_MLP_NW];
+    if (build_slot_map(pairs, host) < 0) return nullptr;
+    uint32_t* dev = nullptr;
+    if (hipMalloc(&dev, sizeof(host)) != hipSuccess) return nullptr;
+    if (hipMemcpy(dev, host, sizeof(host), hipMemcpyHostToDevice) != hipSuccess) { (void)hipFree(dev); return nullptr; }
+    g_slot_maps.push_back(SlotMap{device, pairs, dev});
+    return dev;
+}
+
+const MlpStep* mlp_step_lookup(const float* dW) {
+    std::lock_guard<std::mutex> lock(g_step_mu);
+    for (const StepEntry& e : g_steps) if (e.dW == dW) return e.dev;
+    return nullptr;
+}
+
 }
 
 using namespace ngp;
@@ -641,6 +692,49 @@
                        (half_t*)wpack);
     NGP_LAUNCH_CHECK();
     return 0;
+}
+
+int ngp_mlp_pack_slot_map(int enc_pairs, int32_t* src_of_slot, uint32_t* slots_of_weight) {
+    uint32_t slots[NGP_MLP_NW];
+    const int n = build_slot_map(enc_pairs != 0, slots);
+    if (n < 0) return -1;
+    if (src_of_slot) for (int t = 0; t < N_ALL_FRAGS * 64 * 8; ++t) src_of_slot[t] = pack_src(t, enc_pairs != 0);
+    if (slots_of_weight) memcpy(slots_of_weight, slots, sizeof(slots));
+    return n;
+}
+
+int ngp_mlp_step_register(float* dW, float* p, float* m, float* v, uint16_t* wpack, int enc_pairs) {
+    if (!dW || !p || !m || !v || !wpack) return -1;
+    int device = 0;
+    if (hipGetDevice(&device) != hipSuccess) return -1;
+    std::lock_guard<std::mutex> lock(g_step_mu);
+    const uint32_t* slots = device_slot_map(device, enc_pairs != 0);
+    if (!slots) return -1;
+    StepEntry* e = nullptr;
+    for (StepEntry& x : g_steps) if (x.dW == dW) e = &x;
+    if (e) {
+        if (hipDeviceSynchronize() != hipSuccess) return -1;
+        if (e->device != device) return -1;
+    } else {
+        MlpStep* dev = nullptr;
+        if (hipMalloc(&dev, sizeof(MlpStep)) != hipSuccess) return -1;
+        g_steps.push_back(StepEntry{dW, dev, device});
+        e = &g_steps.back();
+    }
+    const MlpStep host = {p, m, v, (half_t*)wpack, slots};
+    if (hipMemcpy(e->dev, &host, sizeof(host), hipMemcpyHostToDevice) != hipSuccess) return -1;
+    return 0;
+}
+
+int ngp_mlp_step_unregister(const float* dW) {
+    std::lock_guard<std::mutex> lock(g_step_mu);
+    for (size_t k = 0; k < g_steps.size(); ++k)
+        if (g_steps[k].dW == dW) {
+            (void)hipFree(g_steps[k].dev);
+            g_steps.erase(g_steps.begin() + k);
+            return 0;
+        }
+    return -1;
 }
 
 int ngp_adam_mlp_pack(float* p, float* g, float* m, float* v, const float* state_f, const int32_t* state_i, float beta1, float beta2,
diff --git a/taichi-nerfs_amd/csrc/ngp_device.h b/taichi-nerfs_amd/csrc/ngp_device.h
--- a/taichi-nerfs_amd/csrc/ngp_device.h
+++ b/taichi-nerfs_amd/csrc/ngp_device.h
@@ -160,31 +160,6 @@
     z = (z ^ (z >> 27)) * 0x94D049BB133111EBull;
     z ^= z >> 31;
     return (float)(unsigned int)(z >> 40) * (1.0f / 16777216.0f);
-}
-
-constexpr int NGP_MLP_NW = 9408;
-constexpr int NGP_MLP_REDUCE_BLOCKS = (NGP_MLP_NW + 63) / 64;
-constexpr int NGP_MLP_REDUCE_THREADS = 1024;
-__device__ __forceinline__ void mlp_dw_reduce_block(const float* __restrict__ parts, int n_parts, float* __restrict__ dW, int block) {
-    __shared__ float partial[15][64];
-    const int lane = threadIdx.x & 63, w = block * 64 + lane, q = threadIdx.x >> 6;
-    float v[16];
-#pragma unroll
-    for (int k = 0; k < 16; ++k) {
-        const int p = q + 16 * k;
-        v[k] = (w < NGP_MLP_NW && p < n_parts) ? parts[(size_t)p * NGP_MLP_NW + w] : 0.0f;
-    }
-    float s = 0.0f;
-    for (int p = q + 256; p < n_parts; p += 16) s += (w < NGP_MLP_NW) ? parts[(size_t)p * NGP_MLP_NW + w] : 0.0f;
-#pragma unroll
-    for (int k = 0; k < 16; k += 4) s += (v[k] + v[k + 1]) + (v[k + 2] + v[k + 3]);
-    if (q) partial[q - 1][lane] = s;
-    __syncthreads();
-    if (q == 0 && w < NGP_MLP_NW) {
-#pragma unroll
-        for (int k = 0; k < 15; ++k) s += partial[k][lane];
-        dW[w] += s;
-    }
 }
 
 enum { SI_ITER = 0, SI_OPT_STEP = 1, SI_GROWTH = 2, SI_FOUND_INF = 3, SI_SKIP = 4, SI_SKIPPED_TOTAL = 5 };
@@ -235,6 +210,64 @@
     v = v * c.beta2 + gr * gr * (1.0f - c.beta2);
     const float denom = sqrtf(v) / c.bc2_sqrt + c.eps;
     p = p - c.step_size * (m / denom);
+}
+
+constexpr int NGP_MLP_NW = 9408;
+constexpr int NGP_MLP_REDUCE_BLOCKS = (NGP_MLP_NW + 63) / 64;
+constexpr int NGP_MLP_REDUCE_THREADS = 1024;
+
+constexpr uint32_t NGP_MLP_NO_SLOT = 0xffffu;
+struct MlpStep {
+    float* p;
+    float* m;
+    float* v;
+    _Float16* wpack;
+    const uint32_t* slots;
+};
+const MlpStep* mlp_step_lookup(const float* dW);
+
+template <bool STEP = false>
+__device__ __forceinline__ void mlp_dw_reduce_block(const float* __restrict__ parts, int n_parts, float* __restrict__ dW, int block,
+                                                    const MlpStep* __restrict__ step = nullptr, const float* sf = nullptr,
+                                                    const int32_t* si = nullptr, float beta1 = 0.f, float beta2 = 0.f, float eps = 0.f) {
+    __shared__ float partial[15][64];
+    const int lane = threadIdx.x & 63, w = block * 64 + lane, q = threadIdx.x >> 6;
+    float p0 = 0.f, m0 = 0.f, v0 = 0.f, g0 = 0.f;
+    uint32_t sl = 0u;
+    MlpStep st;
+    if constexpr (STEP) {
+        st = *step;
+        if (q == 0 && w < NGP_MLP_NW) { p0 = st.p[w]; m0 = st.m[w]; v0 = st.v[w]; g0 = dW[w]; sl = st.slots[w]; }
+    }
+    float v[16];
+#pragma unroll
+    for (int k = 0; k < 16; ++k) {
+        const int p = q + 16 * k;
+        v[k] = (w < NGP_MLP_NW && p < n_parts) ? parts[(size_t)p * NGP_MLP_NW + w] : 0.0f;
+    }
+    float s = 0.0f;
+    for (int p = q + 256; p < n_parts; p += 16) s += (w < NGP_MLP_NW) ? parts[(size_t)p * NGP_MLP_NW + w] : 0.0f;
+#pragma unroll
+    for (int k = 0; k < 16; k += 4) s += (v[k] + v[k + 1]) + (v[k + 2] + v[k + 3]);
+    if (q) partial[q - 1][lane] = s;
+    __syncthreads();
+    if (q == 0 && w < NGP_MLP_NW) {
+#pragma unroll
+        for (int k = 0; k < 15; ++k) s += partial[k][lane];
+        if constexpr (!STEP) {
+            dW[w] += s;
+        } else {
+            const float g = g0 + s;
+            if (si[SI_SKIP] == 0) {
+                adam_update(p0, m0, v0, g, adam_consts(sf, beta1, beta2, eps));
+                st.p[w] = p0; st.m[w] = m0; st.v[w] = v0;
+            }
+            dW[w] = 0.0f;
+            const _Float16 h = (_Float16)p0;
+            st.wpack[sl & 0xffffu] = h;
+            if ((sl >> 16) != NGP_MLP_NO_SLOT) st.wpack[sl >> 16] = h;
+        }
+    }
 }
 
 template <int SHADOW, bool GRAD16 = false>
diff --git a/taichi-nerfs_amd/ngp_hip/experiment.py b/taichi-nerfs_amd/ngp_hip/experiment.py
--- a/taichi-nerfs_amd/ngp_hip/experiment.py
+++ b/taichi-nerfs_amd/ngp_hip/experiment.py
@@ -13,6 +13,7 @@
     "bwd_concentrated": "1 / 0: the scatter-add's concentrated-scene task plan (unset: on for multi-cascade scenes)",
     "mlp_dw": "atomic: round 3's float-atomic weight gradients instead of per-block slabs",
     "mlp_dw_reduce": "prologue: the slab sum in the prologue launch instead of the head of the scatter-add launch",
+    "mlp_step": "tail: the MLP's Adam + fp16 repack as one workgroup of the optimizer launch instead of per weight at the head of the scatter-add launch",
     "svox_trilinear": "1: VoxelGrid(use_trilinear=None) interpolates the eight surrounding grid points instead of reading the nearest (how the reference's train.py, which has no flag for it, reaches the lookup)",
     "comm_overlap": "1: one scatter-add launch + async reduce-scatter / Adam / all-gather per level group",
     "comm_groups": "first level of each group in launch order (default '8,0')",
diff --git a/taichi-nerfs_amd/ngp_hip/lib.py b/taichi-nerfs_amd/ngp_hip/lib.py
--- a/taichi-nerfs_amd/ngp_hip/lib.py
+++ b/taichi-nerfs_amd/ngp_hip/lib.py
@@ -35,6 +35,7 @@
 NGP_MAX_LEVELS = _ABI.defines["NGP_MAX_LEVELS"]
 ABI_VERSION = _ABI.defines["NGP_ABI_VERSION"]
 BWD_PLAN_DETERMINISTIC, BWD_PLAN_CONCENTRATED = _ABI.defines["NGP_BWD_PLAN_DETERMINISTIC"], _ABI.defines["NGP_BWD_PLAN_CONCENTRATED"]
+BWD_PLAN_MLP_STEP = _ABI.defines["NGP_BWD_PLAN_MLP_STEP"]
 
 
 class HashLevels(ctypes.Structure):
diff --git a/taichi-nerfs_amd/ngp_hip/trainer.py b/taichi-nerfs_amd/ngp_hip/trainer.py
--- a/taichi-nerfs_amd/ngp_hip/trainer.py
+++ b/taichi-nerfs_amd/ngp_hip/trainer.py
@@ -94,6 +94,7 @@
         self._init_table_copies(model, dev, exp_step_factor)
         self._init_exchange(model, dev, exchange)
         self.repack()
+        self._register_mlp_step()
 
     def _init_options(self, model, exp_step_factor, max_samples, chunked_forward, process_group, world_size):
         ck = _exp.get("chunked_fwd")
@@ -235,6 +236,8 @@
         self._flush_adam = _exp.get("flush_adam", "1") != "0"
         self._fold_prologue = True
         self._adam_prefix = {}
+        self._mlp_step = _exp.get("mlp_step", "scatter") == "scatter"
+        self._mlp_step_key = None
         self.deterministic = False
         self._concentrated = concentrated_scene(exp_step_factor, model.cascades)
         self.set_deterministic(os.environ.get("NGP_DETERMINISTIC", "0") == "1")
@@ -270,6 +273,18 @@
     def _scatter_mode(self):
         return ((_lib_mod.BWD_PLAN_DETERMINISTIC if self.deterministic else 0)
                 | (_lib_mod.BWD_PLAN_CONCENTRATED if self._concentrated else 0))
+
+    def _register_mlp_step(self):
+        if not self._mlp_step:
+            return
+        key = (self.mlp_grad.data_ptr(), self.mlp_flat.data_ptr(), self.mlp_m.data_ptr(), self.mlp_v.data_ptr(), self.wpack.data_ptr(),
+               self.enc_pairs)
+        if key == self._mlp_step_key:
+            return
+        with torch.cuda.device(self.dev):
+            check(self.L.ngp_mlp_step_register(_ptr(self.mlp_grad), _ptr(self.mlp_flat), _ptr(self.mlp_m), _ptr(self.mlp_v),
+                                               _ptr(self.wpack), self.enc_pairs), "ngp_mlp_step_register")
+        self._mlp_step_key = key
 
     def repack(self):
         ws = self.model._mlp_weights()
@@ -581,7 +596,8 @@
         quartet = [_ptr(t if mlp else None) for t in (self.mlp_flat, self.mlp_grad, self.mlp_m, self.mlp_v)]
         rest = (_ptr(self.state_f), _ptr(self.state_i), self.beta1, self.beta2, self.eps, self.enc_pairs, _ptr(self.wpack), st)
         if n == 0:
-            check(L.ngp_adam_mlp_pack(*quartet, *rest), "ngp_adam_mlp_pack")
+            if mlp:
+                check(L.ngp_adam_mlp_pack(*quartet, *rest), "ngp_adam_mlp_pack")
             return
 
         def at(t):
@@ -642,7 +658,9 @@
 
     def _tail_flush_adam(self, s, n_parts, npre):
         L, A, st, sf, si = self.L, s.A, s.st, self.state_f, self.state_i
-        args = (_ptr(A.d_enc), ctypes.byref(s.lvp), A.cap, _ptr(s.cnt), s.P, _ptr(self.table_grad), _ptr(s.ws), s.ws.numel(),
+        step_here = self._mlp_step and self._mlp_step_key is not None
+        lvp = s.cfg.levels.with_plan(s.lvp.bwd_plan | _lib_mod.BWD_PLAN_MLP_STEP) if step_here else s.lvp
+        args = (_ptr(A.d_enc), ctypes.byref(lvp), A.cap, _ptr(s.cnt), s.P, _ptr(self.table_grad), _ptr(s.ws), s.ws.numel(),
                 _ptr(self.mlp_parts), n_parts, _ptr(self.mlp_grad), _ptr(self.table), _ptr(self.table_m), _ptr(self.table_v),
                 _ptr(self._copy16), _ptr(sf), _ptr(si))
         if self._fold_prologue:
@@ -653,7 +671,7 @@
             self._prologue(st)
             check(L.ngp_hash_bwd_sliced_main_adam(*args, self.beta1, self.beta2, self.eps, st), "ngp_hash_bwd_sliced_main_adam")
         s.pf.reach(4)
-        self._adam(st, 0, npre, self.table_grad)
+        self._adam(st, 0, npre, self.table_grad, mlp=not step_here)
 
     def _composite_with_distortion(self, s, target):
         L, st, sf = self.L, s.st, self.state_f
@@ -905,9 +923,16 @@
         TrainArena.invalidate_coarse()
         self._master_stale = False
         self.repack()
+        self._register_mlp_step()
 
     def close(self):
         side, self._side, self._side_low = getattr(self, "_side_low", None), None, None
+        key, self._mlp_step_key = getattr(self, "_mlp_step_key", None), None
+        if key is not None:
+            try:
+                self.L.ngp_mlp_step_unregister(ctypes.c_void_p(key[0]))
+            except Exception:
+                pass
         host, self._marched_host = getattr(self, "_marched_host", None), None
         dflt, self._side_default = getattr(self, "_side_default", None), None
         if host is not None:
```

New measurement: 18.10 million (median of 6 runs). No clear change (+1.5%).
